# multicom-toolbox/Chromosome3D

Hardware: AMD Instinct MI355X
Metric: SA-steps/sec (replica-steps/s, 20 replicas of chr1_500kb in all: 20 per GPU, weak scaling; regions of 20 steps inside the first 2172 of the schedule's 5172: MD and FIRE steps in front of the final minimisation); wall-clock per chromosome (higher is better)
Workload: dtype f32

## Files before the change

chromosome3d_amd/csrc/c3d_api.cpp:

```cpp
#include <cstdlib>

#include "c3d_ctx.h"

using namespace c3d::host;

namespace {
inline void philox4x32(const uint32_t ctr_in[4], const uint32_t key_in[2], uint32_t out[4]) {
    uint32_t c[4] = {ctr_in[0], ctr_in[1], ctr_in[2], ctr_in[3]};
    uint32_t k[2] = {key_in[0], key_in[1]};
    for (int r = 0; r < 10; ++r) {
        const uint64_t p0 = (uint64_t)0xD2511F53u * c[0];
        const uint64_t p1 = (uint64_t)0xCD9E8D57u * c[2];
        const uint32_t n0 = (uint32_t)(p1 >> 32) ^ c[1] ^ k[0];
        const uint32_t n1 = (uint32_t)p1;
        const uint32_t n2 = (uint32_t)(p0 >> 32) ^ c[3] ^ k[1];
        const uint32_t n3 = (uint32_t)p0;
        c[0] = n0; c[1] = n1; c[2] = n2; c[3] = n3;
        k[0] += 0x9E3779B9u;
        k[1] += 0xBB67AE85u;
    }
    memcpy(out, c, sizeof(c));
}
inline double u01(uint32_t u) { return ((double)u + 0.5) * (1.0 / 4294967296.0); }
void philox_draw(uint64_t seed, uint32_t replica, uint32_t bead, uint32_t purpose, uint32_t out[4]) {
    const uint32_t ctr[4] = {bead, purpose, 0u, 0u};
    const uint32_t key[2] = {(uint32_t)(seed & 0xFFFFFFFFu) ^ (replica * 0x9E3779B9u), (uint32_t)(seed >> 32) + replica};
    philox4x32(ctr, key, out);
}
void normals4(uint64_t seed, uint32_t replica, uint32_t bead, uint32_t purpose, double g[4]) {
    uint32_t r[4];
    philox_draw(seed, replica, bead, purpose, r);
    const double two_pi = 6.283185307179586476925286766559;
    double a = sqrt(-2.0 * log(u01(r[0]))), b = two_pi * u01(r[1]);
    g[0] = a * cos(b); g[1] = a * sin(b);
    a = sqrt(-2.0 * log(u01(r[2]))); b = two_pi * u01(r[3]);
    g[2] = a * cos(b); g[3] = a * sin(b);
}

void release_context(c3d_ctx* c) {
    for (hipStream_t s : c->gstream) if (s) (void)hipStreamSynchronize(s);
    drop_graphs(c);
    free_replica_buffers(c);
    dev_free(c->buf.tgt); dev_free(c->buf.tgs2);
    dev_free(c->d_prog); dev_free(c->d_claim); dev_free(c->d_score);
    if (c->h_tmo) (void)hipHostFree(c->h_tmo);
    if (c->h_stage) (void)hipHostFree(c->h_stage);
    for (hipEvent_t e : {c->ev0, c->ev1, c->kev0, c->kev1, c->fork_ev}) if (e) (void)hipEventDestroy(e);
    for (hipEvent_t e : c->gev) if (e) (void)hipEventDestroy(e);
    for (hipStream_t s : c->gstream) if (s && s != c->stream) (void)hipStreamDestroy(s);
    if (c->stream) (void)hipStreamDestroy(c->stream);
}

void set_dims(c3d_ctx* c, int n) {
    c->n = n;
    c->npad = (n + 255) / 256 * 256;
    c->ntiles = (n + c3d::kTileRows - 1) / c3d::kTileRows;
    c->rep_floats = (size_t)3 * c->npad;
}

float pad_coord(int comp, int k) { return c3d::kPadCoord * (float)(comp + 1) + 16.0f * (float)k; }

void pack(const c3d_ctx* c, const float* aos, std::vector<float>& soa, bool pad_far) {
    soa.assign(c->rep_floats * c->nrep, 0.0f);
    for (int r = 0; r < c->nrep; ++r) {
        float* base = soa.data() + c->rep_floats * r;
        for (int comp = 0; comp < 3; ++comp) {
            for (int i = 0; i < c->n; ++i) base[(size_t)comp * c->npad + i] = aos[((size_t)r * c->n + i) * 3 + comp];
            if (pad_far)
                for (int i = c->n; i < c->npad; ++i) base[(size_t)comp * c->npad + i] = pad_coord(comp, i - c->n);
        }
    }
}
void unpack(const c3d_ctx* c, const float* soa, float* aos) {
    for (int r = 0; r < c->nrep; ++r) {
        const float* base = soa + c->rep_floats * r;
        for (int comp = 0; comp < 3; ++comp)
            for (int i = 0; i < c->n; ++i) aos[((size_t)r * c->n + i) * 3 + comp] = base[(size_t)comp * c->npad + i];
    }
}

void copy_energies(const c3d_ctx* c, double* e) {
    const double* h = static_cast<const double*>(c->h_stage);
    for (int r = 0; r < c->nrep; ++r) for (int k = 0; k < 3; ++k) e[3 * r + k] = h[4 * r + k];
}
float final_repel_s(const c3d_ctx* c) { return c->stages.empty() ? 0.85f : c->stages.back().repel_s; }

int import64(c3d_ctx* c) {
    LAUNCH_TRY("fp64 import", c3d::launch_import64(dev_model(c), c->buf.X[c->parity], c->b64, c->stream));
    HIP_TRY(hipStreamSynchronize(c->stream));
    return C3D_OK;
}
}

namespace c3d::host {
void free_replica_buffers(c3d_ctx* c) {
    for (int k = 0; k < 2; ++k) {
        dev_free(c->buf.X[k]); dev_free(c->buf.V[k]); dev_free(c->buf.P[k]); dev_free(c->buf.S[k]);
    }
    dev_free(c->d_crec);
    c->crec_bytes = 0; c->cl_ok = false;
    dev_free(c->buf.Vinit); dev_free(c->buf.E); dev_free(c->d_feval);
    dev_free(c->d_sym_scratch); dev_free(c->d_sym_tiles);
    dev_free(c->lb.hist); dev_free(c->lb.part); dev_free(c->lb.S[0]); dev_free(c->lb.S[1]);
    dev_free(c->lb64.hist); dev_free(c->lb64.part); dev_free(c->lb64.S[0]); dev_free(c->lb64.S[1]);
    c->lbfgs_parity = -1;
    dev_free(c->b64.T); dev_free(c->b64.t10); dev_free(c->b64.Vinit); dev_free(c->b64.F);
    for (int k = 0; k < 2; ++k) { dev_free(c->b64.X[k]); dev_free(c->b64.V[k]); dev_free(c->b64.P[k]); dev_free(c->b64.S[k]); }
    c->have_replicas = false;
}
int build_targets64(c3d_ctx* c) {
    const c3d::Model64 m = c3d::model64(dev_model(c), c->model);
    LAUNCH_TRY("fp64 targets", c3d::launch_targets64(m, c3d::form64(m, 0.0, 0), c->b64.t10, c->b64.T, c->stream));
    HIP_TRY(hipStreamSynchronize(c->stream));
    return C3D_OK;
}

int ensure_stage(c3d_ctx* c, size_t bytes) {
    if (bytes <= c->h_stage_bytes) return C3D_OK;
    if (c->h_stage) { HIP_TRY(hipStreamSynchronize(c->stream)); (void)hipHostFree(c->h_stage); c->h_stage = nullptr; c->h_stage_bytes = 0; }
    const size_t cap = std::max<size_t>(bytes, (size_t)64 << 10);
    HIP_TRY(hipHostMalloc(&c->h_stage, cap, hipHostMallocDefault));
    c->h_stage_bytes = cap;
    return C3D_OK;
}
int read_back(c3d_ctx* c, const void* dev, size_t bytes) {
    if (int rc = ensure_stage(c, bytes)) return rc;
    HIP_TRY(hipMemcpyAsync(c->h_stage, dev, bytes, hipMemcpyDeviceToHost, c->stream));
    HIP_TRY(hipStreamSynchronize(c->stream));
    return C3D_OK;
}
}

extern "C" int c3d_device_count(void) {
    int n = 0;
    if (hipGetDeviceCount(&n) != hipSuccess) return 0;
    return n;
}

extern "C" int c3d_create(int device, c3d_ctx** out) {
    if (!out) return fail(C3D_ERR_INVALID, "c3d_create: null out");
    int ndev = 0;
    if (hipGetDeviceCount(&ndev) != hipSuccess || ndev < 1)
        return fail(C3D_ERR_NO_DEVICE, "no HIP device visible: libc3d has no CPU fallback");
    if (device < 0 || device >= ndev) return fail(C3D_ERR_INVALID, "c3d_create: device index out of range");
    HIP_TRY(hipSetDevice(device));
    hipDeviceProp_t prop;
    HIP_TRY(hipGetDeviceProperties(&prop, device));
    if (strncmp(prop.gcnArchName, "gfx950", 6) != 0)
        return fail(C3D_ERR_NO_DEVICE, std::string("device is ") + prop.gcnArchName + ", libc3d is built for gfx950 only");
    int num_xcc = 0;
    if (hipDeviceGetAttribute(&num_xcc, hipDeviceAttributeNumberOfXccs, device) != hipSuccess) num_xcc = 0;
    if (const int rc = preload_units(device)) return rc;
    c3d_ctx* c = new c3d_ctx();
    c->device = device;
    c->num_cus = prop.multiProcessorCount;
    c->num_xcc = num_xcc;
    c3d_default_model(&c->model);
    c3d_default_fire(&c->fire);
    c->stages.resize(c3d_default_schedule(nullptr, 0, 3000));
    c3d_default_schedule(c->stages.data(), (int)c->stages.size(), 3000);
    Entry gate(c, 0u, false);
    if (gate.rc != C3D_OK) { delete c; return gate.rc; }
    bool ok = hipStreamCreateWithFlags(&c->stream, hipStreamNonBlocking) == hipSuccess &&
              hipEventCreate(&c->ev0) == hipSuccess && hipEventCreate(&c->ev1) == hipSuccess &&
              hipEventCreate(&c->kev0) == hipSuccess && hipEventCreate(&c->kev1) == hipSuccess &&
              hipEventCreateWithFlags(&c->fork_ev, hipEventDisableTiming) == hipSuccess;
    c->gstream[0] = c->stream;
    ok = ok && hipHostMalloc(reinterpret_cast<void**>(&c->h_tmo), 64, hipHostMallocMapped) == hipSuccess;
    if (ok) {
        *c->h_tmo = 0;
        ok = hipHostGetDevicePointer(reinterpret_cast<void**>(&c->h_tmo_dev), c->h_tmo, 0) == hipSuccess &&
             hipMalloc(&c->d_claim, sizeof(unsigned) * c3d_ctx::kClaimWords * c3d_ctx::kClaimSets) == hipSuccess;
        c->h_tmo[1] = 0;
    }
    if (!ok) {
        c3d_destroy(c);
        return fail(C3D_ERR_HIP, "cannot create HIP stream/events");
    }
    *out = c;
    return C3D_OK;
}

extern "C" void c3d_destroy(c3d_ctx* c) {
    if (!c) return;
    c->ifr.release();
    {
        Entry gate(c, 0u, false);
        release_context(c);
    }
    delete c;
}

static constexpr int kDefaultMaxBeads = C3D_MAX_BEADS_DEFAULT;
static constexpr int kMaxBeadsLimit = C3D_MAX_BEADS_LIMIT;
static_assert(kDefaultMaxBeads == c3d::kMaxStagedCols, "the default limit is the staged form's");
static int too_many_beads(const c3d_ctx* c, const char* fn, int n) {
    char b[192];
    if (c->max_beads == kDefaultMaxBeads)
        snprintf(b, sizeof b, "%s: %d beads: more than %d are accepted only after c3d_set_option(\"max_beads\", n) (up to %d)", fn, n,
                 kDefaultMaxBeads, kMaxBeadsLimit);
    else
        snprintf(b, sizeof b, "%s: %d beads: more than max_beads = %d (the option goes up to %d)", fn, n, c->max_beads, kMaxBeadsLimit);
    return fail(C3D_ERR_INVALID, b);
}
static constexpr int kRankPrefetchBeads = 2048;

extern "C" int c3d_set_if_matrix(c3d_ctx* c, const double* IF, int n, double alpha, double K) {
    if (!c || !IF || n < 2) return fail(C3D_ERR_INVALID, "c3d_set_if_matrix: bad arguments");
    if (n > c->max_beads) return too_many_beads(c, "c3d_set_if_matrix", n);
    C3D_ENTRY(c, 0u);
    free_replica_buffers(c);
    set_dims(c, n);
    const size_t nn = (size_t)n * n;
    c->ifr.join();
    c->ifr.valid = false;
    if (c->prefetch_ranks && n <= kRankPrefetchBeads) {
        try {
            c->ifr.matrix.assign(IF, IF + nn);
            c->ifr.n = n; c->ifr.range = 3;
            c3d_ctx::IfRanks* const w = &c->ifr;
            c->ifr.worker = std::thread([w] {
                try { c3d::if_pair_ranks(w->matrix.data(), w->n, w->range, w->rank, w->m, w->mean, w->saa); w->valid = true; }
                catch (...) { w->valid = false; }
            });
        } catch (...) { c->ifr.release(); }
    } else {
        c->ifr.release();
    }
    DevTmp<double> dIF, dP, dpart;
    DevTmp<int32_t> ddist;
    DevTmp<unsigned char> dflags;
    DevTmp<unsigned> dnflag;
    const int npartial = 64;
    dev_free(c->buf.tgt); dev_free(c->buf.tgs2);
    c->have_targets = false;
    HIP_TRY(hipMalloc(&dIF.p, sizeof(double) * nn));
    HIP_TRY(hipMalloc(&dP.p, sizeof(double) * nn));
    HIP_TRY(hipMalloc(&dpart.p, sizeof(double) * npartial));
    HIP_TRY(hipMalloc(&ddist.p, sizeof(int32_t) * nn));
    HIP_TRY(hipMalloc(&dflags.p, nn));
    HIP_TRY(hipMalloc(&dnflag.p, sizeof(unsigned)));
    HIP_TRY(hipMalloc(&c->buf.tgt, sizeof(float) * (size_t)n * c->npad));
    HIP_TRY(hipMemcpyAsync(dIF.p, IF, sizeof(double) * nn, hipMemcpyHostToDevice, c->stream));
    HIP_TRY(hipMemsetAsync(dnflag.p, 0, sizeof(unsigned), c->stream));
    HIP_TRY(hipMemsetAsync(dflags.p, 0, nn, c->stream));
    LAUNCH_TRY("K1 launch", c3d::launch_if_to_target(dIF.p, n, c->npad, alpha, K, c->model.min_sep, c->model.rep_sep, dP.p, dpart.p, npartial, ddist.p,
                                                     c->buf.tgt, dflags.p, dnflag.p, c->stream));
    c->h_dist10.resize(nn);
    c->r_i.clear(); c->r_j.clear(); c->r_t10.clear();
    unsigned nflag = 0;
    HIP_TRY(hipMemcpyAsync(c->h_dist10.data(), ddist.p, sizeof(int32_t) * nn, hipMemcpyDeviceToHost, c->stream));
    HIP_TRY(hipMemcpyAsync(&nflag, dnflag.p, sizeof(unsigned), hipMemcpyDeviceToHost, c->stream));
    HIP_TRY(hipStreamSynchronize(c->stream));
    c->k1_recomputed = 0;
    if (nflag) {
        std::vector<unsigned char> flags(nn);
        HIP_TRY(hipMemcpyAsync(flags.data(), dflags.p, nn, hipMemcpyDeviceToHost, c->stream));
        HIP_TRY(hipStreamSynchronize(c->stream));
        double sum = 0.0;
        for (size_t k = 0; k < nn; ++k) sum += pow(IF[k], alpha);
        const double mean = sum / ((double)n * (double)n);
        for (size_t k = 0; k < nn; ++k) {
            if (!flags[k]) continue;
            double v = pow(IF[k], alpha) / mean;
            if (v == 0) continue;
            v = K / v;
            char b[64];
            snprintf(b, sizeof b, "%.1f", v);
            char* dot = strchr(b, '.');
            long long t = atoll(b) * 10 + (dot ? dot[1] - '0' : 0);
            if (t > 2000000000LL) t = 2000000000LL;
            ++c->k1_recomputed;
            if ((int32_t)t == c->h_dist10[k]) continue;
            c->h_dist10[k] = (int32_t)t;
            const int i = (int)(k / n), j = (int)(k % n);
            const int sep = i > j ? i - j : j - i;
            const float enc = (sep >= c->model.min_sep && t > 0) ? (float)((double)t / 10.0) : 0.0f;
            HIP_TRY(hipMemcpyAsync(c->buf.tgt + (size_t)i * c->npad + j, &enc, sizeof(float), hipMemcpyHostToDevice, c->stream));
            HIP_TRY(hipStreamSynchronize(c->stream));
            dev_free(c->buf.tgs2);
            ++c->k1_patched;
        }
    }
    int R = 0;
    for (int i = 0; i < n; ++i)
        for (int j = i + 1; j < n; ++j)
            if (j - i >= c->model.min_sep && c->h_dist10[(size_t)i * n + j] > 0) ++R;
    c->R = R;
    c->have_targets = true;
    build_program(c);
    return C3D_OK;
}

extern "C" int c3d_set_restraints(c3d_ctx* c, int n, int R, const int32_t* ri, const int32_t* rj, const int32_t* rt10) {
    if (!c || n < 2 || R < 0 || (R > 0 && (!ri || !rj || !rt10))) return fail(C3D_ERR_INVALID, "c3d_set_restraints: bad arguments");
    if (n > c->max_beads) return too_many_beads(c, "c3d_set_restraints", n);
    C3D_ENTRY(c, 0u);
    free_replica_buffers(c);
    c->ifr.release();
    set_dims(c, n);
    std::vector<float> enc((size_t)n * c->npad);
    std::fill(enc.begin(), enc.end(), 0.0f);
    for (int k = 0; k < R; ++k) {
        const int i = ri[k] - 1, j = rj[k] - 1;
        if (i < 0 || j < 0 || i >= n || j >= n || i == j) return fail(C3D_ERR_INVALID, "c3d_set_restraints: index out of range");
        if (rt10[k] <= 0) continue;
        const float t = (float)((double)rt10[k] / 10.0);
        enc[(size_t)i * c->npad + j] = c3d::encode_target_host(t);
        enc[(size_t)j * c->npad + i] = c3d::encode_target_host(t);
    }
    dev_free(c->buf.tgt); dev_free(c->buf.tgs2);
    HIP_TRY(hipMalloc(&c->buf.tgt, sizeof(float) * enc.size()));
    HIP_TRY(hipMemcpyAsync(c->buf.tgt, enc.data(), sizeof(float) * enc.size(), hipMemcpyHostToDevice, c->stream));
    HIP_TRY(hipStreamSynchronize(c->stream));
    c->h_dist10.clear();
    {
        std::vector<std::pair<uint64_t, int>> key;
        key.reserve(R);
        for (int k = 0; k < R; ++k) {
            const int i = std::min(ri[k], rj[k]) - 1, j = std::max(ri[k], rj[k]) - 1;
            key.emplace_back((uint64_t)i * n + j, k);
        }
        std::sort(key.begin(), key.end());
        c->r_i.clear(); c->r_j.clear(); c->r_t10.clear();
        int32_t last = 0;
        for (size_t q = 0; q < key.size(); ++q) {
            if (rt10[key[q].second] > 0) last = rt10[key[q].second];
            if (q + 1 < key.size() && key[q + 1].first == key[q].first) continue;
            if (last > 0) { c->r_i.push_back((int32_t)(key[q].first / n)); c->r_j.push_back((int32_t)(key[q].first % n)); c->r_t10.push_back(last); }
            last = 0;
        }
    }
    c->R = R;
    c->have_targets = true;
    build_program(c);
    return C3D_OK;
}

extern "C" int c3d_get_dist10(c3d_ctx* c, int32_t* out) {
    if (!c || !out) return fail(C3D_ERR_INVALID, "c3d_get_dist10: null argument");
    if (c->h_dist10.empty()) return fail(C3D_ERR_INVALID, "c3d_get_dist10: targets were not built from an IF matrix");
    memcpy(out, c->h_dist10.data(), sizeof(int32_t) * c->h_dist10.size());
    return C3D_OK;
}
extern "C" int c3d_num_beads(const c3d_ctx* c) { return c ? c->n : 0; }
extern "C" int c3d_num_restraints(const c3d_ctx* c) { return c ? c->R : 0; }

// ... 390 lines not shown
```

chromosome3d_amd/csrc/c3d_cluster.hip:

```cpp
#include <hip/hip_ext.h>
#include <atomic>
#include <type_traits>
#include <cstdio>
#include <cstdlib>

#include "c3d_step_core.h"

namespace c3d {

typedef unsigned u32x4 __attribute__((ext_vector_type(4)));
constexpr int kClMaxThreads = 1024;

#ifdef C3D_STAMPS
__device__ unsigned long long g_cstamps[64][8];
__device__ unsigned long long g_pstamps[8];
#define CSTAMP(k) do { if (stamper) g_cstamps[s & 63][k] = __builtin_amdgcn_s_memrealtime(); } while (0)
#define CSTAMP_C(k) do { if (cstamper) g_cstamps[s & 63][k] = __builtin_amdgcn_s_memrealtime(); } while (0)
#else
#define CSTAMP(k) do { } while (0)
#define CSTAMP_C(k) do { } while (0)
#endif

template <int POT, int RPW, int NB, int WL, bool LATE, bool TWO>
__device__ __forceinline__ void cluster_body(
    const float* __restrict__ tgt, unsigned* __restrict__ claim, const StepRun* __restrict__ runs, const int P, const int CW, const int NH,
    const int static_place, const int nbeads, const int run0, const int skip0, const int nsteps,
    const unsigned tag_base, u32x4* __restrict__ rec, volatile unsigned* __restrict__ timeout, const unsigned expected,
    const AnnealIO& io, const DevModel& m, const DevFire& fp) {
    constexpr int NPAD = 256 * NB;
    constexpr int MAXT = NPAD / 8;
    constexpr int KUMAX = NB > 2 ? 3 : 2;
    extern __shared__ __attribute__((aligned(16))) float smem[];
    float* xs = smem;
    float* ys = smem + NPAD;
    float* zs = smem + 2 * NPAD;
    float* ps = smem + 3 * NPAD;
    float* fbuf = ps + 4 * MAXT;
    float* cbuf = fbuf + 3 * 64;
    float* lbuf = cbuf + 3 * 64;
    float* lcon = lbuf + 3 * 64;
    float* dump = lcon + 3 * 4 * 2 * 64;
    int* s_slot = reinterpret_cast<int*>(dump + 4);
#ifdef C3D_STAMPS
    const unsigned long long t_entry = __builtin_amdgcn_s_memrealtime();
#endif
    const int tid = threadIdx.x, lane = tid & 63, wave = tid >> 6;
    const int nthreads = (CW + NH) * 64;
    const int RW = CW * RPW;

    const int xcc = (int)(__builtin_amdgcn_s_getreg((3 << 11) | 20) & 0x7);
    const int sp_mode = static_place & 0xff, xcd0 = (static_place >> 8) & 0xff, nxcd = (static_place >> 16) & 0xff;
    int slot;
    if (sp_mode) {
        const unsigned off = ((unsigned)xcc - blockIdx.x + (sp_mode == 2 && blockIdx.x == 0 ? 1u : 0u)) & 7u;
        if (tid == 0) atomicOr(&claim[9], 1u << off);
        slot = (int)(blockIdx.x >> 3);
    } else {
        if (tid == 0) *s_slot = (int)atomicAdd(&claim[xcc], 1u);
        __syncthreads();
        slot = *s_slot;
    }
    const int lxcd = xcc - xcd0;
    const int lrep = lxcd + nxcd * (slot / P), part = slot % P;
#ifdef C3D_STAMPS
    const unsigned long long t_placed = __builtin_amdgcn_s_memrealtime();
#endif
    const bool is_compute = wave >= NH, is_h0 = wave == 0;
    const int cwave = wave - NH;
    const int wg_row0 = part * RW;
    const int row0 = wg_row0 + cwave * RPW;
    const StepRun first_run = runs[run0];
    float4 traw[RPW][NB];
#pragma unroll
    for (int r = 0; r < RPW; ++r)
#pragma unroll
        for (int jb = 0; jb < NB; ++jb) {
            float4 t = make_float4(0, 0, 0, 0);
            if (is_compute) {
                const float* trow = tgt + (size_t)min(row0 + r, nbeads - 1) * NPAD + 256 * jb;
                if (jb < NB - 1 || WL == 4) t = *reinterpret_cast<const float4*>(trow + 4 * lane);
                else if constexpr (WL == 3) {
                    struct F3 { float a, b, c; };
                    const F3 q = *reinterpret_cast<const F3*>(trow + 3 * lane);
                    t = make_float4(q.a, q.b, q.c, 0.0f);
                } else if constexpr (WL == 2) {
                    const float2 q = *reinterpret_cast<const float2*>(trow + 2 * lane);
                    t = make_float4(q.x, q.y, 0.0f, 0.0f);
                } else t = make_float4(trow[lane], 0.0f, 0.0f, 0.0f);
            }
            traw[r][jb] = t;
        }
    if (lxcd < 0 || lxcd >= nxcd || lrep >= m.nrep_g) return;
    const int rep = m.rep_base + lrep;
    const bool solo = P == 1;
    if (!is_compute) __builtin_amdgcn_s_setprio(3);

    const size_t roff = (size_t)rep * 3 * NPAD;
    const int hrow = wg_row0 + lane;
    const bool hfin = is_h0 && lane < RW && hrow < m.n;
#define C3D_HROW_INDEX const size_t ix = roff + hrow, iy = ix + NPAD, iz = iy + NPAD
    constexpr int rec_stride = NPAD + NPAD / 4;
    constexpr int KT = (MAXT + 63) / 64;
    constexpr bool late = LATE;
    const int gthreads = late ? nthreads - 64 : nthreads;
    const int gtid = late ? tid - 64 : tid;
    const int units = late ? m.n : m.n + 2 * m.ntiles;
    const int ku = (units + gthreads - 1) / gthreads;
    const auto rsrc = __builtin_amdgcn_make_buffer_rsrc(rec, 0, (int)(sizeof(u32x4) * 2 * m.nrep_g * rec_stride), 0x00020000);

    float vcx = 0.0f, vcy = 0.0f, vcz = 0.0f;
    FireState st;
    float4 cin[2], pin4 = make_float4(0, 0, 0, 0);
    {
        const float* xin = io.xin;
        const float* pin = io.pin;
        const float* vin = io.vin;
#pragma unroll
        for (int k = 0; k < 2; ++k) {
            const int b = 4 * (tid + k * nthreads);
            cin[k] = b < 3 * NPAD ? *reinterpret_cast<const float4*>(xin + roff + b) : make_float4(0, 0, 0, 0);
        }
        if (tid < m.ntiles) pin4 = reinterpret_cast<const float4*>(pin)[(size_t)rep * m.ntiles + tid];
        if (hfin) { C3D_HROW_INDEX; vcx = vin[ix]; vcy = vin[iy]; vcz = vin[iz]; }
        st = io.sin[rep];
    }
    float* const lc = lcon + (size_t)((wave >= 1 && wave <= 3) ? wave - 1 : 0) * (4 * 2 * 64);
    if (!is_compute && !is_h0 && wave <= 3 && m.nleft > 0) {
        for (int q = 0; q < 4; ++q) {
            const int k = 8 * (wave - 1) + 8 * (NH - 1) * q + (lane >> 3), c = lane & 7;
            float b = 0.0f, a = 0.0f;
            if (k < RW && c < m.nleft && wg_row0 + k < m.n) {
                const float t = tgt[(size_t)(wg_row0 + k) * NPAD + m.jl0 + c];
                b = t * m.inv_rs;
                a = t > 0.0f ? m.inv_rs : 0.0f;
            }
            lc[(2 * q) * 64 + lane] = b; lc[(2 * q + 1) * 64 + lane] = a;
        }
    }
#pragma unroll
    for (int k = 0; k < 2; ++k) {
        const int b = 4 * (tid + k * nthreads);
        if (b < 3 * NPAD) *reinterpret_cast<float4*>(smem + b) = cin[k];
    }
    if (tid < m.ntiles) reinterpret_cast<float4*>(ps)[tid] = pin4;
    if (tid < 3 * 64) lbuf[tid] = 0.0f;
#ifdef C3D_STAMPS
    asm volatile("s_waitcnt lgkmcnt(0)" ::: "memory");
    const unsigned long long t_coords = __builtin_amdgcn_s_memrealtime();
#endif
    constexpr bool PK = POT == 4;
    float4 tv[PK ? 1 : RPW][NB];
    PairConsts2<PK ? RPW : 1, NB> pc;
    float4* const mw = reinterpret_cast<float4*>(dump + 8) + (size_t)(is_compute ? cwave : 0) * (RPW * NB * 64);
    if constexpr (PK) {
        pair_consts2_build<RPW, NB>(m, traw, is_compute, lane, pc, mw);
    } else {
        DevStep p0{};
#pragma unroll
        for (int r = 0; r < RPW; ++r)
#pragma unroll
            for (int jb = 0; jb < NB; ++jb) {
                tv[r][jb] = pair_b<false>(m, traw[r][jb]);
                if (is_compute) mw[(r * NB + jb) * 64 + lane] = pair_a<false>(m, p0, traw[r][jb]);
            }
    }
#ifdef C3D_STAMPS
    asm volatile("s_waitcnt vmcnt(0) lgkmcnt(0)" ::: "memory");
    const unsigned long long t_targets = __builtin_amdgcn_s_memrealtime();
#endif
    int gsrc[KUMAX], gda[KUMAX], gdb[KUMAX], gdc[KUMAX];
    const int dump_off = (int)(dump - smem);
#pragma unroll
    for (int k = 0; k < KUMAX; ++k) {
        const int u = min(max(gtid + gthreads * k, 0), units - 1);
        int src, da, db = dump_off, dc = dump_off;
        if (u < m.n) { src = u; da = u; db = NPAD + u; dc = 2 * NPAD + u; }
        else {
            const int j = u - m.n, t = j >> 1;
            src = NPAD + j;
            if ((j & 1) == 0) { da = 3 * NPAD + 4 * t; db = da + 1; dc = da + 2; }
            else da = 3 * NPAD + 4 * t + 3;
        }
        if (gtid < 0 || gtid + gthreads * k >= units) da = db = dc = dump_off;
        gsrc[k] = src; gda[k] = da; gdb[k] = db; gdc[k] = dc;
    }

#ifdef C3D_STAMPS
    const bool stamper = lrep == 0 && part == 0 && is_h0 && lane == 0;
    const bool cstamper = lrep == 0 && part == 0 && cwave == 0 && lane == 0;
    if (stamper) { g_pstamps[0] = t_entry; g_pstamps[1] = __builtin_amdgcn_s_memrealtime(); g_pstamps[6] = t_placed; }
    if (cstamper) { g_pstamps[4] = t_targets; g_pstamps[5] = t_coords; }
#endif
    auto role_loop = [&](auto role) {
    constexpr int ROLE = decltype(role)::value;
    int s = 0;
    StepRun cur = first_run;
    for (int run = run0;; ++run) {
      if (run != run0) cur = runs[run];
      const DevStep p = cur.p;
      const int count = cur.count;
      const bool needs_partials = p.kind == 0 || p.kind == 1 || p.kind == 2 || (TWO && p.kind == 5);
      for (int it = run == run0 ? skip0 : 0; it < count; ++it, ++s) {
#ifdef C3D_STAMPS
        if (cstamper && s == 0) g_pstamps[7] = __builtin_amdgcn_s_memrealtime();
#endif
        __syncthreads();
        CSTAMP(0);
#ifdef C3D_STAMPS
        if (stamper && s == 0) g_pstamps[2] = __builtin_amdgcn_s_memrealtime();
#endif
        CSTAMP_C(6);

        float hx0 = 0.0f, hy0 = 0.0f, hz0 = 0.0f;
        StepScalars sc;
        sc.lam = 1.0f; sc.cmx = sc.cmy = sc.cmz = 0.0f; sc.keep = 0.0f; sc.mix = 0.0f;
        if constexpr (ROLE == 0) {
            if (p.kind != 4) {
                float Fx, Fy, Fz;
                if constexpr (PK) tile_pair_sums_pk<RPW, NB, WL>(m, p, pc, mw, xs, ys, zs, row0, lane, Fx, Fy, Fz);
                else tile_pair_sums_reg<POT, RPW, NB, WL, 1>(m, p, tv, mw, xs, ys, zs, row0, lane, Fx, Fy, Fz);
                if (lane < RPW) {
                    const int k = cwave * RPW + lane;
                    fbuf[k] = Fx; fbuf[64 + k] = Fy; fbuf[128 + k] = Fz;
                }
                CSTAMP_C(7);
            }
        } else if constexpr (ROLE == 1) {
            if (p.kind != 2 && !(TWO && p.kind == 5)) { st.dt = fp.dt_start; st.alpha = fp.alpha_start; st.npos = 0; st.pad = 0; }
            float4 psum = make_float4(0, 0, 0, 0);
            if (needs_partials) {
                if (late && !solo && s > 0) {
                    const unsigned tagp = tag_base + (unsigned)s;
                    const int basep = ((s & 1) * m.nrep_g + lrep) * rec_stride + NPAD;
                    u32x4 a[KT], b[KT];
                    unsigned spins = 0;
                    for (;;) {
                        bool ok = true;
                        asm volatile("" ::: "memory");
#pragma unroll
                        for (int k = 0; k < KT; ++k) {
                            const int t = min(lane + 64 * k, m.ntiles - 1);
                            a[k] = __builtin_amdgcn_raw_buffer_load_b128(rsrc, (basep + 2 * t) * 16, 0, 16);
                            b[k] = __builtin_amdgcn_raw_buffer_load_b128(rsrc, (basep + 2 * t + 1) * 16, 0, 16);
                        }
#pragma unroll
                        for (int k = 0; k < KT; ++k) ok &= a[k].x == tagp && b[k].x == tagp;
                        if (__all(ok)) break;
                        __builtin_amdgcn_s_sleep(1);
                        ++spins;
                        if (spins > (1u << 18) || ((spins & 1023u) == 0 && *timeout != 0u)) {
                            if (lane == 0) *timeout = 1u;
                            return;
                        }
                    }
#pragma unroll
                    for (int k = 0; k < KT; ++k)
                        if (lane + 64 * k < m.ntiles)
                            reinterpret_cast<float4*>(ps)[lane + 64 * k] = make_float4(__uint_as_float(a[k].y), __uint_as_float(a[k].z), __uint_as_float(a[k].w), __uint_as_float(b[k].y));
                }
                for (int t = lane; t < m.ntiles; t += 64) {
                    const float4 q = reinterpret_cast<const float4*>(ps)[t];
                    psum.x += q.x; psum.y += q.y; psum.z += q.z; psum.w += q.w;
                }
                psum = wave_sum4(psum);
                psum.x = __uint_as_float(__builtin_amdgcn_readfirstlane(__float_as_uint(psum.x)));
                psum.y = __uint_as_float(__builtin_amdgcn_readfirstlane(__float_as_uint(psum.y)));
                psum.z = __uint_as_float(__builtin_amdgcn_readfirstlane(__float_as_uint(psum.z)));
                psum.w = __uint_as_float(__builtin_amdgcn_readfirstlane(__float_as_uint(psum.w)));
            }
            sc = step_scalars<TWO>(m, p, fp, psum, st);
            if (lane < RW && hrow < NPAD) { hx0 = xs[hrow]; hy0 = ys[hrow]; hz0 = zs[hrow]; }
            CSTAMP(1);
        } else if (p.kind != 4) {
            for (int cb = 16 * (wave - 1); cb < RW; cb += 16 * (NH - 1)) {
                const int k = cb + (lane >> 2);
                float cx, cy, cz;
                chain_term(m, p, xs, ys, zs, wg_row0 + k, lane & 3, k < RW, cx, cy, cz);
                cx = quad_chain_sum(cx); cy = quad_chain_sum(cy); cz = quad_chain_sum(cz);
                if ((lane & 3) == 0 && k < RW) { cbuf[k] = cx; cbuf[64 + k] = cy; cbuf[128 + k] = cz; }
            }
            if (m.nleft > 0) {
                const PairK kk = pair_k(m, p);
                for (int q = 0; q < 4; ++q) {
                    const int k = 8 * (wave - 1) + 8 * (NH - 1) * q + (lane >> 3), c = lane & 7;
                    if (8 * (wave - 1) + 8 * (NH - 1) * q < RW) {
                        const bool active = k < RW && c < m.nleft && wg_row0 + k < m.n;
                        float lx, ly, lz;
                        leftover_terms<POT, false>(m, p, kk, xs, ys, zs, min(wg_row0 + k, m.n - 1), c, active, lc[(2 * q) * 64 + lane], lc[(2 * q + 1) * 64 + lane], lx, ly, lz);
                        if (c == 0 && k < RW) { lbuf[k] = lx; lbuf[64 + k] = ly; lbuf[128 + k] = lz; }
                    }
                }
            }
        }
        __syncthreads();
        CSTAMP(2);
        const bool last = s + 1 == nsteps;
        const unsigned tag = tag_base + (unsigned)s + 1u;
        const int base = (((s + 1) & 1) * m.nrep_g + lrep) * rec_stride;

        if constexpr (ROLE == 1) {
            float4 q = make_float4(0, 0, 0, 0);
            float xn = 0.0f, yn = 0.0f, zn = 0.0f;
            auto row_update = [&](auto kc) {
                constexpr int K = decltype(kc)::value;
                DevStep pk = p;
                pk.kind = K;
                if (hfin) {
                    float Fx = 0.0f, Fy = 0.0f, Fz = 0.0f;
                    if constexpr (K != 4) {
                        const float sx0 = fbuf[lane], sy0 = fbuf[64 + lane], sz0 = fbuf[128 + lane];
                        const float lx = lbuf[lane], ly = lbuf[64 + lane], lz = lbuf[128 + lane];
                        const float cx = cbuf[lane], cy = cbuf[64 + lane], cz = cbuf[128 + lane];
                        const bool lo = m.nleft > 0;
                        const float sx = lo ? sx0 + lx : sx0, sy = lo ? sy0 + ly : sy0, sz = lo ? sz0 + lz : sz0;
                        Fx = row_total<false>(pk, sx, cx);
                        Fy = row_total<false>(pk, sy, cy);
                        Fz = row_total<false>(pk, sz, cz);
                    }
                    float vx0 = vcx, vy0 = vcy, vz0 = vcz;
                    if constexpr (K == 3 || K == 6) { vx0 = vy0 = vz0 = 0.0f; }
                    else if constexpr (K == 4) { C3D_HROW_INDEX; const float* vinit = io.vinit; vx0 = vinit[ix]; vy0 = vinit[iy]; vz0 = vinit[iz]; }
                    finish_row(m, pk, fp, sc, st, Fx, Fy, Fz, hx0, hy0, hz0, vx0, vy0, vz0, xn, yn, zn, vcx, vcy, vcz, q);
                    if (!last && !solo) {
                        u32x4 o;
                        o.x = tag; o.y = __float_as_uint(xn); o.z = __float_as_uint(yn); o.w = __float_as_uint(zn);
                        __builtin_amdgcn_raw_buffer_store_b128(o, rsrc, (base + hrow) * 16, 0, 0);
                    }
                } else {
                    xn = hx0; yn = hy0; zn = hz0;
                }
            };
            bool two_point_step = false;
            if constexpr (TWO) {
                two_point_step = p.kind >= 5;
                if (p.kind == 5) row_update(std::integral_constant<int, 5>{});
                else if (p.kind == 6) row_update(std::integral_constant<int, 6>{});
            }
            if (!two_point_step) switch (p.kind) {
                case 0: row_update(std::integral_constant<int, 0>{}); break;
                case 1: row_update(std::integral_constant<int, 1>{}); break;
                case 2: row_update(std::integral_constant<int, 2>{}); break;
                case 3: row_update(std::integral_constant<int, 3>{}); break;
                default: row_update(std::integral_constant<int, 4>{}); break;
            }
            if (late && !last && !solo) { CSTAMP(4); __builtin_amdgcn_s_barrier(); }
            float4 t = q;
            t.x += dpp_mov<0xB1>(t.x); t.y += dpp_mov<0xB1>(t.y); t.z += dpp_mov<0xB1>(t.z); t.w += dpp_mov<0xB1>(t.w);
            t.x += dpp_mov<0x4E>(t.x); t.y += dpp_mov<0x4E>(t.y); t.z += dpp_mov<0x4E>(t.z); t.w += dpp_mov<0x4E>(t.w);
            t.x += dpp_mov<0x12C>(t.x); t.y += dpp_mov<0x12C>(t.y); t.z += dpp_mov<0x12C>(t.z); t.w += dpp_mov<0x12C>(t.w);
            CSTAMP(3);
            if (last) {
                if (hfin) {
                    C3D_HROW_INDEX;
                    float* xout = io.xout;
                    float* vout = io.vout;
                    xout[ix] = xn; xout[iy] = yn; xout[iz] = zn;
                    vout[ix] = vcx; vout[iy] = vcy; vout[iz] = vcz;
                }
                const int tl = (wg_row0 + lane) >> 3;
                if ((lane & 7) == 0 && lane < RW && tl < m.ntiles) reinterpret_cast<float4*>(io.pout)[(size_t)rep * m.ntiles + tl] = t;
                if (lane == 0 && part == 0) io.sout[rep] = st;
                if (lane == 0 && atomicAdd(&claim[8], 1u) + 1u == expected) {
                    const unsigned seen = sp_mode ? atomicOr(&claim[9], 0u) : 1u;
                    if ((seen & (seen - 1u)) == 0u) timeout[1] = tag_base | 1u;
                    else timeout[2] = 1u;
                }
#ifdef C3D_STAMPS
                if (stamper) g_pstamps[3] = __builtin_amdgcn_s_memrealtime();
#endif
                return;
            }
            if (solo) {
                if (lane < RW && hrow < NPAD) { xs[hrow] = xn; ys[hrow] = yn; zs[hrow] = zn; }
                if ((lane & 7) == 0 && lane < RW) reinterpret_cast<float4*>(ps)[lane >> 3] = t;
            } else if ((lane & 7) == 0 && lane < RW && ((wg_row0 + lane) >> 3) < m.ntiles) {
                u32x4 o0, o1;
                o0.x = tag; o0.y = __float_as_uint(t.x); o0.z = __float_as_uint(t.y); o0.w = __float_as_uint(t.z);
                o1.x = tag; o1.y = __float_as_uint(t.w); o1.z = 0u; o1.w = 0u;
                const int u0 = base + NPAD + 2 * ((wg_row0 + lane) >> 3);
                __builtin_amdgcn_raw_buffer_store_b128(o0, rsrc, u0 * 16, 0, 0);
                __builtin_amdgcn_raw_buffer_store_b128(o1, rsrc, (u0 + 1) * 16, 0, 0);
            }
            CSTAMP(5);
            if (solo || late) continue;
        }
        {
            if (last) return;
            if (solo) continue;
            __builtin_amdgcn_s_barrier();
            u32x4 v[KUMAX];
            unsigned spins = 0;
            for (;;) {
                bool ok = true;
                asm volatile("" ::: "memory");
#pragma unroll
                for (int k = 0; k < KUMAX; ++k)
                    if (k < ku) v[k] = __builtin_amdgcn_raw_buffer_load_b128(rsrc, (base + gsrc[k]) * 16, 0, 16);
#pragma unroll
                for (int k = 0; k < KUMAX; ++k)
                    if (k < ku) ok &= v[k].x == tag;
                if (__all(ok)) break;
                __builtin_amdgcn_s_sleep(1);
                ++spins;
                if (spins > (1u << 18) || ((spins & 1023u) == 0 && *timeout != 0u)) {
                    if (lane == 0) *timeout = 1u;
                    return;
                }
            }
#pragma unroll
            for (int k = 0; k < KUMAX; ++k)
                if (k < ku) { smem[gda[k]] = __uint_as_float(v[k].y); smem[gdb[k]] = __uint_as_float(v[k].z); smem[gdc[k]] = __uint_as_float(v[k].w); }
        }
      }
    }
    };
    if (is_compute) role_loop(std::integral_constant<int, 0>{});
    else if (is_h0) role_loop(std::integral_constant<int, 1>{});
    else role_loop(std::integral_constant<int, 2>{});
}

#define C3D_CLUSTER_ARGS                                                                                                                  \
    const float* __restrict__ tgt, unsigned* __restrict__ claim, const StepRun* __restrict__ runs, const int P, const int CW, const int NH, \
    const int static_place, const int nbeads, const int run0, const int skip0, const int nsteps, const unsigned tag_base,                 \
    u32x4* __restrict__ rec, volatile unsigned* __restrict__ timeout, const unsigned expected, const AnnealIO io, const DevModel m, const DevFire fp
#define C3D_CLUSTER_PASS tgt, claim, runs, P, CW, NH, static_place, nbeads, run0, skip0, nsteps, tag_base, rec, timeout, expected, io, m, fp
template <int POT, int RPW, int NB, int WL, bool LATE>
__global__ __launch_bounds__(kClMaxThreads) void k_cluster(C3D_CLUSTER_ARGS) { cluster_body<POT, RPW, NB, WL, LATE, false>(C3D_CLUSTER_PASS); }
template <int POT, int RPW, int NB, int WL, bool LATE>
__global__ __launch_bounds__(kClMaxThreads) void k_cluster_tp(C3D_CLUSTER_ARGS) { cluster_body<POT, RPW, NB, WL, LATE, true>(C3D_CLUSTER_PASS); }
#undef C3D_CLUSTER_ARGS
#undef C3D_CLUSTER_PASS

constexpr bool cluster_late_ok(int pot, int rpw, int nb, int wl) { return pot >= 3 && rpw * (4 * (nb - 1) + wl) >= 6; }
#ifndef C3D_CLUSTER_POT
#ifdef C3D_STAMPS
hipError_t read_cluster_stamps(unsigned long long* out) { return hipMemcpyFromSymbol(out, HIP_SYMBOL(g_cstamps), sizeof(unsigned long long) * 64 * 8); }
hipError_t read_cluster_pstamps(unsigned long long* out) { return hipMemcpyFromSymbol(out, HIP_SYMBOL(g_pstamps), sizeof(unsigned long long) * 8); }
#endif

__global__ __launch_bounds__(kClMaxThreads) void k_tear16(u32x4* buf, unsigned* stop, unsigned long long* stats, int iters) {
    const auto rsrc = __builtin_amdgcn_make_buffer_rsrc(buf, 0, kClMaxThreads * 16, 0x00020000);
    const int tid = threadIdx.x;
    if (blockIdx.x == 0) {
        for (int i = 1; i <= iters; ++i) {
            u32x4 v; v.x = v.y = v.z = v.w = (unsigned)i;
            __builtin_amdgcn_raw_buffer_store_b128(v, rsrc, tid * 16, 0, 0);
        }
        __threadfence();
        if (tid == 0) atomicExch(stop, 1u);
        return;
    }
    const auto ssrc = __builtin_amdgcn_make_buffer_rsrc(stop, 0, 4, 0x00020000);
    unsigned long long reads = 0, torn = 0, fresh = 0;
    unsigned lastv = 0;
    for (unsigned guard = 0; guard < (1u << 26); ++guard) {
        asm volatile("" ::: "memory");
        const u32x4 v = __builtin_amdgcn_raw_buffer_load_b128(rsrc, tid * 16, 0, 16);
        ++reads;
        if (!(v.x == v.y && v.y == v.z && v.z == v.w)) ++torn;
        if (v.x != lastv) { ++fresh; lastv = v.x; }
        if ((reads & 255) == 0 && __builtin_amdgcn_raw_buffer_load_b32(ssrc, 0, 0, 16) != 0u) break;
    }
    atomicAdd(&stats[0], reads); atomicAdd(&stats[1], torn); atomicAdd(&stats[2], fresh);
}
hipError_t launch_tear16(int num_cus, void* buf, unsigned* stop, unsigned long long* stats, int iters, hipStream_t s) {
    hipLaunchKernelGGL(k_tear16, dim3(num_cus), dim3(kClMaxThreads), 0, s, reinterpret_cast<u32x4*>(buf), stop, stats, iters);
    return hipGetLastError();
}


bool cluster_plan(const DevModel& m, int num_cus, int num_xcc, int forced_geom, int forced_late, int xcd_count, ClusterPlan* plan) {
    if (m.npad > 1024 || num_xcc != 8 || num_cus < 8 || num_cus % 8) return false;
    const int cus_per_xcd = num_cus / 8;
    if (xcd_count < 1 || xcd_count > 8) return false;
    const int per_xcd = (m.nrep_g + xcd_count - 1) / xcd_count;
    const int nb = m.npad / 256;
    static const int geoms[][4] = {{8, 1, 4, 1}, {8, 2, 4, 1}, {12, 2, 4, 1}, {8, 4, 4, 1}, {10, 4, 4, 1}, {12, 4, 4, 1}, {8, 3, 4, 1},
                                   {4, 2, 4, 1}, {4, 4, 4, 1}, {6, 4, 4, 1}};
    double best = 1e30;
    bool found = false;
    const int fcw = forced_geom / 100, frpw = forced_geom / 10 % 10, fnh = forced_geom % 10;
    for (const auto& g : geoms) {
        const int cw = g[0], rpw = g[1], nh = g[2], wpc = g[3], rw = cw * rpw;
        if (fcw && (cw != fcw || rpw != frpw || nh != fnh)) continue;
        if (rw % 8 || rw > 64) continue;
        if (rpw * nb > 8) continue;
        if (m.noe_pot < 3 && (m.wl != 4 || m.nleft != 0)) continue;
        if (m.nleft > 0 && (nh != 4 || (rw + 8 * (nh - 1) - 1) / (8 * (nh - 1)) > 4)) continue;
        const int P = (m.n + rw - 1) / rw;
        if (per_xcd * P > cus_per_xcd * wpc) continue;
        const int threads = (cw + nh) * 64;
        const int kumax = nb > 2 ? 3 : 2;
        const int late = P > 1 && forced_late != 0 && cluster_late_ok(m.noe_pot, rpw, nb, m.wl) &&
                         (m.noe_pot != 4 || ((cw + 3) / 4) * rpw * (4 * (nb - 1) + m.wl) >= 12);
        if ((late ? m.n : m.n + 2 * ((m.n + 7) / 8)) > (late ? threads - 64 : threads) * kumax) continue;
        size_t lds = sizeof(float) * (3 * m.npad + 4 * (m.npad / 8) + 9 * 64 + 24 * 64 + 16) + (size_t)cw * rpw * nb * 64 * 16;
        if (wpc == 1) { if (lds < 84 * 1024) lds = 84 * 1024; }
        else if (lds > 78 * 1024 || threads > 512) continue;
        const int wps = (cw * wpc + 3) / 4;
        const double per_slot = m.noe_pot == 4 ? (rpw / 2) * 22.0 + (rpw & 1) * 19.0 : rpw * 15.0;
        const double valu = (wps == 1 ? 1.6 : (wps == 2 ? 1.15 : 1.0)) * wps * ((4 * (nb - 1) + m.wl) * per_slot + 60.0);
        const double serial = 200.0 + (P > 1 ? 140.0 + 0.92 * m.n : 0.0);
        const double cost = wpc == 1 ? valu + serial : (valu > serial ? valu + 0.35 * serial : 0.5 * valu + serial);
        if (cost < best) {
            best = cost; found = true;
            plan->rpw = rpw; plan->cw = cw; plan->helpers = nh; plan->wgs_per_cu = wpc; plan->parts = P; plan->per_xcd = per_xcd;
            plan->grid = num_cus * wpc; plan->threads = threads; plan->units = 2 * rw; plan->device = 0; plan->lds = lds;
            plan->expected = (unsigned)(m.nrep_g * P);
            plan->late_tiles = late;
            plan->xcd_count = xcd_count;
        }
    }
    return found;
}

size_t cluster_record_bytes(const DevModel& m, const ClusterPlan& pl) { (void)pl; return (size_t)2 * m.nrep_g * (m.npad + m.npad / 4) * 16; }

#endif

template <int POT, int RPW, int NB, int WL, bool LATE>
static hipError_t cluster_go(const DevModel& m, const DevFire& fp, const ClusterPlan& pl, const AnnealIO& io, const float* tgt, void* rec,
                             const StepRun* runs, int run0, int skip0, int nsteps, unsigned tag_base, unsigned* timeout, unsigned* claim,
                             hipStream_t s) {
#if defined(C3D_CLUSTER_TP)
    constexpr bool kHasLean = false, kHasTp = true;
#elif defined(C3D_CLUSTER_POT)
    constexpr bool kHasLean = true, kHasTp = false;
#else
    constexpr bool kHasLean = true, kHasTp = true;
#endif
    const int tp = pl.two_point ? 1 : 0;
    if ((tp && !kHasTp) || (!tp && !kHasLean)) return hipErrorInvalidValue;
    const int sp = (pl.static_place & 0xff) | ((pl.xcd_base & 0xff) << 8) | ((pl.xcd_count & 0xff) << 16);
#define C3D_CL_LAUNCH(K)                                                                                                                              \
    do {                                                                                                                                              \
        if (pl.t0 && pl.t1)                                                                                                                           \
            hipExtLaunchKernelGGL((K<POT, RPW, NB, WL, LATE>), dim3(pl.grid), dim3(pl.threads), pl.lds, s, pl.t0, pl.t1, 0, tgt, claim, runs,          \
                                  pl.parts, pl.cw, pl.helpers, sp, m.n, run0, skip0, nsteps, tag_base, reinterpret_cast<u32x4*>(rec), timeout, pl.expected, io, m, fp); \
        else                                                                                                                                          \
            hipLaunchKernelGGL((K<POT, RPW, NB, WL, LATE>), dim3(pl.grid), dim3(pl.threads), pl.lds, s, tgt, claim, runs, pl.parts, pl.cw, pl.helpers, \
                               sp, m.n, run0, skip0, nsteps, tag_base, reinterpret_cast<u32x4*>(rec), timeout, pl.expected, io, m, fp);                \
    } while (0)
    if constexpr (kHasTp) { if (tp) C3D_CL_LAUNCH(k_cluster_tp); }
    if constexpr (kHasLean) { if (!tp) C3D_CL_LAUNCH(k_cluster); }
#undef C3D_CL_LAUNCH
    return hipGetLastError();
}
template <int POT, class F>
static void for_each_cluster_form(F&& f) {
    auto widths = [&](auto R, auto B) {
        auto w = [&](auto W) {
            f(R, B, W, bool_c<false>{});
            if constexpr (cluster_late_ok(POT, R, B, W)) f(R, B, W, bool_c<true>{});
        };
        w(int_c<4>{});
        if constexpr (POT >= 3) { w(int_c<3>{}); w(int_c<2>{}); w(int_c<1>{}); }
    };
    widths(int_c<1>{}, int_c<1>{}); widths(int_c<1>{}, int_c<2>{}); widths(int_c<1>{}, int_c<3>{}); widths(int_c<1>{}, int_c<4>{});
    widths(int_c<2>{}, int_c<1>{}); widths(int_c<2>{}, int_c<2>{}); widths(int_c<2>{}, int_c<3>{}); widths(int_c<2>{}, int_c<4>{});
    widths(int_c<3>{}, int_c<1>{}); widths(int_c<3>{}, int_c<2>{});
    widths(int_c<4>{}, int_c<1>{}); widths(int_c<4>{}, int_c<2>{});
}
template <int POT>
static hipError_t cluster_geom(const DevModel& m, const DevFire& fp, const ClusterPlan& pl, const AnnealIO& io, const float* tgt, void* rec,
                               const StepRun* runs, int run0, int skip0, int nsteps, unsigned tag_base, unsigned* timeout, unsigned* claim,
                               hipStream_t s) {
    hipError_t e = hipErrorInvalidValue;
    for_each_cluster_form<POT>([&](auto R, auto B, auto W, auto L) {
        if (pl.rpw == R && m.npad == 256 * B && m.wl == W && (pl.late_tiles != 0) == L)
            e = cluster_go<POT, R, B, W, L>(m, fp, pl, io, tgt, rec, runs, run0, skip0, nsteps, tag_base, timeout, claim, s);
    });
    return e;
}

template <int POT, bool TP>
static hipError_t cluster_prepare_unit() {
    hipError_t e = hipSuccess;
    for_each_cluster_form<POT>([&](auto R, auto B, auto W, auto L) {
        const void* k;
        if constexpr (TP) k = reinterpret_cast<const void*>(&k_cluster_tp<POT, R, B, W, L>);
        else k = reinterpret_cast<const void*>(&k_cluster<POT, R, B, W, L>);
        if (e == hipSuccess) e = hipFuncSetAttribute(k, hipFuncAttributeMaxDynamicSharedMemorySize, 160 * 1024);
    });
    return e;
}

#define C3D_CL_CAT2(a, b) a##b
#define C3D_CL_CAT(a, b) C3D_CL_CAT2(a, b)
#if defined(C3D_CLUSTER_POT) && defined(C3D_CLUSTER_TP)
hipError_t C3D_CL_CAT(launch_cluster_tp_pot, C3D_CLUSTER_POT)(const DevModel& m, const DevFire& fp, const ClusterPlan& pl, const AnnealIO& io, const float* tgt, void* rec,
                          const StepRun* runs, int run0, int skip0, int nsteps, unsigned tag_base, unsigned* timeout, unsigned* claim,
                          hipStream_t s) {
    return cluster_geom<C3D_CLUSTER_POT>(m, fp, pl, io, tgt, rec, runs, run0, skip0, nsteps, tag_base, timeout, claim, s);
}
hipError_t C3D_CL_CAT(preload_cluster_tp_pot, C3D_CLUSTER_POT)() { return cluster_prepare_unit<C3D_CLUSTER_POT, true>(); }
#elif defined(C3D_CLUSTER_POT)
hipError_t C3D_CL_CAT(launch_cluster_pot, C3D_CLUSTER_POT)(const DevModel& m, const DevFire& fp, const ClusterPlan& pl, const AnnealIO& io, const float* tgt, void* rec,
                          const StepRun* runs, int run0, int skip0, int nsteps, unsigned tag_base, unsigned* timeout, unsigned* claim,
                          hipStream_t s) {
    return cluster_geom<C3D_CLUSTER_POT>(m, fp, pl, io, tgt, rec, runs, run0, skip0, nsteps, tag_base, timeout, claim, s);
}
hipError_t C3D_CL_CAT(preload_cluster_pot, C3D_CLUSTER_POT)() { return cluster_prepare_unit<C3D_CLUSTER_POT, false>(); }
#else
using ClusterLaunch = hipError_t(const DevModel& m, const DevFire& fp, const ClusterPlan& pl, const AnnealIO& io, const float* tgt, void* rec,
                                 const StepRun* runs, int run0, int skip0, int nsteps, unsigned tag_base, unsigned* timeout, unsigned* claim,
                                 hipStream_t s);
#if defined(C3D_CLUSTER_SPLIT)
ClusterLaunch launch_cluster_pot0, launch_cluster_pot1, launch_cluster_pot2, launch_cluster_pot3, launch_cluster_pot4;
ClusterLaunch launch_cluster_tp_pot0, launch_cluster_tp_pot1, launch_cluster_tp_pot2, launch_cluster_tp_pot3, launch_cluster_tp_pot4;
hipError_t preload_cluster_pot0(), preload_cluster_pot1(), preload_cluster_pot2(), preload_cluster_pot3(), preload_cluster_pot4();
hipError_t preload_cluster_tp_pot0(), preload_cluster_tp_pot1(), preload_cluster_tp_pot2(), preload_cluster_tp_pot3(), preload_cluster_tp_pot4();
static ClusterLaunch* const kClusterLaunch[2][5] = {{launch_cluster_pot0, launch_cluster_pot1, launch_cluster_pot2, launch_cluster_pot3, launch_cluster_pot4},
                                                    {launch_cluster_tp_pot0, launch_cluster_tp_pot1, launch_cluster_tp_pot2, launch_cluster_tp_pot3, launch_cluster_tp_pot4}};
static hipError_t (*const kClusterPreload[2][5])() = {{preload_cluster_pot0, preload_cluster_pot1, preload_cluster_pot2, preload_cluster_pot3, preload_cluster_pot4},
                                                      {preload_cluster_tp_pot0, preload_cluster_tp_pot1, preload_cluster_tp_pot2, preload_cluster_tp_pot3, preload_cluster_tp_pot4}};
#endif
hipError_t launch_cluster(const DevModel& m, const DevFire& fp, const ClusterPlan& pl, const AnnealIO& io, const float* tgt, void* rec,
                          const StepRun* runs, int run0, int skip0, int nsteps, unsigned tag_base, unsigned* timeout, unsigned* claim,
                          hipStream_t s) {
#if defined(C3D_CLUSTER_SPLIT)
    return kClusterLaunch[pl.two_point][device_pot(m.noe_pot)](m, fp, pl, io, tgt, rec, runs, run0, skip0, nsteps, tag_base, timeout, claim, s);
#else
    return with_pot(m.noe_pot, [&](auto POT) { return cluster_geom<POT>(m, fp, pl, io, tgt, rec, runs, run0, skip0, nsteps, tag_base, timeout, claim, s); });
#endif
}

AnnealIO anneal_io(const DevBuffers& b, int parity) {
    const int q = parity ^ 1;
    AnnealIO io;
    io.pin = b.P[parity]; io.xin = b.X[parity]; io.vin = b.V[parity]; io.vinit = b.Vinit; io.sin = b.S[parity];
    io.xout = b.X[q]; io.vout = b.V[q]; io.pout = b.P[q]; io.sout = b.S[q];
    return io;
}

hipError_t preload_cluster_unit(int pot, bool two_point) {
    if (pot < 0 || pot > 4) return hipErrorInvalidValue;
#if defined(C3D_CLUSTER_SPLIT)
    return kClusterPreload[two_point][pot]();
#else
    return with_pot(pot, [&](auto POT) { return with_bool(two_point, [&](auto TP) { return cluster_prepare_unit<POT, TP>(); }); });
#endif
}
hipError_t preload_cluster_base_unit() {
    hipFuncAttributes a;
    return hipFuncGetAttributes(&a, reinterpret_cast<const void*>(&k_tear16));
}
#endif

}
```

chromosome3d_amd/csrc/c3d_config.cpp:

```cpp
#include <climits>

#include "c3d_ctx.h"

using namespace c3d::host;

namespace {
float clamp_scale(const c3d_ctx* c) { return dev_model(c).noe_pot == 4 ? c->model.mrswitch : c->model.rswitch; }

enum Stale : unsigned { STALE_REPLICAS = 1, STALE_GRAPHS = 2, STALE_PAIR_TARGETS = 4, STALE_PROGRAM = 8 };
void drop_stale(c3d_ctx* c, unsigned stale) {
    if (stale & STALE_REPLICAS) free_replica_buffers(c);
    if (stale & STALE_PAIR_TARGETS) dev_free(c->buf.tgs2);
    if (stale & STALE_PROGRAM) build_program(c);
    else if (stale & STALE_GRAPHS) drop_graphs(c);
}
int drop_stale_gated(c3d_ctx* c, unsigned stale) {
    const bool device_side = ((stale & STALE_REPLICAS) && (c->buf.X[0] || c->b64.t10)) || ((stale & STALE_PAIR_TARGETS) && c->buf.tgs2) ||
                             ((stale & (STALE_GRAPHS | STALE_PROGRAM)) && !c->graphs.empty());
    if (!device_side) { drop_stale(c, stale); return C3D_OK; }
    C3D_GATE(c);
    drop_stale(c, stale);
    return C3D_OK;
}
bool holds_lbfgs_stage(const c3d_ctx* c) { return std::any_of(c->stages.begin(), c->stages.end(), [](const c3d_stage& s) { return s.kind == 8; }); }

using Admit = const char* (*)(c3d_ctx* c, double value, const char* refusal);
template <class Member, class V> const char* store(Member& m, V v) { m = v; return nullptr; }
template <auto M> const char* flag(c3d_ctx* c, double v, const char*) { return store(c->*M, v != 0); }
template <auto M> const char* tristate(c3d_ctx* c, double v, const char*) { return store(c->*M, v < 0 ? -1 : (v != 0)); }
template <auto M, int... Set> const char* one_of(c3d_ctx* c, double v, const char* refusal) { return ((v != Set) && ...) ? refusal : store(c->*M, (int)v); }
template <auto M, int Lo, int Hi> const char* whole_in(c3d_ctx* c, double v, const char* refusal) { return v != (int)v || v < Lo || v > Hi ? refusal : store(c->*M, (int)v); }
template <auto M, int Lo, int Hi> const char* truncated_in(c3d_ctx* c, double v, const char* refusal) { return v < Lo || v > Hi ? refusal : store(c->*M, (int)v); }
template <auto M, bool (*Valid)(int)> const char* chunk(c3d_ctx* c, double v, const char* refusal) { return v != (int)v || (v != 0 && !Valid((int)v)) ? refusal : store(c->*M, (int)v); }
const char* set_resident(c3d_ctx* c, double v, const char*) { c->resident_skip = 0; return store(c->resident, v < 0 ? -1 : (v != 0)); }
const char* set_precision(c3d_ctx* c, double v, const char* refusal) {
    if (v != 32 && v != 64) return refusal;
    if (v == 64 && !c->f64_lbfgs && holds_lbfgs_stage(c)) return "precision 64: the schedule holds a stage of kind 8 (L-BFGS), which has no fp64 form";
    return store(c->precision, (int)v);
}
const char* set_f64_lbfgs(c3d_ctx* c, double v, const char* refusal) {
    if (v != 0 && v != 1) return refusal;
    if (v == 0 && c->precision == 64 && holds_lbfgs_stage(c)) return "f64_lbfgs: precision is 64 and the schedule holds a stage of kind 8 (L-BFGS); change one of them first";
    return store(c->f64_lbfgs, v != 0);
}
const char* set_symmetric(c3d_ctx* c, double v, const char*) { return store(c->sym, v > 0); }
const char* set_static_placement(c3d_ctx* c, double v, const char*) { c->inject_misplaced = v == 2; return store(c->static_place, v != 0); }
const char* set_num_xcc(c3d_ctx* c, double v, const char*) { return store(c->num_xcc, (int)v); }
const char* set_xcd_count(c3d_ctx* c, double v, const char* refusal) { return (int)v < 1 || (int)v > 8 || c->xcd_base + (int)v > 8 ? refusal : store(c->xcd_count, (int)v); }
const char* set_xcd_base(c3d_ctx* c, double v, const char* refusal) { return (int)v < 0 || (int)v + c->xcd_count > 8 ? refusal : store(c->xcd_base, (int)v); }
const char* set_late_tiles(c3d_ctx* c, double v, const char*) { return store(c->cluster_late, v != 0 ? -1 : 0); }
const char* set_spin_wait(c3d_ctx* c, double v, const char*) { return store(c->spin_wait_us, v < 0 ? 0 : v); }
const char* set_resident_min_ops(c3d_ctx* c, double v, const char*) { return store(c->resident_min_ops, v < 1 ? 1 : (int)v); }
const char* set_graph_chunk(c3d_ctx* c, double v, const char* refusal) { return v < 8 ? refusal : store(c->graph_chunk, (int)v & ~1); }

constexpr unsigned R = STALE_REPLICAS, G = STALE_GRAPHS, T = STALE_PAIR_TARGETS, P = STALE_PROGRAM;
using X = c3d_ctx;
const struct Option { const char* key; unsigned stale; Admit admit; const char* refusal; } kOptions[] = {
    {"use_graph",                 0,     flag<&X::use_graph>},
    {"rows_per_wave",             G,     one_of<&X::rpw, 1, 2, 4>, "rows_per_wave must be 1, 2 or 4"},
    {"replica_groups",            G,     truncated_in<&X::ngroups, 1, X::kMaxGroups>, "replica_groups must be 1..4"},
    {"event_timing",              0,     flag<&X::event_timing>},
    {"kernel_timing",             0,     flag<&X::kernel_timing>},
    {"resident",                  0,     set_resident},
    {"precision",                 R | G, set_precision, "precision must be 32 or 64"},
    {"eval_rows_per_wave",        0,     one_of<&X::eval_rpw, 2, 4, -2>, "eval_rows_per_wave must be 4, 2 (packed pair term) or -2 (two rows per wave, scalar pair term)"},
    {"pair_targets",              T | G, flag<&X::pair_targets>},
    {"wide_tiles",                G,     flag<&X::wide_tiles>},
    {"symmetric",                 R | G, set_symmetric},
    {"start",                     0,     one_of<&X::start_mode, 0, 1>, "start must be 0 (random coil) or 1 (extended strand)"},
    {"cluster",                   0,     tristate<&X::cluster>},
    {"resident_inject_timeout",   0,     flag<&X::inject_timeout>},
    {"narrow_columns",            R | G, flag<&X::narrow_columns>},
    {"cluster_static_placement",  0,     set_static_placement},
    {"cluster_inject_incomplete", 0,     flag<&X::inject_incomplete>},
    {"cluster_num_xcc",           R,     set_num_xcc},
    {"prefetch_ranks",            0,     flag<&X::prefetch_ranks>},
    {"device_ranks",              0,     one_of<&X::device_ranks, -1, 0, 1>, "device_ranks is 0 (the device beyond 5120 beads), 1 (the device for every symmetric matrix) or -1 (the host)"},
    {"final_minimiser_steps",     P,     truncated_in<&X::bb_steps, 2, INT_MAX>, "c3d_set_option: final_minimiser_steps >= 2"},
    {"final_minimiser",           P,     one_of<&X::final_bb, 0, 1>, "c3d_set_option: final_minimiser is 0 (FIRE) or 1 (two-point step size)"},
    {"lbfgs_memory",              G,     whole_in<&X::lbfgs_mem, 1, c3d::kLbfgsMaxPairs>, "c3d_set_option: lbfgs_memory is 1..8"},
    {"cluster_xcd_count",         R,     set_xcd_count, "cluster_xcd_count: 1..8, and cluster_xcd_base + cluster_xcd_count <= 8"},
    {"cluster_xcd_base",          0,     set_xcd_base, "cluster_xcd_base: 0 .. 8 - cluster_xcd_count"},
    {"cluster_late_tiles",        R,     set_late_tiles},
    {"cluster_geometry",          R,     truncated_in<&X::cluster_geom, 0, 1699>, "cluster_geometry = 100 compute waves + 10 rows per wave + helper waves"},
    {"spin_wait_us",              0,     set_spin_wait},
    {"resident_min_ops",          0,     set_resident_min_ops},
    {"stage_dma",                 G,     flag<&X::stage_dma>},
    {"max_beads",                 0,     whole_in<&X::max_beads, C3D_MAX_BEADS_DEFAULT, C3D_MAX_BEADS_LIMIT>, "max_beads must be an integer from 5120 to 16384"},
    {"embed_max_beads",           0,     whole_in<&X::embed_max_beads, C3D_EMBED_MAX_BEADS_DEFAULT, C3D_EMBED_MAX_BEADS_LIMIT>, "embed_max_beads must be an integer from 4549 to 16384"},
    {"f64_max_beads",             0,     whole_in<&X::f64_max_beads, C3D_F64_MAX_BEADS_DEFAULT, C3D_F64_MAX_BEADS_LIMIT>, "f64_max_beads must be an integer from 2560 to 16384"},
    {"f64_lbfgs",                 0,     set_f64_lbfgs, "f64_lbfgs must be 0 or 1"},
    {"f64_column_chunk",          G,     chunk<&X::f64_column_chunk, c3d::column_chunk64_valid>, "f64_column_chunk must be 0 (by size), 256, 512 or 1024"},
    {"embed_form",                0,     one_of<&X::embed_form, 0, 1>, "embed_form is 0 (k_dg_eig while it fits, tiled beyond) or 1 (tiled)"},
    {"embed_batch",               0,     whole_in<&X::embed_batch, 0, INT_MAX>, "embed_batch is 0 (by the scratch budget) or a number of replicas"},
    {"column_chunk",              G,     chunk<&X::column_chunk, c3d::column_chunk_valid>, "column_chunk must be 0 (the library's choice), 256, 1024 or 2048"},
    {"graph_chunk",               G,     set_graph_chunk, "graph_chunk must be >= 8"},
};

template <auto M> double value(const c3d_ctx* c) { return (double)(c->*M); }
template <auto M> double planned(const c3d_ctx* c) { return c->cl_ok ? (double)(c->cl_plan.*M) : 0.0; }
int rms_force(const c3d_ctx* c, double* out) {
    if (!c->have_replicas) return fail(C3D_ERR_INVALID, "c3d_get_stat: rms_force needs replicas");
    C3D_ENTRY(c, 0u);
    return max_rms_force(const_cast<c3d_ctx*>(c), out);
}
int lbfgs_resets(const c3d_ctx* c, double* out) {
    *out = 0;
    const c3d::LbfgsState* dev = c->lbfgs_parity < 0 ? nullptr : c->precision == 64 ? c->lb64.S[c->lbfgs_parity] : c->lb.S[c->lbfgs_parity];
    if (!dev) return C3D_OK;
    C3D_ENTRY(c, 0u);
    if (int rc = read_back(const_cast<c3d_ctx*>(c), dev, sizeof(c3d::LbfgsState) * c->nrep)) return rc;
    const c3d::LbfgsState* h = static_cast<const c3d::LbfgsState*>(c->h_stage);
    long r = 0;
    for (int k = 0; k < c->nrep; ++k) r += h[k].resets;
    *out = (double)r;
    return C3D_OK;
}
const struct Stat { const char* key; double (*get)(const c3d_ctx*); int (*enter)(const c3d_ctx*, double*); } kStats[] = {
    {"graph_captures", value<&X::graph_captures>},
    {"last_kernel_us", [](const c3d_ctx* c) { return 1e3 * c->last_kernel_ms; }},
    {"last_host_launch_us", value<&X::last_host_launch_us>},
    {"last_host_sync_us", value<&X::last_host_sync_us>},
    {"graph_launches", value<&X::graph_launches>},
    {"graphs_cached", [](const c3d_ctx* c) { return (double)c->graphs.size(); }},
    {"step_launches", value<&X::step_launches>},
    {"resident_launches", value<&X::resident_launches>},
    {"cluster_launches", value<&X::cluster_launches>},
    {"resident_fallbacks", value<&X::resident_fallbacks>},
    {"cluster_incomplete", value<&X::cluster_incomplete>},
    {"spin_completions", value<&X::spin_completions>},
    {"cluster_static_placement", value<&X::static_place>},
    {"cluster_placement_mismatches", value<&X::placement_mismatches>},
    {"num_xcc", value<&X::num_xcc>},
    {"rms_force", nullptr, rms_force},
    {"lbfgs_steps", value<&X::lbfgs_steps>},
    {"lbfgs_resets", nullptr, lbfgs_resets},
    {"k1_recomputed", value<&X::k1_recomputed>},
    {"k1_patched", value<&X::k1_patched>},
    {"last_path", value<&X::last_path>},
    {"rank_prefetch_hits", value<&X::rank_prefetch_hits>},
    {"device_rank_runs", value<&X::device_rank_runs>},
    {"score_wide_runs", value<&X::score_wide_runs>},
    {"compare_runs", value<&X::compare_runs>},
    {"f64_evals", value<&X::f64_evals>},
    {"superpose_runs", value<&X::superpose_runs>},
    {"rmsd_table_runs", value<&X::rmsd_table_runs>},
    {"ensemble_map_runs", value<&X::ensemble_map_runs>},
    {"ensemble_score_runs", value<&X::ensemble_score_runs>},
    {"geometry_runs", value<&X::geometry_runs>},
    {"separation_runs", value<&X::separation_runs>},
    {"stratified_runs", value<&X::stratified_runs>},
    {"stratified_if_ms", value<&X::stratified_if_ms>},
    {"stratified_models_ms", value<&X::stratified_models_ms>},
    {"bead_runs", value<&X::bead_runs>},
    {"bead_if_ms", value<&X::bead_if_ms>},
    {"bead_models_ms", value<&X::bead_models_ms>},
    {"cluster_xcd_count", value<&X::xcd_count>},
    {"cluster_xcd_base", value<&X::xcd_base>},
    {"cluster_ok", value<&X::cl_ok>},
    {"cluster_parts", planned<&c3d::ClusterPlan::parts>},
    {"cluster_rows_per_wave", planned<&c3d::ClusterPlan::rpw>},
    {"cluster_late_tiles", planned<&c3d::ClusterPlan::late_tiles>},
    {"cluster_compute_waves", planned<&c3d::ClusterPlan::cw>},
    {"cluster_helper_waves", planned<&c3d::ClusterPlan::helpers>},
    {"cluster_wgs_per_cu", planned<&c3d::ClusterPlan::wgs_per_cu>},
    {"replica_groups", [](const c3d_ctx* c) { return (double)active_groups(c); }},
    {"embed_form", value<&X::last_embed_form>},
    {"embed_batches", value<&X::last_embed_batches>},
    {"units_loaded", [](const c3d_ctx*) { return (double)units_loaded(); }},
    {"units_loaded_mask", [](const c3d_ctx* c) { return (double)units_loaded_mask(c->device); }},
};

template <class Row, size_t N> const Row* find_row(const Row (&rows)[N], const char* key) {
    for (const Row& r : rows) if (!strcmp(key, r.key)) return &r;
    return nullptr;
}
}

namespace c3d::host {
const char* option_key(int k) { return k >= 0 && k < (int)std::size(kOptions) ? kOptions[k].key : nullptr; }
const char* stat_key(int k) { return k >= 0 && k < (int)std::size(kStats) ? kStats[k].key : nullptr; }

c3d::DevModel dev_model(const c3d_ctx* c) {
    c3d::DevModel m{};
    const c3d_model& h = c->model;
    m.n = c->n; m.npad = c->npad; m.ntiles = c->ntiles; m.nrep = c->nrep;
    m.rep_base = 0; m.nrep_g = c->nrep;
    m.rpw = c->rpw;
    m.stage_dma = c->stage_dma;
    m.noe_pot = h.noe_pot; m.ang_mode = h.ang_mode; m.rep_sep = h.rep_sep;
    m.mexp = h.msoexp == 2 ? 2 : 1;
    m.rs = h.rswitch;
    m.tail_c = h.asym * h.rswitch;
    m.tail_b = (m.tail_c - 2.0f * h.rswitch) * h.rswitch * h.rswitch;
    m.mrs = h.mrswitch; m.nmrs = -h.mrswitch;
    m.inv_rs = 1.0f / h.rswitch; m.nm_rs = -h.mrswitch / h.rswitch;
    if (h.noe_pot == 3 && h.msoexp == 2 && h.masym == 0.0f && m.tail_b == 0.0f && m.tail_c == 2.0f * m.rs) {
        m.noe_pot = 4;
        m.inv_rs = 1.0f / h.mrswitch; m.nm_rs = h.rswitch / h.mrswitch;
    }
    {
        const int cols_last = c->n - (c->npad - 256);
        int wl = cols_last / 64, nleft = cols_last - 64 * wl;
        if (wl == 0 || nleft > 8) { wl = std::min(4, wl + 1); nleft = 0; }
        if (!c->narrow_columns || c->npad > 1024) { wl = 4; nleft = 0; }
        m.wl = wl; m.nleft = nleft; m.jl0 = c->npad - 256 + 64 * wl;
    }
    m.mtail_c = h.masym;
    m.mtail_b = (m.mtail_c - 2.0f * h.mrswitch) * h.mrswitch * h.mrswitch * (m.mexp == 2 ? h.mrswitch : 1.0f);
    m.k_bond2 = 2.0f * h.k_bond; m.b0 = h.b0;
    m.k_ang2 = 2.0f * h.k_ang; m.a0 = h.a0;
    m.acc = c3d::kAccel / h.mass;
    const int ndf = std::max(3 * c->n - 3, 1);
    m.t_fac = h.mass / c3d::kAccel / ((float)ndf * c3d::kBoltz);
    m.fbeta = h.fbeta;
    m.inv_n = 1.0f / (float)c->n;
    return m;
}
c3d::DevStep dev_step(const c3d_ctx* c, int kind, float dt, float w_all, float w_vdw, float repel_s, float t_bath) {
    c3d::DevStep p;
    p.kind = kind; p.dt = dt; p.w_all = w_all;
    p.w_noe2n = -2.0f * w_all * c->model.s_noe;
    p.w_rep4 = 4.0f * w_vdw * c->model.k_rep;
    const float rr = repel_s * c->model.r0_rep;
    p.rep_r2 = rr * rr;
    p.inv_rep_r2 = rr > 0.0f ? 1.0f / p.rep_r2 : 0.0f;
    p.w_rep4r2 = p.w_rep4 * p.rep_r2;
    p.w_rs = p.w_noe2n * clamp_scale(c);
    p.kq = p.w_rs != 0.0f ? p.w_rep4r2 / p.w_rs : 0.0f;
    p.t_bath = t_bath;
    return p;
}
}

extern "C" void c3d_default_model(c3d_model* m) {
    if (!m) return;
    m->min_sep = 5; m->noe_pot = 3; m->rep_sep = 2; m->ang_mode = 1;
    m->s_noe = 10.0f; m->rswitch = 0.5f; m->asym = 2.0f;
    m->k_bond = 500.0f; m->b0 = 3.93f;
    m->k_ang = 15.0f; m->a0 = 5.55f;
    m->r0_rep = 5.25f; m->k_rep = 4.0f;
    m->mass = 100.0f; m->fbeta = 10.0f;
    m->mrswitch = 10.0f; m->masym = 0.0f; m->msoexp = 2;
}
extern "C" void c3d_default_fire(c3d_fire_params* f) {
    if (!f) return;
    f->dt_start = 0.002f; f->dt_max = 0.02f; f->f_inc = 1.1f; f->f_dec = 0.5f;
    f->alpha_start = 0.1f; f->f_alpha = 0.99f; f->max_step = 0.5f; f->n_min = 5;
}
extern "C" int c3d_default_schedule(c3d_stage* st, int cap, int min_steps) {
    std::vector<c3d_stage> v;
    v.push_back({2, 200, 0.0f, 1.0f, 20.0f, 0.5f, 0.0f});
    const float hot_t = 2000.0f, hot_dt = 0.003f;
    const int hot_n[5] = {125, 125, 125, 500, 125};
    const float hot_w[5] = {0.1f, 0.2f, 0.2f, 0.4f, 1.0f};
    const float hot_v[5] = {20.0f, 20.0f, 0.01f, 0.003f, 0.003f};
    const float hot_r[5] = {0.5f, 0.5f, 0.9f, 0.9f, 0.9f};
    for (int k = 0; k < 5; ++k) v.push_back({0, hot_n[k], hot_dt, hot_w[k], hot_v[k], hot_r[k], hot_t});
    const int ncycle = (int)(hot_t / 25.0f);
    const int nstep = 1000 / ncycle;
    const double vdw_step = pow(4.0 / 0.003, 1.0 / ncycle);
    const double rad_step = (1.0 - 0.85) / ncycle;
    double radius = 1.0, kv = 0.003, bath = hot_t;
    for (int i = 0; i <= ncycle; ++i) {
        v.push_back({1, nstep, 0.005f, 1.0f, (float)kv, (float)radius, (float)bath});
        radius = std::max(0.85, radius - rad_step);
        kv = std::min(4.0, kv * vdw_step);
        bath -= 25.0;
    }
    v.push_back({5, min_steps, 0.0f, 1.0f, 1.0f, 0.85f, 0.0f});
    if (st) for (int k = 0; k < (int)v.size() && k < cap; ++k) st[k] = v[k];
    return (int)v.size();
}

extern "C" int c3d_set_model(c3d_ctx* c, const c3d_model* m) {
    if (!c || !m) return fail(C3D_ERR_INVALID, "c3d_set_model: null argument");
    const int msoexp = m->msoexp == 0 ? 2 : m->msoexp;
    if (m->mass <= 0 || m->rswitch <= 0 || m->min_sep < 1 || m->rep_sep < 1 || m->rep_sep > 3 || m->noe_pot < 0 || m->noe_pot > 3 || m->mrswitch <= 0 || (msoexp != 1 && msoexp != 2))
        return fail(C3D_ERR_INVALID, "c3d_set_model: parameter out of range");
    if (c->have_targets && m->min_sep != c->model.min_sep)
        return fail(C3D_ERR_INVALID, "c3d_set_model: min_sep must be set before the targets are built");
    const bool targets64 = c->precision == 64 && c->b64.T;
    Entry entry(c, 0u, targets64);
    if (entry.rc != C3D_OK) return entry.rc;
    c->model = *m;
    c->model.msoexp = msoexp;
    drop_stale(c, STALE_PAIR_TARGETS | STALE_PROGRAM);
    if (c->have_replicas)
        if (int rc = plan_cluster(c)) return rc;
    return targets64 ? build_targets64(c) : C3D_OK;
}

extern "C" int c3d_set_schedule(c3d_ctx* c, const c3d_stage* st, int n_stages, const c3d_fire_params* fire, float gtol,
                                int check_every) {
    if (!c || !st || n_stages < 1) return fail(C3D_ERR_INVALID, "c3d_set_schedule: bad arguments");
    for (int k = 0; k < n_stages; ++k) {
        if (st[k].kind < 0 || (st[k].kind > 2 && st[k].kind != 5 && st[k].kind != 8) || st[k].nsteps < 0) return fail(C3D_ERR_INVALID, "c3d_set_schedule: bad stage");
        if (st[k].kind == 8 && c->precision == 64 && !c->f64_lbfgs)
            return fail(C3D_ERR_INVALID, "c3d_set_schedule: a stage of kind 8 (L-BFGS) has no fp64 form; set precision 32 first");
    }
    c->stages.assign(st, st + n_stages);
    if (fire) c->fire = *fire;
    c->gtol = gtol;
    if (check_every > 0) c->check_every = check_every;
    return drop_stale_gated(c, STALE_PROGRAM);
}

extern "C" int c3d_set_option(c3d_ctx* c, const char* key, double value) {
    if (!c || !key) return fail(C3D_ERR_INVALID, "c3d_set_option: null argument");
    const Option* row = find_row(kOptions, key);
    if (!row) return fail(C3D_ERR_INVALID, std::string("unknown option ") + key);
    if (const char* refusal = row->admit(c, value, row->refusal)) return fail(C3D_ERR_INVALID, refusal);
    return drop_stale_gated(c, row->stale);
}

extern "C" int c3d_get_stat(const c3d_ctx* c, const char* key, double* value) {
    if (!c || !key || !value) return fail(C3D_ERR_INVALID, "c3d_get_stat: null argument");
    const Stat* row = find_row(kStats, key);
    if (!row) return fail(C3D_ERR_INVALID, std::string("c3d_get_stat: unknown key ") + key);
    if (row->enter) return row->enter(c, value);
    *value = row->get(c);
    return C3D_OK;
}
```

chromosome3d_amd/csrc/c3d_ctx.h:

```cpp
#pragma once
#include <hip/hip_runtime.h>

#include <algorithm>
#include <cmath>
#include <cstdio>
#include <cstring>
#include <map>
#include <string>
#include <thread>
#include <tuple>
#include <vector>

#include "../../include/c3d.h"
#include "c3d_host.h"
#include "c3d_internal.h"

#define LAUNCH_TRY(what, expr)                                                                 \
    do {                                                                                       \
        if (const hipError_t e__ = (expr); e__ != hipSuccess)                                  \
            return c3d::fail(C3D_ERR_HIP, std::string(what ": ") + hipGetErrorString(e__));    \
    } while (0)
#define HIP_TRY(expr) LAUNCH_TRY(#expr, expr)

namespace c3d::host {
using c3d::fail;
template <class T>
struct DevTmp {
    T* p = nullptr;
    ~DevTmp() { if (p) (void)hipFree(p); }
};

struct Op {
    c3d::DevStep p;
    int stage;
    bool counted;
};

struct KernelRecord {
    enum Family { NONE, STEP, LBFGS_EVAL, PAIRS_SYM, STEP64, LBFGS_EVAL64, CLUSTER } family = NONE;
    c3d::StepForm step{};
    c3d::Form64 f64{};
    int pot = 0, rpw = 0, nb = 0, wl = 0;
    bool rs1 = false, late = false, tp = false;
};

template <class T>
void dev_free(T*& p) {
    if (!p) return;
    const hipError_t e = hipFree(p);
    if (e != hipSuccess) (void)fail(C3D_ERR_HIP, std::string("hipFree: ") + hipGetErrorString(e));
    p = nullptr;
}

c3d::DevModel dev_model(const c3d_ctx* c);
c3d::DevStep dev_step(const c3d_ctx* c, int kind, float dt, float w_all, float w_vdw, float repel_s, float t_bath);
const char* option_key(int k);
const char* stat_key(int k);

void free_replica_buffers(c3d_ctx* c);
int build_targets64(c3d_ctx* c);
int ensure_stage(c3d_ctx* c, size_t bytes);
int read_back(c3d_ctx* c, const void* dev, size_t bytes);

enum Unit : unsigned {
    UNIT_DEVICE = 0, UNIT_SCORE, UNIT_CLUSTER_BASE, UNIT_EMBED, UNIT_F64, UNIT_SYM,
    UNIT_CLUSTER_P0, UNIT_CLUSTER_TP0 = UNIT_CLUSTER_P0 + 5, UNIT_COUNT = UNIT_CLUSTER_TP0 + 5
};
constexpr unsigned unit_bit(unsigned u) { return 1u << u; }
struct Entry {
    int rc = C3D_OK;
    bool locked = false;
    Entry(const c3d_ctx* c, unsigned extra, bool launches);
    ~Entry();
    Entry(const Entry&) = delete;
    Entry& operator=(const Entry&) = delete;
};
int preload_units(int device);
long units_loaded();
unsigned units_loaded_mask(int device);

void build_program(c3d_ctx* c);
void drop_graphs(c3d_ctx* c);
int plan_cluster(c3d_ctx* c);
int active_groups(const c3d_ctx* c);
int max_rms_force(c3d_ctx* c, double* out);
}

struct c3d_ctx {
    c3d_model model;
    std::vector<c3d_stage> stages;
    c3d_fire_params fire;
    float gtol = 0.0f;
    int check_every = 250;
    bool use_graph = true;
    int rpw = 2, stage_dma = 1, graph_chunk = 256;
    static constexpr int kMaxGroups = 4;
    int ngroups = 2;
    int event_timing = 1;
    int kernel_timing = 0;
    int precision = 32;
    int f64_max_beads = C3D_F64_MAX_BEADS_DEFAULT;
    bool f64_lbfgs = false;
    int f64_column_chunk = 0;
    int sym = 0;
    int start_mode = 0;
    bool narrow_columns = true;
    int resident = -1;
    int resident_min_ops = 4;
    double spin_wait_us = 400.0;
    int cluster = -1;
    int cluster_late = -1;
    int cluster_geom = 0;
    int xcd_base = 0, xcd_count = 8;
    bool static_place = true;
    int eval_rpw = 4;
    bool pair_targets = true;
    bool wide_tiles = true;
    int column_chunk = 0;
    int max_beads = C3D_MAX_BEADS_DEFAULT;
    int embed_max_beads = C3D_EMBED_MAX_BEADS_DEFAULT;
    int embed_form = 0;
    int embed_batch = 0;
    int bb_steps = 1000;
    bool final_bb = true;
    int lbfgs_mem = 5;
    int prefetch_ranks = 1;
    int device_ranks = 0;
    bool inject_timeout = false;
    bool inject_misplaced = false;
    bool inject_incomplete = false;
    int device = 0, num_cus = 0, num_xcc = 0;
    int n = 0, npad = 0, ntiles = 0, nrep = 0, R = 0;
    size_t rep_floats = 0;
    bool have_targets = false, have_replicas = false;
    uint64_t seed = 82364;
    uint32_t first_rep = 0;
    std::vector<int32_t> h_dist10;
    std::vector<int32_t> r_i, r_j, r_t10;
    c3d::DevBuffers buf{};
    c3d::Buffers64 b64;
    float *d_feval = nullptr, *d_sym_scratch = nullptr;
    int2* d_sym_tiles = nullptr;
    c3d::LbfgsBuffers lb{};
    c3d::LbfgsBuffers64 lb64{};
    int lbfgs_parity = -1;
    int parity = 0;
    struct IfRanks {
        std::thread worker;
        std::vector<double> matrix, rank;
        size_t m = 0;
        double mean = 0, saa = 0;
        int n = 0, range = 0;
        bool valid = false;
        void join() { if (worker.joinable()) worker.join(); }
        void release() {
            join();
            valid = false;
            std::vector<double>().swap(matrix);
            std::vector<double>().swap(rank);
        }
    } ifr;
    std::vector<c3d::host::Op> program;
    size_t pc = 0;
    long steps_done = 0;
    bool zero_weight = false;
    bool has_two_point = false;
    bool has_lbfgs = false;
    std::map<std::tuple<long, int, int, int>, hipGraphExec_t> graphs;
    hipStream_t stream = nullptr;
    hipStream_t gstream[kMaxGroups] = {nullptr, nullptr, nullptr, nullptr};
    hipEvent_t gev[kMaxGroups] = {nullptr, nullptr, nullptr, nullptr};
    hipEvent_t fork_ev = nullptr, ev0 = nullptr, ev1 = nullptr;
    hipEvent_t kev0 = nullptr, kev1 = nullptr;
    bool ev1_recorded = false;
    c3d::host::KernelRecord ran;
    bool cl_ok = false;
    c3d::ClusterPlan cl_plan{};
    void* d_crec = nullptr;
    size_t crec_bytes = 0;
    static constexpr unsigned kClaimSets = 4096;
    static constexpr unsigned kClaimWords = 16;
    unsigned* d_claim = nullptr;
    unsigned cl_seq = 0;
    c3d::StepRun* d_prog = nullptr;
    size_t prog_cap = 0;
    bool prog_dirty = true;
    std::vector<int> op_run, op_skip;
    std::vector<c3d::StepRun> prog_runs;
    unsigned *h_tmo = nullptr, *h_tmo_dev = nullptr;
    int resident_skip = 0;
    int resident_backoff = 0;
    void* h_stage = nullptr;
    size_t h_stage_bytes = 0;
    void* d_score = nullptr;
    size_t d_score_bytes = 0;
    double last_ms = 0, last_kernel_ms = 0;
    long last_steps = 0, last_launches = 0;
    double last_host_launch_us = 0, last_host_sync_us = 0;
    int last_path = 0;
    long graph_captures = 0, graph_launches = 0, step_launches = 0, resident_launches = 0, cluster_launches = 0;
    long spin_completions = 0, lbfgs_steps = 0;
    int resident_fallbacks = 0;
    int cluster_incomplete = 0, placement_mismatches = 0;
    long k1_recomputed = 0, k1_patched = 0;
    int last_embed_form = 0, last_embed_batches = 0;
    long rank_prefetch_hits = 0, device_rank_runs = 0, score_wide_runs = 0;
    long compare_runs = 0, f64_evals = 0;
    long superpose_runs = 0, rmsd_table_runs = 0;
    long ensemble_map_runs = 0, ensemble_score_runs = 0;
    long geometry_runs = 0, separation_runs = 0;
    long stratified_runs = 0, bead_runs = 0;
    double stratified_if_ms = 0, stratified_models_ms = 0;
    double bead_if_ms = 0, bead_models_ms = 0;
};

#define C3D_ENTRY(c, extra)                       \
    c3d::host::Entry entry__((c), (extra), true); \
    if (entry__.rc != C3D_OK) return entry__.rc
#define C3D_GATE(c)                           \
    c3d::host::Entry entry__((c), 0u, false); \
    if (entry__.rc != C3D_OK) return entry__.rc
```

chromosome3d_amd/csrc/c3d_internal.h:

```cpp
#pragma once
#include <hip/hip_runtime.h>
#include <stdint.h>
#include <type_traits>

#include "../../include/c3d.h"
#include "c3d_superpose.h"

namespace c3d {

constexpr float kBoltz = 0.0019872f;
constexpr float kAccel = 418.4f;

constexpr int kTileRows = 8;
constexpr int kEvalRowsPerWave = 4;
constexpr int kEvalBlock = 64 * kTileRows / kEvalRowsPerWave;

constexpr float kPadCoord = 1.0e4f;

struct DevModel {
    int n, npad, ntiles, nrep;
    int rep_base, nrep_g;
    int stage_dma;
    int rpw;
    int noe_pot, ang_mode, rep_sep;
    int mexp;
    float rs, tail_c, tail_b;
    float mrs, mtail_c, mtail_b;
    float nmrs;
    float inv_rs, nm_rs;
    int wl, nleft, jl0;
    float k_bond2, b0;
    float k_ang2, a0;
    float acc;
    float t_fac;
    float fbeta;
    float inv_n;
    const float* tgs2;
};

struct DevStep {
    int kind;
    float dt;
    float w_all;
    float w_noe2n;
    float w_rep4;
    float rep_r2;
    float inv_rep_r2;
    float w_rep4r2;
    float w_rs;
    float kq;
    float t_bath;
};

struct DevFire {
    float dt_start, dt_max, f_inc, f_dec, alpha_start, f_alpha, max_step;
    int n_min;
};

struct FireState {
    float dt, alpha;
    int npos, pad;
};

struct DevBuffers {
    float* tgt;
    float* tgs2;
    float* X[2];
    float* V[2];
    float* Vinit;
    float* P[2];
    FireState* S[2];
    double* E;
};

template <int V> using int_c = std::integral_constant<int, V>;
template <bool V> using bool_c = std::integral_constant<bool, V>;
inline int device_pot(int noe_pot) { return noe_pot == 0 || noe_pot == 1 || noe_pot == 3 || noe_pot == 4 ? noe_pot : 2; }
template <class F> hipError_t with_pot(int pot, F&& f) {
    switch (device_pot(pot)) {
        case 0: return f(int_c<0>{});
        case 1: return f(int_c<1>{});
        case 3: return f(int_c<3>{});
        case 4: return f(int_c<4>{});
        default: return f(int_c<2>{});
    }
}
template <class F> hipError_t with_rpw(int rpw, F&& f) { return rpw == 1 ? f(int_c<1>{}) : rpw == 2 ? f(int_c<2>{}) : f(int_c<4>{}); }
template <class F> hipError_t with_bool(bool b, F&& f) { return b ? f(bool_c<true>{}) : f(bool_c<false>{}); }

inline bool general_tail(const DevModel& m) {
    if (!(m.tail_b == 0.0f && m.tail_c == 2.0f * m.rs)) return true;
    return m.noe_pot == 3 && !(m.mtail_b == 0.0f && m.mtail_c == 2.0f * m.mrs);
}
inline bool general_step(const DevModel& m, const DevStep& p) { return general_tail(m) || p.w_rs == 0.0f; }
inline bool pair_targets_fit(const DevModel& m) { return device_pot(m.noe_pot) == 4 && m.rpw == 2 && m.wl == 4 && m.nleft == 0; }

struct StepForm {
    int pot;
    bool gen;
    int rpw;
    bool nc, pairs, wide;
    int chunk;
};
constexpr int kMaxStagedCols = 5120;
constexpr int kDefaultColumnChunk = 1024;
inline bool column_chunk_valid(int chunk) { return chunk == 256 || chunk == 1024 || chunk == 2048; }
inline int column_chunk_for(const DevModel& m, int option) {
    if (!(m.wl == 4 && m.nleft == 0)) return 0;
    if (option > 0) return option;
    return m.npad <= kMaxStagedCols ? 0 : kDefaultColumnChunk;
}
inline StepForm step_form(const DevModel& m, const DevStep& p, bool wide_tiles, bool pair_targets, bool tgs2_built, int column_chunk) {
    StepForm f;
    f.pot = device_pot(m.noe_pot);
    f.rpw = m.rpw == 1 || m.rpw == 2 ? m.rpw : 4;
    f.gen = general_step(m, p);
    f.nc = !(m.wl == 4 && m.nleft == 0);
    f.pairs = !f.gen && pair_targets_fit(m) && tgs2_built;
    f.wide = wide_tiles && pair_targets && f.pairs && m.npad > 1024;
    f.chunk = column_chunk_for(m, column_chunk);
    return f;
}
inline bool sym_rs1(const DevModel& m) { return m.rs == 1.0f; }

hipError_t launch_step(const DevModel& m, const DevStep& p, const DevFire& fp, const DevBuffers& b, int parity, const StepForm& f, hipStream_t s);
hipError_t launch_eval_forces(const DevModel& m, const DevStep& p, const DevBuffers& b, int parity, float* Fout,
                              bool general_tail, int rows_per_wave, int chunk, hipStream_t s);
hipError_t launch_energy(const DevModel& m, const DevStep& p, const DevBuffers& b, int parity, float s_noe,
                         float k_rep, double rep_r2, hipStream_t s);
hipError_t launch_centre(const DevModel& m, const DevBuffers& b, int parity, hipStream_t s);
constexpr int kLbfgsMaxPairs = 8;
constexpr int kLbfgsQ = 4 * kLbfgsMaxPairs + 4;
struct LbfgsState {
    int cnt, head, mem, resets;
    double gamma;
    double SY[kLbfgsMaxPairs][kLbfgsMaxPairs];
    double YY[kLbfgsMaxPairs][kLbfgsMaxPairs];
};
struct LbfgsBuffers {
    float* hist;
    float* part;
    LbfgsState* S[2];
};
__host__ __device__ inline size_t lbfgs_hist_floats(int npad) { return (size_t)2 * kLbfgsMaxPairs * 3 * npad; }
hipError_t launch_lbfgs_eval(const DevModel& m, const DevStep& p, const DevBuffers& b, const LbfgsBuffers& lb, int parity, int mem,
                             const StepForm& f, hipStream_t s);
hipError_t launch_lbfgs_move(const DevModel& m, const DevStep& p, const DevFire& fp, const DevBuffers& b, const LbfgsBuffers& lb, int parity,
                             int mem, hipStream_t s);
hipError_t launch_lbfgs_direction(const DevModel& m, const DevFire& fp, int rows, const double* sums, const LbfgsState* in, const int* flags,
                                  LbfgsState* out, double* coef, int* shi, hipStream_t s);
size_t pair_targets_floats(int n, int npad);
hipError_t launch_pair_targets(const DevModel& m, const float* tgt, float* tgs2, hipStream_t s);
struct StepRun {
    DevStep p;
    int count;
};
struct AnnealIO {
    const float *pin, *xin, *vin, *vinit;
    const FireState* sin;
    float *xout, *vout, *pout;
    FireState* sout;
};
AnnealIO anneal_io(const DevBuffers& b, int parity);
struct ClusterPlan {
    int rpw, cw, helpers, wgs_per_cu, parts, per_xcd, grid, threads, units, device;
    int static_place = 1;
    int xcd_base = 0, xcd_count = 8;
    bool two_point = false;
    int late_tiles = 0;
    unsigned expected = 0;
    size_t lds;
    hipEvent_t t0 = nullptr, t1 = nullptr;
};
bool cluster_plan(const DevModel& m, int num_cus, int num_xcc, int forced_geom, int forced_late, int xcd_count, ClusterPlan* plan);
size_t cluster_record_bytes(const DevModel& m, const ClusterPlan& pl);
hipError_t launch_cluster(const DevModel& m, const DevFire& fp, const ClusterPlan& pl, const AnnealIO& io, const float* tgt, void* rec,
                          const StepRun* runs, int run0, int skip0, int nsteps, unsigned tag_base, unsigned* timeout,
                          unsigned* claim, hipStream_t s);
hipError_t preload_device_unit();
hipError_t preload_cluster_base_unit();
hipError_t preload_cluster_unit(int pot, bool two_point);
hipError_t preload_score_unit();
hipError_t preload_embed_unit();
hipError_t preload_f64_unit();
hipError_t preload_sym_unit();
hipError_t launch_tear16(int num_cus, void* buf, unsigned* stop, unsigned long long* stats, int iters, hipStream_t s);
void sym_geometry(const DevModel& m, int* Q, int* G, int* ntiles_offdiag, int* ntiles_diag);
size_t sym_scratch_floats(const DevModel& m);
void sym_tile_list(const DevModel& m, int2* out);
hipError_t launch_step_sym(const DevModel& m, const DevStep& p, const DevFire& fp, const DevBuffers& b, int parity, const void* tiles,
                           float* scratch, hipStream_t s);
hipError_t launch_step_scalars(const DevModel& m, const DevStep& p, const DevFire& fp, int rows, const float* psum, const FireState* in,
                               float* scalars, FireState* out, hipStream_t s);
struct Buffers64 {
    int32_t* t10 = nullptr;
    double* T = nullptr;
    double* X[2] = {nullptr, nullptr};
    double* V[2] = {nullptr, nullptr};
    double* Vinit = nullptr;
    double* P[2] = {nullptr, nullptr};
    void* S[2] = {nullptr, nullptr};
    double* F = nullptr;
};
int cols64(int n);
constexpr int kMaxStagedBeads64 = 2560;
constexpr int kDefaultColumnChunk64 = 512;
inline bool column_chunk64_valid(int chunk) { return chunk == 256 || chunk == 512 || chunk == 1024; }
inline int column_chunk64_for(int n, int option) {
    if (option > 0) return n > option ? option : 0;
    return n <= kMaxStagedBeads64 ? 0 : kDefaultColumnChunk64;
}
struct Model64 {
    int n, np, ntiles, min_sep, noe_pot, rep_sep, ang_mode, mexp;
    double s_noe, rs, tail_c, tail_b, mrs, mtail_c, mtail_b;
    double k_bond, b0, k_ang, a0, r0_rep, k_rep, mass, fbeta;
    double nmrs4;
    double t_fac, inv_n;
};
struct Step64 {
    int kind;
    double dt, w_all, w_vdw, repel_s, t_bath;
    double R2, wr4, nws4, wq;
    double acc;
    double kb4, ka4;
    double kacc;
    double a0sq;
};
struct Fire64 {
    double dt_start, dt_max, f_inc, f_dec, alpha_start, f_alpha, max_step;
    int n_min;
};
Model64 model64(const DevModel& d, const c3d_model& h);
Step64 step64(const Model64& m, int kind, double dt, double w_all, double w_vdw, double repel_s, double t_bath);
Fire64 fire64(const c3d_fire_params& f);
struct Form64 {
    int pot;
    bool gen, fold;
    int chunk;
};
inline Form64 form64(const Model64& m, double w_all, int column_chunk) {
    Form64 f;
    f.pot = m.noe_pot;
    f.gen = !(m.tail_b == 0.0 && m.tail_c == 2.0 * m.rs) || (f.pot == 3 && !(m.mtail_b == 0.0 && m.mtail_c == 2.0 * m.mrs));
    f.fold = f.pot == 4 && !f.gen && w_all != 0.0;
    f.chunk = column_chunk64_for(m.n, column_chunk);
    return f;
}
hipError_t launch_step64(const DevModel& d, const Model64& m, const Step64& p, const Fire64& fp, const Form64& f, const Buffers64& b, int parity,
                         hipStream_t s);
struct LbfgsBuffers64 {
    double* hist = nullptr;
    double* part = nullptr;
    LbfgsState* S[2] = {nullptr, nullptr};
};
hipError_t launch_lbfgs_eval64(const DevModel& d, const Model64& m, const Step64& p, const Form64& f, const Buffers64& b, const LbfgsBuffers64& lb,
                               int parity, int mem, hipStream_t s);
hipError_t launch_lbfgs_move64(const DevModel& d, const Model64& m, const Step64& p, const Fire64& fp, const Buffers64& b, const LbfgsBuffers64& lb,
                               int parity, int mem, hipStream_t s);
hipError_t launch_lbfgs_direction64(const Step64& p, const Fire64& fp, int rows, const double* sums, const LbfgsState* in, const int* flags,
                                    LbfgsState* out, double* coef, int* shi, hipStream_t s);
hipError_t launch_targets64(const Model64& m, const Form64& f, const int32_t* t10, double* T, hipStream_t s);
hipError_t launch_tenths64(int n, int R, const int32_t* ri, const int32_t* rj, const int32_t* rt10, int32_t* t10, hipStream_t s);
hipError_t launch_import64(const DevModel& d, const float* Xf, const Buffers64& b, hipStream_t s);
hipError_t launch_export64(const DevModel& d, const Buffers64& b, int parity, float* Xf, float* Vf, float* Pf, hipStream_t s);
hipError_t launch_eval_forces64(const DevModel& d, const Model64& m, const Step64& p, const Form64& f, const Buffers64& b, int parity, double* Fout,
                                hipStream_t s);
hipError_t launch_energy64(const DevModel& d, const Model64& m, double rep_r2, const Buffers64& b, int parity, double* Eout, hipStream_t s);
size_t fire_state64_bytes();
hipError_t launch_if_to_target(const double* IF, int n, int npad, double alpha, double K, int min_sep, int rep_sep,
                               double* scratchP, double* partial, int npartial, int32_t* dist10, float* tgt,
                               unsigned char* flags, unsigned* nflag, hipStream_t s);

constexpr int kDgEigMaxBeads = (int)((160 * 1024 / sizeof(float) - 16) / 9);
hipError_t launch_dg_smooth(const float* tgt, int n, int npad, float b0, float lower, float* U, float* L, hipStream_t s);
hipError_t launch_dg_embed(const float* U, const float* L, int n, int npad, int nrep, uint64_t seed, uint32_t first_replica, int iters,
                           float* v, float* D2, float* wt, float* x0, float* x1, bool tiled, int batch, hipStream_t s);

hipError_t launch_score(const float* xin, const float* tgt, const double* rankA, int n, int npad, int nrep, int range, int min_sep,
                        unsigned nbins, double ma, double mb, double relax, double* xr, unsigned* hist, unsigned* below,
                        double* partial, int* overflow, hipStream_t s);
hipError_t launch_score_bbox(const double* xr, int n, int nrep, double* box, hipStream_t s);
hipError_t launch_score_wide(const double* xr, const float* tgt, const double* rankA, int n, int npad, int nrep, int range, int min_sep,
                             unsigned nbins, double ma, double mb, double relax, unsigned* hist, unsigned* below, double* partial,
                             int* overflow, hipStream_t s);
constexpr int kRankTile = 4096;
inline size_t if_rank_key_slots(size_t mh) {
    size_t slots = kRankTile;
    while (slots < mh) slots <<= 1;
    return slots;
}
hipError_t launch_if_rank_keys(const double* M, int n, int range, unsigned long long* keys, size_t mh, size_t slots, int* asym, hipStream_t s);
hipError_t launch_if_rank_sort(double* M, int n, int range, unsigned long long* keys, size_t mh, size_t slots, double ma, double* saa_rows,
                               hipStream_t s);
constexpr int kCmpModels = 16;
constexpr int model_blocks(int K) { return (K + kCmpModels - 1) / kCmpModels; }
static_assert(kCmpModels == 16, "pair_row shifts by log2(kCmpModels), and a block of pairs is one 256-thread workgroup");
constexpr int pair_row(int tid) { return tid >> 4; }
constexpr int pair_col(int tid) { return tid & (kCmpModels - 1); }
inline size_t compare_chunk_pairs(size_t m, int K) {
    const size_t nb = (size_t)model_blocks(K), want = 2048 / (nb * nb) > 64 ? 2048 / (nb * nb) : 64;
    return ((m + want - 1) / want + 63) / 64 * 64;
}
inline int compare_table_chunks(size_t m, int K) {
    const size_t per = compare_chunk_pairs(m, K);
    return (int)((m + per - 1) / per);
}
hipError_t launch_compare_coords(const float* xin, int n, int npad, int nrep, double* xyz, hipStream_t s);
hipError_t launch_compare_ranks(const double* x, int n, unsigned long long* keys, size_t m, size_t slots, unsigned* ke, double* rowsum,
                                hipStream_t s);
hipError_t launch_compare_table(const double* xyz, const unsigned* ke, const double* rowsum, int n, int K, size_t m, double* sums,
                                double* partial, double* table, hipStream_t s);
constexpr int kSupNoIdent = -(1 << 30);
inline int superpose_chunks(int n) { return (n + 63) / 64; }
inline size_t superpose_partial_doubles(int n, int KB) {
    return (size_t)superpose_chunks(n) * (size_t)model_blocks(KB) * 256 * kSupCov;
}
hipError_t launch_superpose_gather64(const double* X, int n, int np, int nrep, double* xyz, hipStream_t s);
hipError_t launch_superpose_centre(double* xyz, int n, int K, double* cent, hipStream_t s);
hipError_t launch_superpose_fit(const double* A, int KA, const double* B, int KB, int n, int ident, bool mirror, const int* fixed, double* partial,
                                double* cov, double* fit, int* mirrored, double* res, hipStream_t s);
hipError_t launch_superpose_apply(const double* A, int K, int n, const double* fit, const double* shift, double* fitted, hipStream_t s);
hipError_t launch_superpose_mean(const double* fitted, int K, int n, double* mean, double* rmsf, double* dev, hipStream_t s);
hipError_t launch_superpose_store32(const double* fitted, int n, int npad, int nrep, float* X, hipStream_t s);
hipError_t launch_superpose_store64(const double* fitted, int n, int np, int nrep, double* X0, double* X1, hipStream_t s);
constexpr int kEnsModels = 16;
constexpr int kEnsMaxPicks = 4096;
inline int ensemble_tiles(int n) { return (n + 63) / 64; }
hipError_t launch_ensemble_map(const double* xyz, int n, const int* pick, int Kp, double cutoff, double* mean, double* sd, double* contact,
                               hipStream_t s);
hipError_t launch_ensemble_corr(const double* A, const double* B, int n, int range, double ma, double* rows, hipStream_t s);
hipError_t launch_geometry(const double* xyz, int n, int K, double cutoff, int sep, int* bead_clashes, double* nearest, double* furthest,
                           long long* clashes, double* chain, hipStream_t s);
hipError_t launch_separation_profile(const double* xyz, int n, const int* pick, int Kp, double cutoff, double* mean, double* sd, double* contact,
                                     hipStream_t s);
constexpr int kStrFlags = 4;
inline size_t stratified_pairs(int n, int lo, int hi) { return (size_t)(hi - lo + 1) * (size_t)n - ((size_t)hi * (hi + 1) / 2 - (size_t)lo * (lo - 1) / 2); }
hipError_t launch_stratified_if(const double* IF, int n, int lo, int hi, unsigned* a, long long* saa, int* flags, hipStream_t s);
hipError_t launch_stratified_models(const double* xyz, int n, int K, int lo, int hi, const unsigned* a, const long long* saa, long long* sums, int* flags,
                                    hipStream_t s);
hipError_t launch_bead_if(const double* IF, int n, int range, const int* beads, int nb, unsigned* a, long long* saa, int* flags, hipStream_t s);
hipError_t launch_bead_models(const double* xyz, int n, int K, int range, const int* beads, int nb, const unsigned* a, const long long* saa, const float* tgt,
                              int npad, const int* t10, int min_sep, long long* sums, int* restrained, int* satisfied, long long* dev_milli, int* flags,
                              hipStream_t s);
hipError_t launch_accessibility(const double* xyz, int n, int K, const double* points, int P, double R, double R2, double keep2, int* exposed, int* flags,
                                hipStream_t s);

inline float encode_target_host(float t) { return t > 0 ? t : 0.0f; }

}
```

chromosome3d_amd/csrc/c3d_run.cpp:

```cpp
#include <chrono>

#include "c3d_ctx.h"

using namespace c3d::host;

static bool is_two_point(int kind) { return kind == 5 || kind == 6; }
static bool is_lbfgs(int kind) { return kind == 8 || kind == 9; }

namespace c3d::host {
void drop_graphs(c3d_ctx* c) {
    for (auto& kv : c->graphs) (void)hipGraphExecDestroy(kv.second);
    c->graphs.clear();
}

void build_program(c3d_ctx* c) {
    c->program.clear();
    int prev_kind = -1;
    for (size_t s = 0; s < c->stages.size(); ++s) {
        const c3d_stage& st = c->stages[s];
        if (st.kind == 2 || st.kind == 5 || st.kind == 8) {
            const bool lbfgs = st.kind == 8;
            const int nbb = (st.kind == 5 && c->final_bb) || lbfgs ? std::min(st.nsteps, c->bb_steps) : 0;
            for (int k = 0; k < st.nsteps; ++k) {
                const int kind = k < nbb ? (k == 0 ? (lbfgs ? 9 : 6) : (lbfgs ? 8 : 5)) : (k == nbb ? 3 : 2);
                c->program.push_back({dev_step(c, kind, 0.0f, st.w_all, st.w_vdw, st.repel_s, 0.0f), (int)s, true});
            }
        } else {
            if (prev_kind == 2 || prev_kind == 5 || prev_kind == 8 || prev_kind == -1)
                c->program.push_back({dev_step(c, 4, 0.0f, st.w_all, st.w_vdw, st.repel_s, st.t_bath), (int)s, false});
            for (int k = 0; k < st.nsteps; ++k)
                c->program.push_back({dev_step(c, st.kind, st.dt, st.w_all, st.w_vdw, st.repel_s, st.t_bath), (int)s, true});
        }
        prev_kind = st.kind;
    }
    c->pc = 0;
    c->zero_weight = false;
    for (const Op& op : c->program) c->zero_weight = c->zero_weight || op.p.w_rs == 0.0f;
    c->has_two_point = false;
    for (const Op& op : c->program) c->has_two_point = c->has_two_point || is_two_point(op.p.kind);
    c->has_lbfgs = false;
    for (const Op& op : c->program) c->has_lbfgs = c->has_lbfgs || is_lbfgs(op.p.kind);
    drop_graphs(c);
    c->prog_runs.clear();
    c->op_run.assign(c->program.size(), 0);
    c->op_skip.assign(c->program.size(), 0);
    for (size_t k = 0; k < c->program.size(); ++k) {
        const c3d::DevStep& p = c->program[k].p;
        if (!c->prog_runs.empty() && memcmp(&c->prog_runs.back().p, &p, sizeof(p)) == 0) ++c->prog_runs.back().count;
        else c->prog_runs.push_back({p, 1});
        c->op_run[k] = (int)c->prog_runs.size() - 1;
        c->op_skip[k] = c->prog_runs.back().count - 1;
    }
    c->prog_dirty = true;
}

int active_groups(const c3d_ctx* c) { return std::min(c->ngroups, std::max(c->nrep, 1)); }

int plan_cluster(c3d_ctx* c) {
    c3d::DevModel m = dev_model(c);
    m.nrep = c->nrep; m.nrep_g = c->nrep; m.rep_base = 0;
    c->cl_ok = false;
    if (!c3d::cluster_plan(m, c->num_cus, c->num_xcc, c->cluster_geom, c->cluster_late, c->xcd_count, &c->cl_plan)) return C3D_OK;
    c->cl_plan.device = c->device;
    const size_t bytes = c3d::cluster_record_bytes(m, c->cl_plan);
    if (!c->d_crec || bytes > c->crec_bytes) {
        if (c->d_crec) { HIP_TRY(hipStreamSynchronize(c->stream)); dev_free(c->d_crec); }
        c->crec_bytes = 0;
        HIP_TRY(hipMalloc(&c->d_crec, bytes));
        c->crec_bytes = bytes;
    }
    c->cl_seq = 0;
    c->cl_ok = true;
    return C3D_OK;
}

int max_rms_force(c3d_ctx* c, double* out) {
    const int nparts = c->ntiles;
    if (int rc = read_back(c, c->buf.P[c->parity], sizeof(float) * (size_t)c->nrep * nparts * 4)) return rc;
    const float* h = static_cast<const float*>(c->h_stage);
    double worst = 0;
    for (int r = 0; r < c->nrep; ++r) {
        double ff = 0;
        for (int t = 0; t < nparts; ++t) ff += h[((size_t)r * nparts + t) * 4 + 1];
        const double rms = sqrt(ff / (3.0 * c->n));
        if (!(rms <= worst)) worst = rms;
    }
    *out = worst;
    return C3D_OK;
}
}

namespace {
c3d::DevFire dev_fire(const c3d_ctx* c) {
    c3d::DevFire f;
    f.dt_start = c->fire.dt_start; f.dt_max = c->fire.dt_max; f.f_inc = c->fire.f_inc; f.f_dec = c->fire.f_dec;
    f.alpha_start = c->fire.alpha_start; f.f_alpha = c->fire.f_alpha; f.max_step = c->fire.max_step; f.n_min = c->fire.n_min;
    return f;
}

void group_range(const c3d_ctx* c, int g, int& base, int& count) {
    const int G = active_groups(c);
    const int q = c->nrep / G, r = c->nrep % G;
    base = g * q + std::min(g, r);
    count = q + (g < r ? 1 : 0);
}

bool use_sym(const c3d_ctx* c) {
    return c->sym > 0 && c->d_sym_scratch && !c3d::general_tail(dev_model(c));
}

template <class T, class Buffers>
int ensure_lbfgs(c3d_ctx* c, Buffers& lb, int cols) {
    if (lb.hist) return C3D_OK;
    const size_t hist = c3d::lbfgs_hist_floats(cols) * c->nrep, part = (size_t)c->nrep * c->ntiles * c3d::kLbfgsQ;
    HIP_TRY(hipMalloc(&lb.hist, sizeof(T) * hist));
    HIP_TRY(hipMalloc(&lb.part, sizeof(T) * part));
    for (int k = 0; k < 2; ++k) HIP_TRY(hipMalloc(&lb.S[k], sizeof(c3d::LbfgsState) * c->nrep));
    HIP_TRY(hipMemsetAsync(lb.hist, 0, sizeof(T) * hist, c->stream));
    HIP_TRY(hipMemsetAsync(lb.part, 0, sizeof(T) * part, c->stream));
    for (int k = 0; k < 2; ++k) HIP_TRY(hipMemsetAsync(lb.S[k], 0, sizeof(c3d::LbfgsState) * c->nrep, c->stream));
    HIP_TRY(hipStreamSynchronize(c->stream));
    return C3D_OK;
}

int ensure_pair_targets(c3d_ctx* c, const c3d::DevModel& m) {
    if (c->buf.tgs2 || !c->pair_targets || !c3d::pair_targets_fit(m) || c->npad <= 1024 || !c->buf.tgt) return C3D_OK;
    HIP_TRY(hipMalloc(&c->buf.tgs2, sizeof(float) * c3d::pair_targets_floats(c->n, c->npad)));
    LAUNCH_TRY("pair targets", c3d::launch_pair_targets(m, c->buf.tgt, c->buf.tgs2, c->stream));
    HIP_TRY(hipStreamSynchronize(c->stream));
    return C3D_OK;
}
KernelRecord op_kernel(const c3d_ctx* c, const c3d::DevModel& m, const Op& op, const c3d::Model64* m64 = nullptr) {
    KernelRecord k;
    if (c->precision == 64) {
        k.family = is_lbfgs(op.p.kind) ? KernelRecord::LBFGS_EVAL64 : KernelRecord::STEP64;
        k.f64 = c3d::form64(m64 ? *m64 : c3d::model64(m, c->model), c->stages[op.stage].w_all, c->f64_column_chunk);
    } else if (!is_lbfgs(op.p.kind) && use_sym(c)) {
        k.family = KernelRecord::PAIRS_SYM;
        k.pot = c3d::device_pot(m.noe_pot);
        k.rs1 = c3d::sym_rs1(m);
    } else {
        k.family = is_lbfgs(op.p.kind) ? KernelRecord::LBFGS_EVAL : KernelRecord::STEP;
        k.step = c3d::step_form(m, op.p, c->wide_tiles, c->pair_targets, c->buf.tgs2 != nullptr, c->column_chunk);
    }
    return k;
}
int launch_op(c3d_ctx* c, const Op& op, int g, int par) {
    c3d::DevModel m = dev_model(c);
    group_range(c, g, m.rep_base, m.nrep_g);
    if (c->precision == 64) {
        const c3d_stage& st = c->stages[op.stage];
        const c3d::Model64 m64 = c3d::model64(m, c->model);
        const c3d::Step64 p = c3d::step64(m64, op.p.kind, st.dt, st.w_all, st.w_vdw, st.repel_s, st.t_bath);
        const c3d::Fire64 fp = c3d::fire64(c->fire);
        const c3d::Form64 f = op_kernel(c, m, op, &m64).f64;
        if (is_lbfgs(op.p.kind)) {
            hipError_t e = c3d::launch_lbfgs_eval64(m, m64, p, f, c->b64, c->lb64, par, c->lbfgs_mem, c->gstream[g]);
            if (e == hipSuccess) e = c3d::launch_lbfgs_move64(m, m64, p, fp, c->b64, c->lb64, par, c->lbfgs_mem, c->gstream[g]);
            LAUNCH_TRY("fp64 L-BFGS step launch", e);
        } else LAUNCH_TRY("fp64 step launch", c3d::launch_step64(m, m64, p, fp, f, c->b64, par, c->gstream[g]));
        return C3D_OK;
    }
    const KernelRecord k = op_kernel(c, m, op);
    if (k.family == KernelRecord::LBFGS_EVAL) {
        hipError_t e = c3d::launch_lbfgs_eval(m, op.p, c->buf, c->lb, par, c->lbfgs_mem, k.step, c->gstream[g]);
        if (e == hipSuccess) e = c3d::launch_lbfgs_move(m, op.p, dev_fire(c), c->buf, c->lb, par, c->lbfgs_mem, c->gstream[g]);
        LAUNCH_TRY("L-BFGS step launch", e);
        return C3D_OK;
    }
    LAUNCH_TRY("step launch", k.family == KernelRecord::PAIRS_SYM
                                  ? c3d::launch_step_sym(m, op.p, dev_fire(c), c->buf, par, c->d_sym_tiles, c->d_sym_scratch, c->gstream[g])
                                  : c3d::launch_step(m, op.p, dev_fire(c), c->buf, par, k.step, c->gstream[g]));
    return C3D_OK;
}

bool cluster_ok(c3d_ctx* c) {
    if (!c->resident || !c->cluster || !c->cl_ok || !c->d_crec) return false;
    return !c3d::general_tail(dev_model(c));
}

bool launch_was_abandoned(c3d_ctx* c, unsigned done_mark) {
    if (c->h_tmo[2]) { c->h_tmo[2] = 0; c->static_place = false; ++c->placement_mismatches; }
    const bool complete = c->h_tmo[1] == done_mark;
    if (!*c->h_tmo && complete) { c->resident_backoff = 0; return false; }
    if (!*c->h_tmo) ++c->cluster_incomplete;
    *c->h_tmo = 0;
    c->resident_backoff = std::min(4096, std::max(4, 2 * c->resident_backoff));
    c->resident_skip = c->resident_backoff;
    ++c->resident_fallbacks;
    return true;
}

void account_ops(c3d_ctx* c, size_t nops, long launches) {
    for (size_t k = 0; k < nops; ++k)
        if (c->program[c->pc + k].counted) { ++c->steps_done; ++c->last_steps; }
    c->last_launches += launches;
    c->pc += nops;
}

int run_cluster(c3d_ctx* c, size_t nops, bool* ran) {
    if (c->prog_dirty) {
        if (c->prog_runs.size() > c->prog_cap) {
            if (c->d_prog) { HIP_TRY(hipStreamSynchronize(c->stream)); dev_free(c->d_prog); }
            c->prog_cap = std::max<size_t>(c->prog_runs.size(), 256);
            HIP_TRY(hipMalloc(&c->d_prog, sizeof(c3d::StepRun) * c->prog_cap));
        }
        HIP_TRY(hipMemcpyAsync(c->d_prog, c->prog_runs.data(), sizeof(c3d::StepRun) * c->prog_runs.size(), hipMemcpyHostToDevice, c->stream));
        HIP_TRY(hipStreamSynchronize(c->stream));
        c->prog_dirty = false;
    }
    const unsigned seq = c->cl_seq % c3d_ctx::kClaimSets;
    if (seq == 0) {
        HIP_TRY(hipMemsetAsync(c->d_crec, 0, c->crec_bytes, c->stream));
        HIP_TRY(hipMemsetAsync(c->d_claim, 0, sizeof(unsigned) * c3d_ctx::kClaimWords * c3d_ctx::kClaimSets, c->stream));
    }
    ++c->cl_seq;
    if (c->inject_timeout) { *c->h_tmo = 1; c->inject_timeout = false; }
    c->h_tmo[1] = 0;
    const c3d::DevModel m = dev_model(c);
    c3d::ClusterPlan pl = c->cl_plan;
    if (c->inject_incomplete) { ++pl.expected; c->inject_incomplete = false; }
    if (c->kernel_timing) { pl.t0 = c->kev0; pl.t1 = c->kev1; }
    pl.static_place = c->static_place ? (c->inject_misplaced ? 2 : 1) : 0;
    pl.xcd_base = c->xcd_base;
    pl.two_point = false;
    for (size_t k = 0; k < nops && !pl.two_point; ++k) pl.two_point = is_two_point(c->program[c->pc + k].p.kind);
    c->inject_misplaced = false;
    c->h_tmo[2] = 0;
    const auto h0 = std::chrono::steady_clock::now();
    LAUNCH_TRY("cluster launch", c3d::launch_cluster(m, dev_fire(c), pl, c3d::anneal_io(c->buf, c->parity), c->buf.tgt, c->d_crec, c->d_prog,
                                                     c->op_run[c->pc], c->op_skip[c->pc], (int)nops, seq << 20, c->h_tmo_dev,
                                                     c->d_claim + c3d_ctx::kClaimWords * seq, c->stream));
    if (c->event_timing) HIP_TRY(hipEventRecord(c->ev1, c->stream));
    const auto h1 = std::chrono::steady_clock::now();
    bool marked = false;
    if (c->spin_wait_us > 0 && !c->kernel_timing) {
        const unsigned mark = (seq << 20) | 1u;
        for (;;) {
            if (__atomic_load_n(&c->h_tmo[1], __ATOMIC_ACQUIRE) == mark) { marked = true; break; }
            if (__atomic_load_n(&c->h_tmo[0], __ATOMIC_RELAXED) || __atomic_load_n(&c->h_tmo[2], __ATOMIC_RELAXED)) break;
            if (std::chrono::duration<double, std::micro>(std::chrono::steady_clock::now() - h1).count() > c->spin_wait_us) break;
            __builtin_ia32_pause();
        }
    }
    if (!marked) HIP_TRY(hipStreamSynchronize(c->stream));
    else ++c->spin_completions;
    const auto h2 = std::chrono::steady_clock::now();
    c->last_host_launch_us += std::chrono::duration<double, std::micro>(h1 - h0).count();
    c->last_host_sync_us += std::chrono::duration<double, std::micro>(h2 - h1).count();
    c->ev1_recorded = true;
    ++c->cluster_launches;
    if (c->kernel_timing) {
        float kms = 0;
        HIP_TRY(hipEventElapsedTime(&kms, c->kev0, c->kev1));
        c->last_kernel_ms += kms;
    }
    if (launch_was_abandoned(c, (seq << 20) | 1u)) { *ran = false; c->ev1_recorded = false; return C3D_OK; }
    *ran = true;
    c->last_path = 2;
    KernelRecord& k = c->ran;
    k = KernelRecord();
    k.family = KernelRecord::CLUSTER;
    k.pot = c3d::device_pot(m.noe_pot); k.rpw = pl.rpw; k.nb = m.npad / 256; k.wl = m.wl; k.late = pl.late_tiles != 0; k.tp = pl.two_point;
    c->parity ^= 1;
    account_ops(c, nops, 1);
    return C3D_OK;
}

int ensure_group_streams(c3d_ctx* c, int G) {
    for (int g = 1; g < G && g < c3d_ctx::kMaxGroups; ++g) {
        if (c->gstream[g]) continue;
        HIP_TRY(hipStreamCreateWithFlags(&c->gstream[g], hipStreamNonBlocking));
        HIP_TRY(hipEventCreateWithFlags(&c->gev[g], hipEventDisableTiming));
    }
    return C3D_OK;
}

int run_ops_segment(c3d_ctx* c, size_t nops, bool zero_w, bool lbfgs = false) {
    if (nops == 0) return C3D_OK;
    if (c->precision == 64 || zero_w || lbfgs) { }
    else if (c->resident_skip > 0 && c->resident < 1) --c->resident_skip;
    else if (nops >= (size_t)c->resident_min_ops && nops < ((size_t)1 << 20)) {
        bool ran = false;
        int rc = C3D_OK;
        if (cluster_ok(c)) rc = run_cluster(c, nops, &ran);
        if (rc != C3D_OK || ran) return rc;
    }
    c->last_path = 0;
    c->ev1_recorded = false;
    if (c->precision != 64 && (!use_sym(c) || lbfgs)) {
        if (int rc = ensure_pair_targets(c, dev_model(c))) return rc;
    }
    if (lbfgs)
        if (int rc = c->precision == 64 ? ensure_lbfgs<double>(c, c->lb64, c3d::cols64(c->n)) : ensure_lbfgs<float>(c, c->lb, c->npad)) return rc;
    const int G = active_groups(c);
    if (int rc = ensure_group_streams(c, G)) return rc;
    if (G > 1) {
        HIP_TRY(hipEventRecord(c->fork_ev, c->stream));
        for (int g = 1; g < G; ++g) HIP_TRY(hipStreamWaitEvent(c->gstream[g], c->fork_ev, 0));
    }
    size_t done = 0;
    while (done < nops) {
        const size_t chunk = std::min<size_t>(nops - done, c->use_graph ? (size_t)c->graph_chunk : nops - done);
        if (!c->use_graph || chunk < 4) {
            for (int g = 0; g < G; ++g) {
                int par = c->parity;
                for (size_t k = 0; k < chunk; ++k) {
                    if (int rc = launch_op(c, c->program[c->pc + k], g, par)) return rc;
                    par ^= 1;
                }
            }
        } else {
            const Op& first = c->program[c->pc];
            const Op& last = c->program[c->pc + chunk - 1];
            long sig = (long)c->pc;
            if ((first.p.kind == 2 || first.p.kind == 5 || first.p.kind == 8) && last.p.kind == first.p.kind && first.stage == last.stage)
                sig = -(long)(first.stage + 1) - (first.p.kind == 5 ? 1000000L : first.p.kind == 8 ? 2000000L : 0L);
            if (c->graphs.size() >= 2048) {
                for (int g = 0; g < G; ++g) HIP_TRY(hipStreamSynchronize(c->gstream[g]));
                drop_graphs(c);
            }
            for (int g = 0; g < G; ++g) {
                const auto key = std::make_tuple(sig, (int)chunk, c->parity, g);
                auto it = c->graphs.find(key);
                if (it == c->graphs.end()) {
                    hipGraph_t gr = nullptr;
                    HIP_TRY(hipStreamBeginCapture(c->gstream[g], hipStreamCaptureModeThreadLocal));
                    int par = c->parity;
                    int rc = C3D_OK;
                    for (size_t k = 0; k < chunk && rc == C3D_OK; ++k) { rc = launch_op(c, c->program[c->pc + k], g, par); par ^= 1; }
                    hipError_t ce = hipStreamEndCapture(c->gstream[g], &gr);
                    if (rc) { if (gr) (void)hipGraphDestroy(gr); return rc; }
                    LAUNCH_TRY("hipStreamEndCapture", ce);
                    hipGraphExec_t ge = nullptr;
                    hipError_t ie = hipGraphInstantiate(&ge, gr, nullptr, nullptr, 0);
                    (void)hipGraphDestroy(gr);
                    LAUNCH_TRY("hipGraphInstantiate", ie);
                    it = c->graphs.emplace(key, ge).first;
                    ++c->graph_captures;
                }
                HIP_TRY(hipGraphLaunch(it->second, c->gstream[g]));
                ++c->graph_launches;
            }
        }
        c->step_launches += (long)chunk * G;
        if (lbfgs) { c->lbfgs_steps += (long)chunk; c->lbfgs_parity = c->parity ^ (int)(chunk & 1); }
        if (chunk & 1) c->parity ^= 1;
        account_ops(c, chunk, (long)chunk);
        done += chunk;
    }
    for (int g = 1; g < G; ++g) {
        HIP_TRY(hipEventRecord(c->gev[g], c->gstream[g]));
        HIP_TRY(hipStreamWaitEvent(c->stream, c->gev[g], 0));
    }
    if (c->precision == 64) {
        LAUNCH_TRY("fp64 export", c3d::launch_export64(dev_model(c), c->b64, c->parity, c->buf.X[c->parity], c->buf.V[c->parity], c->buf.P[c->parity], c->stream));
        c->last_path = 3;
    }
    c->ran = op_kernel(c, dev_model(c), c->program[c->pc - 1]);
    return C3D_OK;
}

int run_ops(c3d_ctx* c, size_t nops) {
    const bool p64 = c->precision == 64;
    if (p64 ? !c->has_lbfgs : (!c->zero_weight && !c->has_two_point && !c->has_lbfgs)) return run_ops_segment(c, nops, false);
    const size_t end = c->pc + nops;
    while (c->pc < end) {
        const c3d::DevStep& p0 = c->program[c->pc].p;
        const bool z = !p64 && p0.w_rs == 0.0f, tp = !p64 && is_two_point(p0.kind), lb = is_lbfgs(p0.kind);
        size_t k = 1;
        while (c->pc + k < end) {
            const c3d::DevStep& p = c->program[c->pc + k].p;
            if ((!p64 && p.w_rs == 0.0f) != z || (!p64 && is_two_point(p.kind)) != tp || is_lbfgs(p.kind) != lb) break;
            ++k;
        }
        if (int rc = run_ops_segment(c, k, z, lb)) return rc;
    }
    return C3D_OK;
}

int begin_timing(c3d_ctx* c) {
    c->last_ms = 0; c->last_kernel_ms = 0; c->last_steps = 0; c->last_launches = 0; c->last_host_launch_us = 0; c->last_host_sync_us = 0;
    c->ev1_recorded = false;
    if (c->event_timing) HIP_TRY(hipEventRecord(c->ev0, c->stream));
    return C3D_OK;
}
int end_timing(c3d_ctx* c) {
    if (!c->ev1_recorded) {
        if (c->event_timing) HIP_TRY(hipEventRecord(c->ev1, c->stream));
        HIP_TRY(hipStreamSynchronize(c->stream));
    }
    if (!c->event_timing) return C3D_OK;
    HIP_TRY(hipEventSynchronize(c->ev1));
    float ms = 0;
    HIP_TRY(hipEventElapsedTime(&ms, c->ev0, c->ev1));
    c->last_ms = ms;
    return C3D_OK;
}

int partials_finite(c3d_ctx* c, bool* ok) {
    const size_t cnt = (size_t)c->nrep * c->ntiles * 4;
    if (int rc = read_back(c, c->buf.P[c->parity], sizeof(float) * cnt)) return rc;
    const float* h = static_cast<const float*>(c->h_stage);
    *ok = true;
    for (size_t k = 0; k < cnt; ++k) if (!std::isfinite(h[k])) { *ok = false; break; }
    return C3D_OK;
}
}

extern "C" long c3d_schedule_length(const c3d_ctx* c) {
    if (!c) return 0;
    long n = 0;
    for (const Op& op : c->program) n += op.counted;
    return n;
}
extern "C" long c3d_steps_done(const c3d_ctx* c) { return c ? c->steps_done : 0; }

extern "C" int c3d_run_steps(c3d_ctx* c, long nsteps, long* done) {
    if (!c || nsteps < 0) return fail(C3D_ERR_INVALID, "c3d_run_steps: bad arguments");
    if (!c->have_replicas) return fail(C3D_ERR_INVALID, "c3d_run_steps: call c3d_init_replicas first");
    C3D_ENTRY(c, 0u);
    size_t nops = 0;
    long counted = 0;
    while (c->pc + nops < c->program.size() && counted < nsteps) {
        counted += c->program[c->pc + nops].counted;
        ++nops;
    }
    if (int rc = begin_timing(c)) return rc;
    if (int rc = run_ops(c, nops)) return rc;
    if (int rc = end_timing(c)) return rc;
    if (done) *done = counted;
    return C3D_OK;
}

extern "C" int c3d_centre(c3d_ctx* c) {
    if (!c || !c->have_replicas) return fail(C3D_ERR_INVALID, "c3d_centre: bad state");
    C3D_ENTRY(c, 0u);
    LAUNCH_TRY("centre launch", c3d::launch_centre(dev_model(c), c->buf, c->parity, c->stream));
    HIP_TRY(hipStreamSynchronize(c->stream));
    return C3D_OK;
}

extern "C" int c3d_run(c3d_ctx* c) {
    if (!c) return fail(C3D_ERR_INVALID, "c3d_run: null context");
    if (!c->have_replicas) return fail(C3D_ERR_INVALID, "c3d_run: call c3d_init_replicas first");
    C3D_ENTRY(c, 0u);
    if (int rc = begin_timing(c)) return rc;
    const int last_stage = (int)c->stages.size() - 1;
    const bool early = c->gtol > 0.0f && last_stage >= 0 && (c->stages[last_stage].kind == 2 || c->stages[last_stage].kind == 5 || c->stages[last_stage].kind == 8);
    size_t nfixed = c->program.size() - c->pc;
    if (early) {
        nfixed = 0;
        while (c->pc + nfixed < c->program.size() && c->program[c->pc + nfixed].stage != last_stage) ++nfixed;
    }
    if (int rc = run_ops(c, nfixed)) return rc;
    if (early) {
        while (c->pc < c->program.size()) {
            const size_t chunk = std::min<size_t>((size_t)c->check_every, c->program.size() - c->pc);
            if (int rc = run_ops(c, chunk)) return rc;
            double rms = 0;
            if (int rc = max_rms_force(c, &rms)) return rc;
            if (rms < c->gtol) break;
        }
        c->pc = c->program.size();
    }
    LAUNCH_TRY("centre launch", c3d::launch_centre(dev_model(c), c->buf, c->parity, c->stream));
    c->ev1_recorded = false;
    if (int rc = end_timing(c)) return rc;
    bool finite = true;
    if (int rc = partials_finite(c, &finite)) return rc;
    if (!finite) return fail(C3D_ERR_DIVERGED, "c3d_run: the trajectory diverged (non-finite forces); reduce the time step or stiffness");
    return C3D_OK;
}

extern "C" int c3d_last_timing(const c3d_ctx* c, double* ms_total, long* steps, long* launches) {
    if (!c) return fail(C3D_ERR_INVALID, "c3d_last_timing: null context");
    if (ms_total) *ms_total = c->last_ms;
    if (steps) *steps = c->last_steps;
    if (launches) *launches = c->last_launches;
    return C3D_OK;
}

extern "C" int c3d_debug_step_scalars(c3d_ctx* c, int kind, float dt, float t_bath, int rows, const float* psum, const float* state_in,
                                      const int32_t* npos_in, float* scalars, float* state_out, int32_t* npos_out) {
    if (!c || !psum || !state_in || !npos_in || !scalars || !state_out || !npos_out || rows < 1 || rows > (1 << 20))
        return fail(C3D_ERR_INVALID, "c3d_debug_step_scalars: bad arguments");
    if (!(kind == 0 || kind == 1 || kind == 2 || kind == 3 || kind == 5 || kind == 6))
        return fail(C3D_ERR_INVALID, "c3d_debug_step_scalars: kind is 0, 1, 2, 3, 5 or 6");
    if (c->n < 1) return fail(C3D_ERR_INVALID, "c3d_debug_step_scalars: set the targets first (the bead count enters the temperature)");
    C3D_ENTRY(c, unit_bit(UNIT_SYM));
    std::vector<c3d::FireState> st((size_t)rows);
    for (int r = 0; r < rows; ++r) st[r] = c3d::FireState{state_in[2 * r], state_in[2 * r + 1], npos_in[r], 0};
    DevTmp<float> d_psum, d_out;
    DevTmp<c3d::FireState> d_in, d_st;
    HIP_TRY(hipMalloc(&d_psum.p, sizeof(float) * 4 * (size_t)rows));
    HIP_TRY(hipMalloc(&d_out.p, sizeof(float) * 6 * (size_t)rows));
    HIP_TRY(hipMalloc(&d_in.p, sizeof(c3d::FireState) * (size_t)rows));
    HIP_TRY(hipMalloc(&d_st.p, sizeof(c3d::FireState) * (size_t)rows));
    HIP_TRY(hipMemcpyAsync(d_psum.p, psum, sizeof(float) * 4 * (size_t)rows, hipMemcpyHostToDevice, c->stream));
    HIP_TRY(hipMemcpyAsync(d_in.p, st.data(), sizeof(c3d::FireState) * (size_t)rows, hipMemcpyHostToDevice, c->stream));
    LAUNCH_TRY("step scalars launch", c3d::launch_step_scalars(dev_model(c), dev_step(c, kind, dt, 1.0f, 1.0f, 0.85f, t_bath), dev_fire(c), rows,
                                                               d_psum.p, d_in.p, d_out.p, d_st.p, c->stream));
    HIP_TRY(hipMemcpyAsync(scalars, d_out.p, sizeof(float) * 6 * (size_t)rows, hipMemcpyDeviceToHost, c->stream));
    HIP_TRY(hipMemcpyAsync(st.data(), d_st.p, sizeof(c3d::FireState) * (size_t)rows, hipMemcpyDeviceToHost, c->stream));
    HIP_TRY(hipStreamSynchronize(c->stream));
    for (int r = 0; r < rows; ++r) { state_out[2 * r] = st[r].dt; state_out[2 * r + 1] = st[r].alpha; npos_out[r] = st[r].npos; }
    return C3D_OK;
}

static_assert(C3D_LBFGS_MAX_PAIRS == c3d::kLbfgsMaxPairs && C3D_LBFGS_SUMS == c3d::kLbfgsQ, "c3d.h states the L-BFGS stage's sizes");
static_assert(sizeof(c3d::LbfgsState) == 4 * sizeof(int32_t) + C3D_LBFGS_STATE_DOUBLES * sizeof(double), "LbfgsState is 4 ints, then doubles");
extern "C" int c3d_debug_lbfgs_direction(c3d_ctx* c, int rows, const double* sums, const int32_t* state_int_in, const double* state_dbl_in,
                                         const int32_t* first, const int32_t* mem0, int32_t* state_int_out, double* state_dbl_out,
                                         double* coef, int32_t* mask_slot) {
    if (!c || !sums || !state_int_in || !state_dbl_in || !first || !mem0 || !state_int_out || !state_dbl_out || !coef || !mask_slot ||
        rows < 1 || rows > (1 << 16))
        return fail(C3D_ERR_INVALID, "c3d_debug_lbfgs_direction: bad arguments");
    for (int r = 0; r < rows; ++r)
        if (mem0[r] < 1 || mem0[r] > c3d::kLbfgsMaxPairs) return fail(C3D_ERR_INVALID, "c3d_debug_lbfgs_direction: mem0 is 1 .. 8 (lbfgs_memory)");
    if (c->n < 1) return fail(C3D_ERR_INVALID, "c3d_debug_lbfgs_direction: set the targets first (the model is built for a bead count)");
    const bool f64 = c->precision == 64;
    C3D_ENTRY(c, f64 ? unit_bit(UNIT_F64) : 0u);
    constexpr int ND = C3D_LBFGS_STATE_DOUBLES, NC = C3D_LBFGS_COEFS;
    std::vector<c3d::LbfgsState> st((size_t)rows);
    std::vector<int> flags(2 * (size_t)rows);
    for (int r = 0; r < rows; ++r) {
        c3d::LbfgsState& s = st[r];
        s.cnt = state_int_in[4 * r]; s.head = state_int_in[4 * r + 1]; s.mem = state_int_in[4 * r + 2]; s.resets = state_int_in[4 * r + 3];
        memcpy(reinterpret_cast<char*>(&s) + 4 * sizeof(int32_t), state_dbl_in + (size_t)ND * r, sizeof(double) * ND);
        flags[2 * r] = first[r] != 0; flags[2 * r + 1] = mem0[r];
    }
    DevTmp<double> d_sums, d_coef;
    DevTmp<c3d::LbfgsState> d_in, d_out;
    DevTmp<int> d_flags, d_shi;
    HIP_TRY(hipMalloc(&d_sums.p, sizeof(double) * C3D_LBFGS_SUMS * (size_t)rows));
    HIP_TRY(hipMalloc(&d_coef.p, sizeof(double) * NC * (size_t)rows));
    HIP_TRY(hipMalloc(&d_in.p, sizeof(c3d::LbfgsState) * (size_t)rows));
    HIP_TRY(hipMalloc(&d_out.p, sizeof(c3d::LbfgsState) * (size_t)rows));
    HIP_TRY(hipMalloc(&d_flags.p, sizeof(int) * 2 * (size_t)rows));
    HIP_TRY(hipMalloc(&d_shi.p, sizeof(int) * 2 * (size_t)rows));
    HIP_TRY(hipMemcpyAsync(d_sums.p, sums, sizeof(double) * C3D_LBFGS_SUMS * (size_t)rows, hipMemcpyHostToDevice, c->stream));
    HIP_TRY(hipMemcpyAsync(d_in.p, st.data(), sizeof(c3d::LbfgsState) * (size_t)rows, hipMemcpyHostToDevice, c->stream));
    HIP_TRY(hipMemcpyAsync(d_flags.p, flags.data(), sizeof(int) * 2 * (size_t)rows, hipMemcpyHostToDevice, c->stream));
    if (f64) {
        const c3d::Model64 m64 = c3d::model64(dev_model(c), c->model);
        LAUNCH_TRY("fp64 L-BFGS direction launch", c3d::launch_lbfgs_direction64(c3d::step64(m64, 9, 0.0, 1.0, 1.0, 0.85, 0.0), c3d::fire64(c->fire), rows,
                                                                                 d_sums.p, d_in.p, d_flags.p, d_out.p, d_coef.p, d_shi.p, c->stream));
    } else {
        LAUNCH_TRY("L-BFGS direction launch", c3d::launch_lbfgs_direction(dev_model(c), dev_fire(c), rows, d_sums.p, d_in.p, d_flags.p, d_out.p,
                                                                          d_coef.p, d_shi.p, c->stream));
    }
    HIP_TRY(hipMemcpyAsync(coef, d_coef.p, sizeof(double) * NC * (size_t)rows, hipMemcpyDeviceToHost, c->stream));
    HIP_TRY(hipMemcpyAsync(st.data(), d_out.p, sizeof(c3d::LbfgsState) * (size_t)rows, hipMemcpyDeviceToHost, c->stream));
    HIP_TRY(hipMemcpyAsync(flags.data(), d_shi.p, sizeof(int) * 2 * (size_t)rows, hipMemcpyDeviceToHost, c->stream));
    HIP_TRY(hipStreamSynchronize(c->stream));
    for (int r = 0; r < rows; ++r) {
        const c3d::LbfgsState& s = st[r];
        state_int_out[4 * r] = s.cnt; state_int_out[4 * r + 1] = s.head; state_int_out[4 * r + 2] = s.mem; state_int_out[4 * r + 3] = s.resets;
        memcpy(state_dbl_out + (size_t)ND * r, reinterpret_cast<const char*>(&s) + 4 * sizeof(int32_t), sizeof(double) * ND);
        mask_slot[2 * r] = flags[2 * r]; mask_slot[2 * r + 1] = flags[2 * r + 1];
    }
    return C3D_OK;
}

extern "C" const char* c3d_step_kernel_name(const c3d_ctx* c) {
    static thread_local char buf[96];
    if (!c) return "";
    const KernelRecord& k = c->ran;
    auto tf = [](bool b) { return b ? "true" : "false"; };
    switch (k.family) {
        case KernelRecord::CLUSTER:
            snprintf(buf, sizeof(buf), "c3d::k_cluster%s<%d, %d, %d, %d, %s>", k.tp ? "_tp" : "", k.pot, k.rpw, k.nb, k.wl, tf(k.late));
            break;
        case KernelRecord::STEP64:
        case KernelRecord::LBFGS_EVAL64: {
            const char* kernel = k.family == KernelRecord::STEP64 ? "k64_step" : "k64_lbfgs_eval";
            if (k.f64.chunk) snprintf(buf, sizeof(buf), "c3d::%s_chunked<%d, %s, %s, %d>", kernel, k.f64.pot, tf(k.f64.gen), tf(k.f64.fold), k.f64.chunk);
            else snprintf(buf, sizeof(buf), "c3d::%s<%d, %s, %s>", kernel, k.f64.pot, tf(k.f64.gen), tf(k.f64.fold));
            break;
        }
        case KernelRecord::PAIRS_SYM: snprintf(buf, sizeof(buf), "c3d::k_pairs_sym<%d, %s, false>", k.pot, tf(k.rs1)); break;
        case KernelRecord::STEP:
        case KernelRecord::LBFGS_EVAL: {
            const char* kernel = k.family == KernelRecord::STEP ? "k_step" : "k_lbfgs_eval";
            if (k.step.chunk) {
                if (k.step.wide) snprintf(buf, sizeof(buf), "c3d::%s_chunked<4, false, 4, 16, true, %d>", kernel, k.step.chunk);
                else snprintf(buf, sizeof(buf), "c3d::%s_chunked<%d, %s, %d, 8, false, %d>", kernel, k.step.pot, tf(k.step.gen), k.step.rpw, k.step.chunk);
            } else if (k.step.wide) snprintf(buf, sizeof(buf), "c3d::%s<4, false, 4, false, 16, true>", kernel);
            else snprintf(buf, sizeof(buf), "c3d::%s<%d, %s, %d, %s, 8, false>", kernel, k.step.pot, tf(k.step.gen), k.step.rpw, tf(k.step.nc));
            break;
        }
        default: return "";
    }
    return buf;
}
```

chromosome3d_amd/lib.py:

```python
import ctypes as C
import os

import numpy as np

_HERE = os.path.dirname(os.path.abspath(__file__))
LIB_PATH = os.path.join(_HERE, "_lib", "libc3d.so")


class C3DError(RuntimeError):
    pass


class Model(C.Structure):
    _fields_ = [("min_sep", C.c_int32), ("noe_pot", C.c_int32), ("rep_sep", C.c_int32), ("ang_mode", C.c_int32),
                ("s_noe", C.c_float), ("rswitch", C.c_float), ("asym", C.c_float),
                ("k_bond", C.c_float), ("b0", C.c_float), ("k_ang", C.c_float), ("a0", C.c_float),
                ("r0_rep", C.c_float), ("k_rep", C.c_float), ("mass", C.c_float), ("fbeta", C.c_float), ("masym", C.c_float), ("mrswitch", C.c_float),
                ("msoexp", C.c_int32)]


class Stage(C.Structure):
    _fields_ = [("kind", C.c_int32), ("nsteps", C.c_int32), ("dt", C.c_float), ("w_all", C.c_float),
                ("w_vdw", C.c_float), ("repel_s", C.c_float), ("t_bath", C.c_float)]


class FireParams(C.Structure):
    _fields_ = [("dt_start", C.c_float), ("dt_max", C.c_float), ("f_inc", C.c_float), ("f_dec", C.c_float),
                ("alpha_start", C.c_float), ("f_alpha", C.c_float), ("max_step", C.c_float), ("n_min", C.c_int32)]


_vp, _i, _l, _d, _f = C.c_void_p, C.c_int, C.c_long, C.c_double, C.c_float
_i32p, _fp, _dp = C.POINTER(C.c_int32), C.POINTER(C.c_float), C.POINTER(C.c_double)
SIGNATURES = {
    "c3d_last_error": (C.c_char_p, []),
    "c3d_version": (C.c_char_p, []),
    "c3d_device_count": (_i, []),
    "c3d_create": (_i, [_i, C.POINTER(_vp)]),
    "c3d_destroy": (None, [_vp]),
    "c3d_default_model": (None, [C.POINTER(Model)]),
    "c3d_default_fire": (None, [C.POINTER(FireParams)]),
    "c3d_default_schedule": (_i, [C.POINTER(Stage), _i, _i]),
    "c3d_set_if_matrix": (_i, [_vp, _dp, _i, _d, _d]),
    "c3d_set_restraints": (_i, [_vp, _i, _i, _i32p, _i32p, _i32p]),
    "c3d_get_dist10": (_i, [_vp, _i32p]),
    "c3d_num_beads": (_i, [_vp]),
    "c3d_num_restraints": (_i, [_vp]),
    "c3d_set_model": (_i, [_vp, C.POINTER(Model)]),
    "c3d_set_schedule": (_i, [_vp, C.POINTER(Stage), _i, C.POINTER(FireParams), _f, _i]),
    "c3d_set_option": (_i, [_vp, C.c_char_p, _d]),
    "c3d_set_process_option": (_i, [C.c_char_p, _d]),
    "c3d_init_replicas": (_i, [_vp, _i, C.c_uint64, C.c_uint32]),
    "c3d_embed_replicas": (_i, [_vp, _i]),
    "c3d_set_coords": (_i, [_vp, _fp]),
    "c3d_get_coords": (_i, [_vp, _fp]),
    "c3d_get_velocities": (_i, [_vp, _fp]),
    "c3d_get_coords_f64": (_i, [_vp, _dp]),
    "c3d_get_velocities_f64": (_i, [_vp, _dp]),
    "c3d_set_coords_f64": (_i, [_vp, _dp]),
    "c3d_run": (_i, [_vp]),
    "c3d_run_steps": (_i, [_vp, _l, C.POINTER(_l)]),
    "c3d_schedule_length": (_l, [_vp]),
    "c3d_steps_done": (_l, [_vp]),
    "c3d_centre": (_i, [_vp]),
    "c3d_last_timing": (_i, [_vp, _dp, C.POINTER(_l), C.POINTER(_l)]),
    "c3d_get_stat": (_i, [_vp, C.c_char_p, _dp]),
    "c3d_step_kernel_name": (C.c_char_p, [_vp]),
    "c3d_debug_tear16": (_i, [_vp, _i, C.POINTER(C.c_ulonglong), C.POINTER(C.c_ulonglong), C.POINTER(C.c_ulonglong)]),
    "c3d_debug_step_scalars": (_i, [_vp, _i, _f, _f, _i, _fp, _fp, _i32p, _fp, _fp, _i32p]),
    "c3d_debug_lbfgs_direction": (_i, [_vp, _i, _dp, _i32p, _dp, _i32p, _i32p, _i32p, _dp, _dp, _i32p]),
    "c3d_dg_smoothed_bounds": (_i, [_vp, _fp, _fp]),
    "c3d_debug_if_ranks": (_i, [_vp, _dp, _i, _dp, _dp, C.POINTER(C.c_size_t)]),
    "c3d_eval": (_i, [_vp, _f, _f, _f, _fp, _dp]),
    "c3d_eval_f64": (_i, [_vp, _d, _d, _d, _dp, _dp]),
    "c3d_get_energies": (_i, [_vp, _dp]),
    "c3d_score_replicas": (_i, [_vp, _dp, _i, _i32p, _dp, _dp]),
    "c3d_compare_replicas": (_i, [_vp, _dp, _i, _dp, _dp]),
    "c3d_debug_distance_ranks": (_i, [_vp, _i, _dp]),
    "c3d_superpose_replicas": (_i, [_vp, _i, _dp, _i, _i, _dp, _i32p, _dp, _dp]),
    "c3d_rmsd_table": (_i, [_vp, _dp, _i, _i, _dp, _i32p]),
    "c3d_ensemble_map": (_i, [_vp, _dp, _i, _i32p, _i, _d, _dp, _dp, _dp]),
    "c3d_ensemble_score": (_i, [_vp, _dp, _i, _dp, _i, _i32p, _i, _d, _dp, _dp]),
    "c3d_geometry_replicas": (_i, [_vp, _dp, _i, _d, _i, C.POINTER(C.c_int64), _i32p, _dp, _dp]),
    "c3d_separation_profile": (_i, [_vp, _dp, _i, _i32p, _i, _d, _dp, _dp, _dp]),
    "c3d_stratified_score": (_i, [_vp, _dp, _i, _i, _dp, _i, _dp, _dp, C.POINTER(C.c_int64)]),
    "c3d_bead_scores": (_i, [_vp, _dp, _i, _i32p, _i, _dp, _i, _dp, C.POINTER(C.c_int64), _i32p, _i32p, C.POINTER(C.c_int64)]),
    "c3d_sphere_points": (_i, [_i, _dp]),
    "c3d_accessibility": (_i, [_vp, _dp, _i, _d, _d, _dp, _i, _i32p, _dp]),
    "c3d_rank": (_i, [_vp, _i32p]),
    "c3d_reduce_model": (_i, [_dp, _i, _dp]),
    "c3d_model_similarity": (_i, [_dp, _dp, _i, _dp, _dp]),
    "c3d_parse_if_file": (_i, [C.c_char_p, C.POINTER(_dp), C.POINTER(_i)]),
    "c3d_free": (None, [_vp]),
    "c3d_write_front_half": (_i, [_i32p, _i, _i, C.c_char_p, C.c_char_p, C.c_char_p, C.POINTER(_i)]),
    "c3d_read_tbl": (_i, [C.c_char_p, C.POINTER(_i32p), C.POINTER(_i32p), C.POINTER(_i32p), C.POINTER(_i)]),
    "c3d_write_pdb": (_i, [C.c_char_p, _fp, _i, _d, _d, _d, C.c_char_p]),
    "c3d_set_residue_sequence": (_i, [C.c_char_p]),
    "c3d_shape_pdb": (_i, [C.c_char_p, C.c_char_p, C.c_char_p]),
    "c3d_read_pdb_ca": (_i, [C.c_char_p, C.POINTER(_fp), C.POINTER(_i)]),
    "c3d_assess": (_i, [_fp, _i, _i, _i32p, _i32p, _i32p, _d, C.POINTER(_i), _dp]),
    "c3d_write_violations": (_i, [_fp, _i, _i, _i32p, _i32p, _i32p, _d, C.c_char_p, C.c_char_p, C.c_char_p, C.POINTER(_i), _dp]),
    "c3d_spearman_if_dist": (_i, [_dp, _fp, _i, _i, _dp]),
    "c3d_spearman_if_dist_batch": (_i, [_dp, _fp, _i, _i, _i, _dp]),
}

SUPERPOSE_MIRROR, SUPERPOSE_APPLY = 1, 2
GEOMETRY_FIELDS = 6
STRATUM_FIELDS = 3
BEAD_FIELDS = 3
ACCESS_MAX_POINTS = 1024
LBFGS_MAX_PAIRS, LBFGS_SUMS, LBFGS_STATE_DOUBLES, LBFGS_COEFS = 8, 36, 129, 17

_lib = None


def load():
    global _lib
    if _lib is None:
        if not os.path.exists(LIB_PATH):
            raise C3DError(f"{LIB_PATH} not found: build it with `python -c 'import __graft_entry__ as g; g.build()'` "
                           "(make -C chromosome3d_amd/csrc). There is no CPU fallback.")
        os.environ.setdefault("HSA_DISABLE_COREDUMP_ON_EXCEPTION", "1")
        L = C.CDLL(LIB_PATH)
        for name, (res, args) in SIGNATURES.items():
            fn = getattr(L, name)
            fn.restype = res
            fn.argtypes = args
        _lib = L
    return _lib


def check(rc):
    if rc != 0:
        raise C3DError(f"libc3d error {rc}: {load().c3d_last_error().decode(errors='replace')}")


def fptr(a):
    return a.ctypes.data_as(_fp)


def dptr(a):
    return a.ctypes.data_as(_dp)


def i32ptr(a):
    return a.ctypes.data_as(_i32p)


def as_f32(a):
    return np.ascontiguousarray(a, dtype=np.float32)
```

include/c3d.h:

```cpp
#ifndef C3D_H_
#define C3D_H_

#include <stddef.h>
#include <stdint.h>

#ifdef __cplusplus
extern "C" {
#endif

typedef enum {
    C3D_OK = 0,
    C3D_ERR_INVALID = -1,
    C3D_ERR_NO_DEVICE = -2,
    C3D_ERR_HIP = -3,
    C3D_ERR_IO = -4,
    C3D_ERR_NOMEM = -5,
    C3D_ERR_DIVERGED = -6
} c3d_status;

typedef struct c3d_ctx c3d_ctx;

typedef struct {
    int32_t min_sep;
    int32_t noe_pot;
    int32_t rep_sep;
    int32_t ang_mode;
    float s_noe;
    float rswitch;
    float asym;
    float k_bond, b0;
    float k_ang, a0;
    float r0_rep;
    float k_rep;
    float mass;
    float fbeta;
    float masym;
    float mrswitch;
    int32_t msoexp;
} c3d_model;

typedef struct {
    int32_t kind;
    int32_t nsteps;
    float dt;
    float w_all;
    float w_vdw;
    float repel_s;
    float t_bath;
} c3d_stage;

typedef struct {
    float dt_start, dt_max, f_inc, f_dec, alpha_start, f_alpha, max_step;
    int32_t n_min;
} c3d_fire_params;

const char* c3d_last_error(void);
const char* c3d_version(void);
int c3d_device_count(void);
int c3d_create(int device, c3d_ctx** out);
void c3d_destroy(c3d_ctx* ctx);

void c3d_default_model(c3d_model* m);
void c3d_default_fire(c3d_fire_params* f);
int c3d_default_schedule(c3d_stage* stages, int cap, int min_steps);

int c3d_set_if_matrix(c3d_ctx* ctx, const double* IF, int n, double alpha, double K);
int c3d_set_restraints(c3d_ctx* ctx, int n, int R, const int32_t* ri, const int32_t* rj, const int32_t* rt10);
int c3d_get_dist10(c3d_ctx* ctx, int32_t* dist10);
int c3d_num_beads(const c3d_ctx* ctx);
int c3d_num_restraints(const c3d_ctx* ctx);

int c3d_set_model(c3d_ctx* ctx, const c3d_model* m);
int c3d_set_schedule(c3d_ctx* ctx, const c3d_stage* stages, int n_stages, const c3d_fire_params* fire,
                     float gtol, int check_every);
int c3d_set_option(c3d_ctx* ctx, const char* key, double value);
#define C3D_MAX_BEADS_DEFAULT 5120
#define C3D_MAX_BEADS_LIMIT 16384
#define C3D_F64_MAX_BEADS_DEFAULT 2560
#define C3D_F64_MAX_BEADS_LIMIT 16384
#define C3D_EMBED_MAX_BEADS_DEFAULT 4549
#define C3D_EMBED_MAX_BEADS_LIMIT 16384
#define C3D_EMBED_SCRATCH_BYTES (4ull << 30)
#define C3D_SCORE_SCRATCH_BYTES (1ull << 30)

int c3d_set_process_option(const char* key, double value);

int c3d_init_replicas(c3d_ctx* ctx, int n_replicas, uint64_t seed, uint32_t first_replica);
int c3d_embed_replicas(c3d_ctx* ctx, int iters);
int c3d_set_coords(c3d_ctx* ctx, const float* xyz);
int c3d_get_coords(c3d_ctx* ctx, float* xyz);
int c3d_get_velocities(c3d_ctx* ctx, float* v);
int c3d_get_coords_f64(c3d_ctx* ctx, double* xyz);
int c3d_get_velocities_f64(c3d_ctx* ctx, double* v);
int c3d_set_coords_f64(c3d_ctx* ctx, const double* xyz);

int c3d_run(c3d_ctx* ctx);
int c3d_run_steps(c3d_ctx* ctx, long nsteps, long* done);
long c3d_schedule_length(const c3d_ctx* ctx);
long c3d_steps_done(const c3d_ctx* ctx);
int c3d_centre(c3d_ctx* ctx);
int c3d_last_timing(const c3d_ctx* ctx, double* ms_total, long* steps, long* launches);
int c3d_get_stat(const c3d_ctx* ctx, const char* key, double* value);
int c3d_debug_tear16(c3d_ctx* ctx, int iterations, unsigned long long* unit_reads, unsigned long long* torn, unsigned long long* fresh);
int c3d_debug_step_scalars(c3d_ctx* ctx, int kind, float dt, float t_bath, int rows, const float* psum, const float* state_in,
                           const int32_t* npos_in, float* scalars, float* state_out, int32_t* npos_out);
#define C3D_LBFGS_MAX_PAIRS 8
#define C3D_LBFGS_SUMS (4 * C3D_LBFGS_MAX_PAIRS + 4)
#define C3D_LBFGS_STATE_DOUBLES (1 + 2 * C3D_LBFGS_MAX_PAIRS * C3D_LBFGS_MAX_PAIRS)
#define C3D_LBFGS_COEFS (1 + 2 * C3D_LBFGS_MAX_PAIRS)
int c3d_debug_lbfgs_direction(c3d_ctx* ctx, int rows, const double* sums, const int32_t* state_int_in, const double* state_dbl_in,
                              const int32_t* first, const int32_t* mem0, int32_t* state_int_out, double* state_dbl_out, double* coef,
                              int32_t* mask_slot);
int c3d_dg_smoothed_bounds(c3d_ctx* ctx, float* U, float* L);
int c3d_debug_if_ranks(c3d_ctx* ctx, const double* IF, int range, double* rank, double* saa, size_t* m);
const char* c3d_step_kernel_name(const c3d_ctx* ctx);

int c3d_eval(c3d_ctx* ctx, float w_all, float w_vdw, float repel_s, float* F, double* e);
int c3d_eval_f64(c3d_ctx* ctx, double w_all, double w_vdw, double repel_s, double* F, double* e);
int c3d_get_energies(c3d_ctx* ctx, double* e);
int c3d_score_replicas(c3d_ctx* ctx, const double* IF, int range, int32_t* satisfied, double* sum_dev, double* rho);
#define C3D_COMPARE_MAX_MODELS 256
int c3d_compare_replicas(c3d_ctx* ctx, const double* extra_xyz, int n_extra, double* spearman, double* rmsd);
int c3d_debug_distance_ranks(c3d_ctx* ctx, int replica, double* rank);
#define C3D_SUPERPOSE_MIRROR 1
#define C3D_SUPERPOSE_APPLY  2
#define C3D_SUPERPOSE_MAX_ITERS 50
int c3d_superpose_replicas(c3d_ctx* ctx, int reference, const double* ref_xyz, int flags, int iters, double* rmsd, int32_t* mirrored,
                           double* mean_xyz, double* rmsf);
int c3d_rmsd_table(c3d_ctx* ctx, const double* extra_xyz, int n_extra, int flags, double* rmsd, int32_t* mirrored);
int c3d_ensemble_map(c3d_ctx* ctx, const double* extra_xyz, int n_extra, const int32_t* pick, int n_pick, double cutoff,
                     double* mean, double* sd, double* contact);
int c3d_ensemble_score(c3d_ctx* ctx, const double* IF, int range, const double* extra_xyz, int n_extra,
                       const int32_t* pick, int n_pick, double cutoff, double* rho_mean, double* rho_contact);
#define C3D_GEOMETRY_FIELDS 6
int c3d_geometry_replicas(c3d_ctx* ctx, const double* extra_xyz, int n_extra, double cutoff, int sep,
                          int64_t* clashes, int32_t* bead_clashes, double* nearest, double* chain);
int c3d_separation_profile(c3d_ctx* ctx, const double* extra_xyz, int n_extra, const int32_t* pick, int n_pick,
                           double cutoff, double* mean, double* sd, double* contact);
#define C3D_STRATUM_FIELDS 3
int c3d_stratified_score(c3d_ctx* ctx, const double* IF, int range, int max_sep, const double* extra_xyz, int n_extra,
                         double* rho, double* scc, int64_t* sums);
#define C3D_BEAD_FIELDS 3
int c3d_bead_scores(c3d_ctx* ctx, const double* IF, int range, const int32_t* beads, int n_beads,
                    const double* extra_xyz, int n_extra,
                    double* rho, int64_t* sums, int32_t* restrained, int32_t* satisfied, int64_t* dev_milli);
#define C3D_ACCESS_MAX_POINTS 1024
int c3d_sphere_points(int n_points, double* u);
int c3d_accessibility(c3d_ctx* ctx, const double* extra_xyz, int n_extra, double radius, double probe,
                      const double* points, int n_points, int32_t* exposed, double* device_ms);
int c3d_rank(c3d_ctx* ctx, int32_t* rank);

int c3d_parse_if_file(const char* path, double** IF, int* n);
void c3d_free(void* p);
int c3d_write_front_half(const int32_t* dist10, int n, int min_sep, const char* dist_path,
                         const char* rr_path, const char* tbl_path, int* n_restraints);
int c3d_read_tbl(const char* path, int32_t** ri, int32_t** rj, int32_t** rt10, int* R);
int c3d_write_pdb(const char* path, const float* xyz, int n, double e_noe, double e_bond, double e_rep,
                  const char* title);
int c3d_set_residue_sequence(const char* seq1);
int c3d_read_pdb_ca(const char* path, float** xyz, int* n);
int c3d_shape_pdb(const char* in_path, const char* out_path, const char* log_path);
int c3d_assess(const float* xyz, int n, int R, const int32_t* ri, const int32_t* rj, const int32_t* rt10,
               double relax, int* satisfied, double* sum_dev);
int c3d_write_violations(const float* xyz, int n, int R, const int32_t* ri, const int32_t* rj, const int32_t* rt10, double relax,
                         const char* pdb_label, const char* tbl_label, const char* path, int* satisfied, double* sum_dev);
int c3d_spearman_if_dist(const double* IF, const float* xyz, int n, int range, double* rho);
int c3d_spearman_if_dist_batch(const double* IF, const float* xyz, int n, int n_models, int range, double* rho);

int c3d_reduce_model(const double* xyz, int n, double* out);
int c3d_model_similarity(const double* a, const double* b, int n, double* spearman, double* rmsd);

#ifdef __cplusplus
}
#endif
#endif
```

Baseline: 4.705 million.

## Add step-budget load balancing for uneven replica-per-XCD cluster placement

When the replica count leaves some XCDs with fewer replicas (nrep mod 8 == 4), the resident cluster kernel now runs in segments. Replicas rotate between heavy and light XCDs, and light XCDs use a different partition and wave count and take more steps per segment, so all XCDs finish together. A per-replica budget table sets the run, skip and step count for each replica in each segment. The heavy/light speed ratio is measured from device timestamps and fed back, and state is checkpointed so a failed segment can be restored. This adds several launches, checkpoint copies and host bookkeeping per range.

```diff
diff --git a/chromosome3d_amd/csrc/c3d_api.cpp b/chromosome3d_amd/csrc/c3d_api.cpp
--- a/chromosome3d_amd/csrc/c3d_api.cpp
+++ b/chromosome3d_amd/csrc/c3d_api.cpp
@@ -43,6 +43,7 @@
     free_replica_buffers(c);
     dev_free(c->buf.tgt); dev_free(c->buf.tgs2);
     dev_free(c->d_prog); dev_free(c->d_claim); dev_free(c->d_score);
+    dev_free(c->d_budget); dev_free(c->d_budget_ckpt);
     if (c->h_tmo) (void)hipHostFree(c->h_tmo);
     if (c->h_stage) (void)hipHostFree(c->h_stage);
     for (hipEvent_t e : {c->ev0, c->ev1, c->kev0, c->kev1, c->fork_ev}) if (e) (void)hipEventDestroy(e);
diff --git a/chromosome3d_amd/csrc/c3d_cluster.hip b/chromosome3d_amd/csrc/c3d_cluster.hip
--- a/chromosome3d_amd/csrc/c3d_cluster.hip
+++ b/chromosome3d_amd/csrc/c3d_cluster.hip
@@ -21,12 +21,12 @@
 #define CSTAMP_C(k) do { } while (0)
 #endif
 
-template <int POT, int RPW, int NB, int WL, bool LATE, bool TWO>
+template <int POT, int RPW, int NB, int WL, bool LATE, bool TWO, bool BUD = false>
 __device__ __forceinline__ void cluster_body(
-    const float* __restrict__ tgt, unsigned* __restrict__ claim, const StepRun* __restrict__ runs, const int P, const int CW, const int NH,
-    const int static_place, const int nbeads, const int run0, const int skip0, const int nsteps,
+    const float* __restrict__ tgt, unsigned* __restrict__ claim, const StepRun* __restrict__ runs, const int P_launch, const int CW_launch, const int NH,
+    const int static_place, const int nbeads, const int run0_launch, const int skip0_launch, const int nsteps_launch,
     const unsigned tag_base, u32x4* __restrict__ rec, volatile unsigned* __restrict__ timeout, const unsigned expected,
-    const AnnealIO& io, const DevModel& m, const DevFire& fp) {
+    const AnnealIO& io, const DevModel& m, const DevFire& fp, const int* __restrict__ bud = nullptr) {
     constexpr int NPAD = 256 * NB;
     constexpr int MAXT = NPAD / 8;
     constexpr int KUMAX = NB > 2 ? 3 : 2;
@@ -45,6 +45,14 @@
     const unsigned long long t_entry = __builtin_amdgcn_s_memrealtime();
 #endif
     const int tid = threadIdx.x, lane = tid & 63, wave = tid >> 6;
+    int P = P_launch, CW = CW_launch;
+    bool light_xcd = false;
+    if constexpr (BUD) {
+        const int lx = (int)(__builtin_amdgcn_s_getreg((3 << 11) | 20) & 0x7) - ((static_place >> 8) & 0xff);
+        light_xcd = lx >= bud[0] && lx < bud[0] + bud[1];
+        if (light_xcd) { P = bud[2]; CW = bud[3]; }
+        if (wave >= CW + NH) return;
+    }
     const int nthreads = (CW + NH) * 64;
     const int RW = CW * RPW;
 
@@ -69,6 +77,11 @@
     const int cwave = wave - NH;
     const int wg_row0 = part * RW;
     const int row0 = wg_row0 + cwave * RPW;
+    int run0 = run0_launch, skip0 = skip0_launch, nsteps = nsteps_launch, rep_bud = 0;
+    if constexpr (BUD) {
+        const int* e = bud + 4 + 4 * min(max(lrep, 0), m.nrep_g - 1);
+        rep_bud = e[0]; run0 = e[1]; skip0 = e[2]; nsteps = e[3];
+    }
     const StepRun first_run = runs[run0];
     float4 traw[RPW][NB];
 #pragma unroll
@@ -91,7 +104,7 @@
             traw[r][jb] = t;
         }
     if (lxcd < 0 || lxcd >= nxcd || lrep >= m.nrep_g) return;
-    const int rep = m.rep_base + lrep;
+    const int rep = BUD ? rep_bud : m.rep_base + lrep;
     const bool solo = P == 1;
     if (!is_compute) __builtin_amdgcn_s_setprio(3);
 
@@ -360,7 +373,11 @@
                 const int tl = (wg_row0 + lane) >> 3;
                 if ((lane & 7) == 0 && lane < RW && tl < m.ntiles) reinterpret_cast<float4*>(io.pout)[(size_t)rep * m.ntiles + tl] = t;
                 if (lane == 0 && part == 0) io.sout[rep] = st;
+                if constexpr (BUD) {
+                    if (lane == 0) { atomicMax(&claim[light_xcd ? 11 : 10], (unsigned)__builtin_amdgcn_s_memrealtime()); __threadfence(); }
+                }
                 if (lane == 0 && atomicAdd(&claim[8], 1u) + 1u == expected) {
+                    if constexpr (BUD) { timeout[5] = atomicOr(&claim[10], 0u); timeout[6] = atomicOr(&claim[11], 0u); __threadfence_system(); }
                     const unsigned seen = sp_mode ? atomicOr(&claim[9], 0u) : 1u;
                     if ((seen & (seen - 1u)) == 0u) timeout[1] = tag_base | 1u;
                     else timeout[2] = 1u;
@@ -428,6 +445,10 @@
 __global__ __launch_bounds__(kClMaxThreads) void k_cluster(C3D_CLUSTER_ARGS) { cluster_body<POT, RPW, NB, WL, LATE, false>(C3D_CLUSTER_PASS); }
 template <int POT, int RPW, int NB, int WL, bool LATE>
 __global__ __launch_bounds__(kClMaxThreads) void k_cluster_tp(C3D_CLUSTER_ARGS) { cluster_body<POT, RPW, NB, WL, LATE, true>(C3D_CLUSTER_PASS); }
+template <int POT, int RPW, int NB, int WL, bool LATE>
+__global__ __launch_bounds__(kClMaxThreads) void k_cluster_bud(C3D_CLUSTER_ARGS, const int* __restrict__ bud) { cluster_body<POT, RPW, NB, WL, LATE, false, true>(C3D_CLUSTER_PASS, bud); }
+template <int POT, int RPW, int NB, int WL, bool LATE>
+__global__ __launch_bounds__(kClMaxThreads) void k_cluster_tp_bud(C3D_CLUSTER_ARGS, const int* __restrict__ bud) { cluster_body<POT, RPW, NB, WL, LATE, true, true>(C3D_CLUSTER_PASS, bud); }
 #undef C3D_CLUSTER_ARGS
 #undef C3D_CLUSTER_PASS
 
@@ -469,11 +490,11 @@
 }
 
 
-bool cluster_plan(const DevModel& m, int num_cus, int num_xcc, int forced_geom, int forced_late, int xcd_count, ClusterPlan* plan) {
+static bool cluster_plan_search(const DevModel& m, int num_cus, int num_xcc, int forced_geom, int forced_late, int xcd_count, int per_xcd,
+                                int need_rpw, int need_late, ClusterPlan* plan) {
     if (m.npad > 1024 || num_xcc != 8 || num_cus < 8 || num_cus % 8) return false;
     const int cus_per_xcd = num_cus / 8;
     if (xcd_count < 1 || xcd_count > 8) return false;
-    const int per_xcd = (m.nrep_g + xcd_count - 1) / xcd_count;
     const int nb = m.npad / 256;
     static const int geoms[][4] = {{8, 1, 4, 1}, {8, 2, 4, 1}, {12, 2, 4, 1}, {8, 4, 4, 1}, {10, 4, 4, 1}, {12, 4, 4, 1}, {8, 3, 4, 1},
                                    {4, 2, 4, 1}, {4, 4, 4, 1}, {6, 4, 4, 1}};
@@ -484,6 +505,7 @@
         const int cw = g[0], rpw = g[1], nh = g[2], wpc = g[3], rw = cw * rpw;
         if (fcw && (cw != fcw || rpw != frpw || nh != fnh)) continue;
         if (rw % 8 || rw > 64) continue;
+        if (need_rpw && (rpw != need_rpw || nh != plan->helpers)) continue;
         if (rpw * nb > 8) continue;
         if (m.noe_pot < 3 && (m.wl != 4 || m.nleft != 0)) continue;
         if (m.nleft > 0 && (nh != 4 || (rw + 8 * (nh - 1) - 1) / (8 * (nh - 1)) > 4)) continue;
@@ -493,6 +515,7 @@
         const int kumax = nb > 2 ? 3 : 2;
         const int late = P > 1 && forced_late != 0 && cluster_late_ok(m.noe_pot, rpw, nb, m.wl) &&
                          (m.noe_pot != 4 || ((cw + 3) / 4) * rpw * (4 * (nb - 1) + m.wl) >= 12);
+        if (need_rpw && late != need_late) continue;
         if ((late ? m.n : m.n + 2 * ((m.n + 7) / 8)) > (late ? threads - 64 : threads) * kumax) continue;
         size_t lds = sizeof(float) * (3 * m.npad + 4 * (m.npad / 8) + 9 * 64 + 24 * 64 + 16) + (size_t)cw * rpw * nb * 64 * 16;
         if (wpc == 1) { if (lds < 84 * 1024) lds = 84 * 1024; }
@@ -504,6 +527,7 @@
         const double cost = wpc == 1 ? valu + serial : (valu > serial ? valu + 0.35 * serial : 0.5 * valu + serial);
         if (cost < best) {
             best = cost; found = true;
+            plan->cost = cost;
             plan->rpw = rpw; plan->cw = cw; plan->helpers = nh; plan->wgs_per_cu = wpc; plan->parts = P; plan->per_xcd = per_xcd;
             plan->grid = num_cus * wpc; plan->threads = threads; plan->units = 2 * rw; plan->device = 0; plan->lds = lds;
             plan->expected = (unsigned)(m.nrep_g * P);
@@ -512,6 +536,22 @@
         }
     }
     return found;
+}
+
+bool cluster_plan(const DevModel& m, int num_cus, int num_xcc, int forced_geom, int forced_late, int xcd_count, ClusterPlan* plan) {
+    if (xcd_count < 1 || xcd_count > 8) return false;
+    const int per_xcd = (m.nrep_g + xcd_count - 1) / xcd_count;
+    *plan = ClusterPlan();
+    if (!cluster_plan_search(m, num_cus, num_xcc, forced_geom, forced_late, xcd_count, per_xcd, 0, 0, plan)) return false;
+    if (xcd_count == 8 && m.nrep_g >= 12 && m.nrep_g % 8 == 4) {
+        ClusterPlan light = *plan;
+        if (cluster_plan_search(m, num_cus, num_xcc, forced_geom, forced_late, xcd_count, per_xcd - 1, plan->rpw, plan->late_tiles, &light) &&
+            light.cost < plan->cost) {
+            plan->light_parts = light.parts; plan->light_cw = light.cw; plan->light_threads = light.threads; plan->light_lds = light.lds;
+            plan->light_cost = light.cost;
+        }
+    }
+    return true;
 }
 
 size_t cluster_record_bytes(const DevModel& m, const ClusterPlan& pl) { (void)pl; return (size_t)2 * m.nrep_g * (m.npad + m.npad / 4) * 16; }
@@ -541,6 +581,23 @@
             hipLaunchKernelGGL((K<POT, RPW, NB, WL, LATE>), dim3(pl.grid), dim3(pl.threads), pl.lds, s, tgt, claim, runs, pl.parts, pl.cw, pl.helpers, \
                                sp, m.n, run0, skip0, nsteps, tag_base, reinterpret_cast<u32x4*>(rec), timeout, pl.expected, io, m, fp);                \
     } while (0)
+    if (pl.budget) {
+        if constexpr (POT == 4) {
+#define C3D_CL_LAUNCH_BUD(K)                                                                                                                          \
+    do {                                                                                                                                              \
+        if (pl.t0 && pl.t1)                                                                                                                           \
+            hipExtLaunchKernelGGL((K<POT, RPW, NB, WL, LATE>), dim3(pl.grid), dim3(pl.threads), pl.lds, s, pl.t0, pl.t1, 0, tgt, claim, runs,          \
+                                  pl.parts, pl.cw, pl.helpers, sp, m.n, run0, skip0, nsteps, tag_base, reinterpret_cast<u32x4*>(rec), timeout, pl.expected, io, m, fp, pl.budget); \
+        else                                                                                                                                          \
+            hipLaunchKernelGGL((K<POT, RPW, NB, WL, LATE>), dim3(pl.grid), dim3(pl.threads), pl.lds, s, tgt, claim, runs, pl.parts, pl.cw, pl.helpers, \
+                               sp, m.n, run0, skip0, nsteps, tag_base, reinterpret_cast<u32x4*>(rec), timeout, pl.expected, io, m, fp, pl.budget);     \
+    } while (0)
+            if constexpr (kHasTp) { if (tp) C3D_CL_LAUNCH_BUD(k_cluster_tp_bud); }
+            if constexpr (kHasLean) { if (!tp) C3D_CL_LAUNCH_BUD(k_cluster_bud); }
+#undef C3D_CL_LAUNCH_BUD
+            return hipGetLastError();
+        } else return hipErrorInvalidValue;
+    }
     if constexpr (kHasTp) { if (tp) C3D_CL_LAUNCH(k_cluster_tp); }
     if constexpr (kHasLean) { if (!tp) C3D_CL_LAUNCH(k_cluster); }
 #undef C3D_CL_LAUNCH
@@ -581,6 +638,12 @@
         if constexpr (TP) k = reinterpret_cast<const void*>(&k_cluster_tp<POT, R, B, W, L>);
         else k = reinterpret_cast<const void*>(&k_cluster<POT, R, B, W, L>);
         if (e == hipSuccess) e = hipFuncSetAttribute(k, hipFuncAttributeMaxDynamicSharedMemorySize, 160 * 1024);
+        if constexpr (POT == 4) {
+            const void* kb;
+            if constexpr (TP) kb = reinterpret_cast<const void*>(&k_cluster_tp_bud<POT, R, B, W, L>);
+            else kb = reinterpret_cast<const void*>(&k_cluster_bud<POT, R, B, W, L>);
+            if (e == hipSuccess) e = hipFuncSetAttribute(kb, hipFuncAttributeMaxDynamicSharedMemorySize, 160 * 1024);
+        }
     });
     return e;
 }
diff --git a/chromosome3d_amd/csrc/c3d_config.cpp b/chromosome3d_amd/csrc/c3d_config.cpp
--- a/chromosome3d_amd/csrc/c3d_config.cpp
+++ b/chromosome3d_amd/csrc/c3d_config.cpp
@@ -95,6 +95,14 @@
     {"embed_batch",               0,     whole_in<&X::embed_batch, 0, INT_MAX>, "embed_batch is 0 (by the scratch budget) or a number of replicas"},
     {"column_chunk",              G,     chunk<&X::column_chunk, c3d::column_chunk_valid>, "column_chunk must be 0 (the library's choice), 256, 1024 or 2048"},
     {"graph_chunk",               G,     set_graph_chunk, "graph_chunk must be >= 8"},
+};
+const char* set_budget_ratio(c3d_ctx* c, double v, const char* refusal) { return v != 0 && (v <= 1000 || v > 4000) ? refusal : store(c->cluster_budget_ratio, (int)v); }
+const char* set_cluster_budget(c3d_ctx* c, double v, const char*) { c->budget_skip = c->budget_backoff = 0; return store(c->cluster_budget, v < 0 ? -1 : (v != 0)); }
+const Option kBudgetOptions[] = {
+    {"cluster_budget",            0,     set_cluster_budget},
+    {"cluster_budget_min_steps",  0,     whole_in<&X::cluster_budget_min_steps, 1, INT_MAX>, "cluster_budget_min_steps must be an integer >= 1"},
+    {"cluster_budget_ratio",      0,     set_budget_ratio, "cluster_budget_ratio is 0 (model, then measured) or 1001..4000 permille"},
+    {"cluster_budget_inject_segment", 0, whole_in<&X::budget_inject_segment, 0, 64>, "cluster_budget_inject_segment is a segment number, 0..64"},
 };
 
 template <auto M> double value(const c3d_ctx* c) { return (double)(c->*M); }
@@ -170,6 +178,14 @@
     {"units_loaded", [](const c3d_ctx*) { return (double)units_loaded(); }},
     {"units_loaded_mask", [](const c3d_ctx* c) { return (double)units_loaded_mask(c->device); }},
 };
+const Stat kBudgetStats[] = {
+    {"budget_segments", value<&X::budget_segments>},
+    {"budget_ranges", value<&X::budget_ranges>},
+    {"budget_light_parts", planned<&c3d::ClusterPlan::light_parts>},
+    {"budget_light_waves", planned<&c3d::ClusterPlan::light_cw>},
+    {"budget_ratio", value<&X::budget_last_ratio>},
+    {"budget_seen_ratio", value<&X::budget_seen_ratio>},
+};
 
 template <class Row, size_t N> const Row* find_row(const Row (&rows)[N], const char* key) {
     for (const Row& r : rows) if (!strcmp(key, r.key)) return &r;
@@ -309,6 +325,7 @@
 extern "C" int c3d_set_option(c3d_ctx* c, const char* key, double value) {
     if (!c || !key) return fail(C3D_ERR_INVALID, "c3d_set_option: null argument");
     const Option* row = find_row(kOptions, key);
+    if (!row) row = find_row(kBudgetOptions, key);
     if (!row) return fail(C3D_ERR_INVALID, std::string("unknown option ") + key);
     if (const char* refusal = row->admit(c, value, row->refusal)) return fail(C3D_ERR_INVALID, refusal);
     return drop_stale_gated(c, row->stale);
@@ -317,6 +334,7 @@
 extern "C" int c3d_get_stat(const c3d_ctx* c, const char* key, double* value) {
     if (!c || !key || !value) return fail(C3D_ERR_INVALID, "c3d_get_stat: null argument");
     const Stat* row = find_row(kStats, key);
+    if (!row) row = find_row(kBudgetStats, key);
     if (!row) return fail(C3D_ERR_INVALID, std::string("c3d_get_stat: unknown key ") + key);
     if (row->enter) return row->enter(c, value);
     *value = row->get(c);
diff --git a/chromosome3d_amd/csrc/c3d_ctx.h b/chromosome3d_amd/csrc/c3d_ctx.h
--- a/chromosome3d_amd/csrc/c3d_ctx.h
+++ b/chromosome3d_amd/csrc/c3d_ctx.h
@@ -113,6 +113,10 @@
     int cluster_geom = 0;
     int xcd_base = 0, xcd_count = 8;
     bool static_place = true;
+    int cluster_budget = -1;
+    int cluster_budget_min_steps = C3D_CLUSTER_BUDGET_MIN_STEPS_DEFAULT;
+    int cluster_budget_ratio = 0;
+    int budget_inject_segment = 0;
     int eval_rpw = 4;
     bool pair_targets = true;
     bool wide_tiles = true;
@@ -190,6 +194,17 @@
     unsigned *h_tmo = nullptr, *h_tmo_dev = nullptr;
     int resident_skip = 0;
     int resident_backoff = 0;
+    int* d_budget = nullptr;
+    size_t budget_cap = 0;
+    void* d_budget_ckpt = nullptr;
+    size_t budget_ckpt_bytes = 0;
+    int budget_ratio = 0;
+    int budget_skip = 0, budget_backoff = 0;
+    double budget_us_per_step = 0;
+    std::vector<int> h_budget;
+    long budget_segments = 0, budget_ranges = 0;
+    int budget_last_ratio = 0;
+    int budget_seen_ratio = 0;
     void* h_stage = nullptr;
     size_t h_stage_bytes = 0;
     void* d_score = nullptr;
diff --git a/chromosome3d_amd/csrc/c3d_internal.h b/chromosome3d_amd/csrc/c3d_internal.h
--- a/chromosome3d_amd/csrc/c3d_internal.h
+++ b/chromosome3d_amd/csrc/c3d_internal.h
@@ -171,7 +171,14 @@
     unsigned expected = 0;
     size_t lds;
     hipEvent_t t0 = nullptr, t1 = nullptr;
-};
+    int light_parts = 0, light_cw = 0, light_threads = 0;
+    size_t light_lds = 0;
+    double cost = 0, light_cost = 0;
+    const int* budget = nullptr;
+};
+struct ClusterBudgetHead { int light_first, light_count, light_parts, light_cw; };
+struct ClusterBudgetEntry { int rep, run0, skip0, nsteps; };
+bool cluster_budget_segments(long K, int q, int ratio_permille, int* h, int* d);
 bool cluster_plan(const DevModel& m, int num_cus, int num_xcc, int forced_geom, int forced_late, int xcd_count, ClusterPlan* plan);
 size_t cluster_record_bytes(const DevModel& m, const ClusterPlan& pl);
 hipError_t launch_cluster(const DevModel& m, const DevFire& fp, const ClusterPlan& pl, const AnnealIO& io, const float* tgt, void* rec,
diff --git a/chromosome3d_amd/csrc/c3d_run.cpp b/chromosome3d_amd/csrc/c3d_run.cpp
--- a/chromosome3d_amd/csrc/c3d_run.cpp
+++ b/chromosome3d_amd/csrc/c3d_run.cpp
@@ -6,6 +6,20 @@
 
 static bool is_two_point(int kind) { return kind == 5 || kind == 6; }
 static bool is_lbfgs(int kind) { return kind == 8 || kind == 9; }
+
+namespace c3d {
+bool cluster_budget_segments(long K, int q, int ratio_permille, int* h, int* d) {
+    if (K < 1 || q < 1 || ratio_permille <= 1000) return false;
+    const long S = 2 * q + 1, e = ratio_permille - 1000;
+    const long den = 1000 * S + q * e;
+    const long dd = (e * K + den / 2) / den;
+    const long H = K - q * dd;
+    if (dd < 1 || H < S || K >= (1L << 20)) return false;
+    for (long i = 0; i < S; ++i) h[i] = (int)(H / S + (i < H % S ? 1 : 0));
+    *d = (int)dd;
+    return true;
+}
+}
 
 namespace c3d::host {
 void drop_graphs(c3d_ctx* c) {
@@ -70,6 +84,8 @@
         c->crec_bytes = bytes;
     }
     c->cl_seq = 0;
+    c->budget_ratio = 0;
+    c->budget_us_per_step = 0;
     c->cl_ok = true;
     return C3D_OK;
 }
@@ -179,12 +195,18 @@
     return !c3d::general_tail(dev_model(c));
 }
 
-bool launch_was_abandoned(c3d_ctx* c, unsigned done_mark) {
+bool launch_was_abandoned(c3d_ctx* c, unsigned done_mark, bool budget = false) {
     if (c->h_tmo[2]) { c->h_tmo[2] = 0; c->static_place = false; ++c->placement_mismatches; }
     const bool complete = c->h_tmo[1] == done_mark;
-    if (!*c->h_tmo && complete) { c->resident_backoff = 0; return false; }
+    if (!*c->h_tmo && complete) { (budget ? c->budget_backoff : c->resident_backoff) = 0; return false; }
     if (!*c->h_tmo) ++c->cluster_incomplete;
     *c->h_tmo = 0;
+    if (budget) {
+        c->budget_backoff = std::min(4096, std::max(4, 2 * c->budget_backoff));
+        c->budget_skip = c->budget_backoff;
+        ++c->resident_fallbacks;
+        return true;
+    }
     c->resident_backoff = std::min(4096, std::max(4, 2 * c->resident_backoff));
     c->resident_skip = c->resident_backoff;
     ++c->resident_fallbacks;
@@ -198,48 +220,48 @@
     c->pc += nops;
 }
 
-int run_cluster(c3d_ctx* c, size_t nops, bool* ran) {
-    if (c->prog_dirty) {
-        if (c->prog_runs.size() > c->prog_cap) {
-            if (c->d_prog) { HIP_TRY(hipStreamSynchronize(c->stream)); dev_free(c->d_prog); }
-            c->prog_cap = std::max<size_t>(c->prog_runs.size(), 256);
-            HIP_TRY(hipMalloc(&c->d_prog, sizeof(c3d::StepRun) * c->prog_cap));
-        }
-        HIP_TRY(hipMemcpyAsync(c->d_prog, c->prog_runs.data(), sizeof(c3d::StepRun) * c->prog_runs.size(), hipMemcpyHostToDevice, c->stream));
-        HIP_TRY(hipStreamSynchronize(c->stream));
-        c->prog_dirty = false;
-    }
+int upload_program(c3d_ctx* c) {
+    if (!c->prog_dirty) return C3D_OK;
+    if (c->prog_runs.size() > c->prog_cap) {
+        if (c->d_prog) { HIP_TRY(hipStreamSynchronize(c->stream)); dev_free(c->d_prog); }
+        c->prog_cap = std::max<size_t>(c->prog_runs.size(), 256);
+        HIP_TRY(hipMalloc(&c->d_prog, sizeof(c3d::StepRun) * c->prog_cap));
+    }
+    HIP_TRY(hipMemcpyAsync(c->d_prog, c->prog_runs.data(), sizeof(c3d::StepRun) * c->prog_runs.size(), hipMemcpyHostToDevice, c->stream));
+    HIP_TRY(hipStreamSynchronize(c->stream));
+    c->prog_dirty = false;
+    return C3D_OK;
+}
+
+int cluster_launch(c3d_ctx* c, c3d::ClusterPlan pl, int run0, int skip0, int nsteps, bool inject, double spin_us, bool* ok, double* wait_us) {
     const unsigned seq = c->cl_seq % c3d_ctx::kClaimSets;
     if (seq == 0) {
         HIP_TRY(hipMemsetAsync(c->d_crec, 0, c->crec_bytes, c->stream));
         HIP_TRY(hipMemsetAsync(c->d_claim, 0, sizeof(unsigned) * c3d_ctx::kClaimWords * c3d_ctx::kClaimSets, c->stream));
     }
     ++c->cl_seq;
-    if (c->inject_timeout) { *c->h_tmo = 1; c->inject_timeout = false; }
+    if (inject && c->inject_timeout) { *c->h_tmo = 1; c->inject_timeout = false; }
     c->h_tmo[1] = 0;
     const c3d::DevModel m = dev_model(c);
-    c3d::ClusterPlan pl = c->cl_plan;
-    if (c->inject_incomplete) { ++pl.expected; c->inject_incomplete = false; }
+    if (inject && c->inject_incomplete) { ++pl.expected; c->inject_incomplete = false; }
     if (c->kernel_timing) { pl.t0 = c->kev0; pl.t1 = c->kev1; }
-    pl.static_place = c->static_place ? (c->inject_misplaced ? 2 : 1) : 0;
+    pl.static_place = c->static_place ? (inject && c->inject_misplaced ? 2 : 1) : 0;
     pl.xcd_base = c->xcd_base;
-    pl.two_point = false;
-    for (size_t k = 0; k < nops && !pl.two_point; ++k) pl.two_point = is_two_point(c->program[c->pc + k].p.kind);
-    c->inject_misplaced = false;
+    if (inject) c->inject_misplaced = false;
     c->h_tmo[2] = 0;
     const auto h0 = std::chrono::steady_clock::now();
     LAUNCH_TRY("cluster launch", c3d::launch_cluster(m, dev_fire(c), pl, c3d::anneal_io(c->buf, c->parity), c->buf.tgt, c->d_crec, c->d_prog,
-                                                     c->op_run[c->pc], c->op_skip[c->pc], (int)nops, seq << 20, c->h_tmo_dev,
+                                                     run0, skip0, nsteps, seq << 20, c->h_tmo_dev,
                                                      c->d_claim + c3d_ctx::kClaimWords * seq, c->stream));
     if (c->event_timing) HIP_TRY(hipEventRecord(c->ev1, c->stream));
     const auto h1 = std::chrono::steady_clock::now();
     bool marked = false;
-    if (c->spin_wait_us > 0 && !c->kernel_timing) {
+    if (spin_us > 0 && !c->kernel_timing) {
         const unsigned mark = (seq << 20) | 1u;
         for (;;) {
             if (__atomic_load_n(&c->h_tmo[1], __ATOMIC_ACQUIRE) == mark) { marked = true; break; }
             if (__atomic_load_n(&c->h_tmo[0], __ATOMIC_RELAXED) || __atomic_load_n(&c->h_tmo[2], __ATOMIC_RELAXED)) break;
-            if (std::chrono::duration<double, std::micro>(std::chrono::steady_clock::now() - h1).count() > c->spin_wait_us) break;
+            if (std::chrono::duration<double, std::micro>(std::chrono::steady_clock::now() - h1).count() > spin_us) break;
             __builtin_ia32_pause();
         }
     }
@@ -248,6 +270,7 @@
     const auto h2 = std::chrono::steady_clock::now();
     c->last_host_launch_us += std::chrono::duration<double, std::micro>(h1 - h0).count();
     c->last_host_sync_us += std::chrono::duration<double, std::micro>(h2 - h1).count();
+    if (wait_us) *wait_us = std::chrono::duration<double, std::micro>(h2 - h1).count();
     c->ev1_recorded = true;
     ++c->cluster_launches;
     if (c->kernel_timing) {
@@ -255,15 +278,149 @@
         HIP_TRY(hipEventElapsedTime(&kms, c->kev0, c->kev1));
         c->last_kernel_ms += kms;
     }
-    if (launch_was_abandoned(c, (seq << 20) | 1u)) { *ran = false; c->ev1_recorded = false; return C3D_OK; }
-    *ran = true;
+    *ok = !launch_was_abandoned(c, (seq << 20) | 1u, pl.budget != nullptr);
+    if (!*ok) c->ev1_recorded = false;
+    return C3D_OK;
+}
+
+bool range_has_two_point(const c3d_ctx* c, size_t nops) {
+    for (size_t k = 0; k < nops; ++k)
+        if (is_two_point(c->program[c->pc + k].p.kind)) return true;
+    return false;
+}
+void account_cluster(c3d_ctx* c, const c3d::ClusterPlan& pl, size_t nops, long launches) {
+    const c3d::DevModel m = dev_model(c);
     c->last_path = 2;
     KernelRecord& k = c->ran;
     k = KernelRecord();
     k.family = KernelRecord::CLUSTER;
     k.pot = c3d::device_pot(m.noe_pot); k.rpw = pl.rpw; k.nb = m.npad / 256; k.wl = m.wl; k.late = pl.late_tiles != 0; k.tp = pl.two_point;
+    account_ops(c, nops, launches);
+}
+
+int run_cluster(c3d_ctx* c, size_t nops, bool* ran) {
+    if (int rc = upload_program(c)) return rc;
+    c3d::ClusterPlan pl = c->cl_plan;
+    pl.two_point = range_has_two_point(c, nops);
+    if (int rc = cluster_launch(c, pl, c->op_run[c->pc], c->op_skip[c->pc], (int)nops, true, c->spin_wait_us, ran, nullptr)) return rc;
+    if (!*ran) return C3D_OK;
     c->parity ^= 1;
-    account_ops(c, nops, 1);
+    account_cluster(c, pl, nops, 1);
+    return C3D_OK;
+}
+
+bool budget_applies(const c3d_ctx* c, size_t nops) {
+    if (c->cluster_budget == 0 || nops < (size_t)c->cluster_budget_min_steps || nops >= ((size_t)1 << 20)) return false;
+    if (c->xcd_count != 8 || c->xcd_base != 0 || c->nrep < 12 || c->nrep % 8 != 4) return false;
+    if (!c->cl_plan.light_parts && c->cluster_budget != 1) return false;
+    return c3d::device_pot(dev_model(c).noe_pot) == 4;
+}
+int budget_ratio_now(const c3d_ctx* c) {
+    if (c->cluster_budget_ratio) return c->cluster_budget_ratio;
+    if (c->budget_ratio) return c->budget_ratio;
+    const c3d::ClusterPlan& p = c->cl_plan;
+    return p.light_parts && p.light_cost > 0 ? std::min(2000, std::max(1001, (int)(1000.0 * p.cost / p.light_cost + 0.5))) : 1000;
+}
+
+int run_budget(c3d_ctx* c, size_t nops, bool* ran) {
+    *ran = false;
+    const int nrep = c->nrep, q = (nrep - 4) / 8, S = 2 * q + 1;
+    const int ratio = budget_ratio_now(c);
+    std::vector<int> h((size_t)S);
+    int d = 0;
+    if (!c3d::cluster_budget_segments((long)nops, q, ratio, h.data(), &d)) return C3D_OK;
+    if (c->budget_skip > 0) { --c->budget_skip; return C3D_OK; }
+    if (int rc = upload_program(c)) return rc;
+    const c3d::ClusterPlan& base = c->cl_plan;
+    const int lp = base.light_parts ? base.light_parts : base.parts, lcw = base.light_parts ? base.light_cw : base.cw;
+    const size_t stride = 4 + 4 * (size_t)nrep;
+    std::vector<int>& tab = c->h_budget;
+    tab.assign(stride * S, 0);
+    std::vector<size_t> pos((size_t)nrep, c->pc);
+    for (int i = 0; i < S; ++i) {
+        int* t = tab.data() + stride * i;
+        t[0] = 4; t[1] = 4; t[2] = lp; t[3] = lcw;
+        for (int cl = 0; cl < S; ++cl) {
+            const int k = (cl - i + S) % S;
+            const bool light = k < q;
+            for (int j = 0; j < 4; ++j) {
+                const int rep = 4 * cl + j, lrep = light ? 4 + j + 8 * k : j + 8 * (k - q), n = h[i] + (light ? d : 0);
+                int* e = t + 4 + 4 * lrep;
+                e[0] = rep; e[1] = c->op_run[pos[rep]]; e[2] = c->op_skip[pos[rep]]; e[3] = n;
+                pos[rep] += (size_t)n;
+            }
+        }
+    }
+    for (int r = 0; r < nrep; ++r)
+        if (pos[r] != c->pc + nops) return fail(C3D_ERR_INVALID, "step budgets: a replica's segments do not add up to the range");
+    if (tab.size() > c->budget_cap) {
+        if (c->d_budget) { HIP_TRY(hipStreamSynchronize(c->stream)); dev_free(c->d_budget); }
+        c->budget_cap = 0;
+        HIP_TRY(hipMalloc(&c->d_budget, sizeof(int) * tab.size()));
+        c->budget_cap = tab.size();
+    }
+    const size_t xb = sizeof(float) * c->rep_floats * nrep, pb = sizeof(float) * 4 * (size_t)nrep * c->ntiles, sb = sizeof(c3d::FireState) * nrep;
+    if (2 * xb + pb + sb > c->budget_ckpt_bytes) {
+        if (c->d_budget_ckpt) { HIP_TRY(hipStreamSynchronize(c->stream)); dev_free(c->d_budget_ckpt); }
+        c->budget_ckpt_bytes = 0;
+        HIP_TRY(hipMalloc(&c->d_budget_ckpt, 2 * xb + pb + sb));
+        c->budget_ckpt_bytes = 2 * xb + pb + sb;
+    }
+    const int par0 = c->parity;
+    char* ck = static_cast<char*>(c->d_budget_ckpt);
+    auto checkpoint = [&](bool restore) -> hipError_t {
+        struct { void* buf; size_t off, bytes; } part[4] = {{c->buf.X[par0], 0, xb}, {c->buf.V[par0], xb, xb}, {c->buf.P[par0], 2 * xb, pb}, {c->buf.S[par0], 2 * xb + pb, sb}};
+        for (const auto& p : part) {
+            const hipError_t e = restore ? hipMemcpyAsync(p.buf, ck + p.off, p.bytes, hipMemcpyDeviceToDevice, c->stream)
+                                         : hipMemcpyAsync(ck + p.off, p.buf, p.bytes, hipMemcpyDeviceToDevice, c->stream);
+            if (e != hipSuccess) return e;
+        }
+        return hipSuccess;
+    };
+    HIP_TRY(hipMemcpyAsync(c->d_budget, tab.data(), sizeof(int) * tab.size(), hipMemcpyHostToDevice, c->stream));
+    LAUNCH_TRY("step budgets: checkpoint", checkpoint(false));
+    c3d::ClusterPlan pl = base;
+    pl.two_point = range_has_two_point(c, nops);
+    pl.threads = std::max(base.threads, base.light_parts ? base.light_threads : base.threads);
+    pl.lds = std::max(base.lds, base.light_parts ? base.light_lds : base.lds);
+    pl.expected = (unsigned)(4 * (q + 1) * base.parts + 4 * q * lp);
+    double seen_sum = 0;
+    int seen_n = 0;
+    for (int i = 0; i < S; ++i) {
+        pl.budget = c->d_budget + stride * i;
+        const double expect_us = (c->budget_us_per_step > 0 ? c->budget_us_per_step : 4.0) * h[i];
+        const double spin = c->spin_wait_us > 0 ? std::max(c->spin_wait_us, 1.25 * expect_us) : 0.0;
+        bool ok = false;
+        double wait_us = 0;
+        c->h_tmo[5] = c->h_tmo[6] = 0;
+        if (int rc = cluster_launch(c, pl, c->op_run[c->pc], c->op_skip[c->pc], h[i], i == c->budget_inject_segment, spin, &ok, &wait_us)) return rc;
+        ++c->budget_segments;
+        if (!ok) {
+            LAUNCH_TRY("step budgets: restore", checkpoint(true));
+            HIP_TRY(hipStreamSynchronize(c->stream));
+            c->parity = par0;
+            c->budget_inject_segment = 0;
+            return C3D_OK;
+        }
+        c->parity ^= 1;
+        const double gap_us = 0.01 * (double)(int)(c->h_tmo[5] - c->h_tmo[6]);
+        const double t_heavy = gap_us >= 0 ? wait_us : wait_us + gap_us, t_light = gap_us >= 0 ? wait_us - gap_us : wait_us;
+        if (c->h_tmo[5] && c->h_tmo[6] && t_heavy > 0.5 * wait_us && t_light > 0.5 * wait_us) {
+            seen_sum += (t_heavy / h[i]) / (t_light / (h[i] + d));
+            ++seen_n;
+            c->budget_us_per_step = t_heavy / h[i];
+        }
+    }
+    if (seen_n) {
+        c->budget_seen_ratio = (int)(1000.0 * seen_sum / seen_n + 0.5);
+        const int r = std::min(2000, std::max(1001, c->budget_seen_ratio));
+        c->budget_ratio = c->budget_ratio ? (c->budget_ratio + r + 1) / 2 : r;
+    }
+    c->budget_last_ratio = ratio;
+    ++c->budget_ranges;
+    c->budget_inject_segment = 0;
+    *ran = true;
+    account_cluster(c, pl, nops, S);
     return C3D_OK;
 }
 
@@ -283,7 +440,10 @@
     else if (nops >= (size_t)c->resident_min_ops && nops < ((size_t)1 << 20)) {
         bool ran = false;
         int rc = C3D_OK;
-        if (cluster_ok(c)) rc = run_cluster(c, nops, &ran);
+        if (cluster_ok(c)) {
+            if (budget_applies(c, nops)) rc = run_budget(c, nops, &ran);
+            if (rc == C3D_OK && !ran) rc = run_cluster(c, nops, &ran);
+        }
         if (rc != C3D_OK || ran) return rc;
     }
     c->last_path = 0;
@@ -433,6 +593,34 @@
     return C3D_OK;
 }
 
+extern "C" int c3d_debug_budget_segments(long K, int q, int ratio_permille, int* h, int* d, int* light) {
+    if (!h || !d || !light || q < 1 || q > 31) return 0;
+    const int S = 2 * q + 1;
+    if (!c3d::cluster_budget_segments(K, q, ratio_permille, h, d)) return 0;
+    for (int i = 0; i < S; ++i)
+        for (int cl = 0; cl < S; ++cl) light[i * S + cl] = (cl - i + S) % S < q;
+    return 1;
+}
+extern "C" int c3d_debug_budget_plan(int n, int nrep, int* out) {
+    if (!out || n < 1 || n > 1024 || nrep < 1) return 0;
+    c3d_ctx c;
+    c3d_default_model(&c.model);
+    c.n = n; c.npad = (n + 255) / 256 * 256; c.ntiles = (n + 7) / 8; c.nrep = nrep;
+    c3d::DevModel m = dev_model(&c);
+    m.nrep = nrep; m.nrep_g = nrep; m.rep_base = 0;
+    c3d::ClusterPlan p;
+    for (int k = 0; k < 12; ++k) out[k] = 0;
+    if (!c3d::cluster_plan(m, 256, 8, 0, -1, 8, &p)) return 0;
+    out[0] = p.parts; out[1] = p.cw; out[2] = p.rpw; out[3] = p.late_tiles; out[4] = p.threads; out[5] = p.helpers;
+    out[6] = p.light_parts; out[7] = p.light_cw; out[8] = p.light_threads;
+    if (p.light_parts) {
+        const int late = p.late_tiles, kumax = m.npad / 256 > 2 ? 3 : 2;
+        out[9] = (late ? m.n : m.n + 2 * ((m.n + 7) / 8)) <= (late ? p.light_threads - 64 : p.light_threads) * kumax;
+    }
+    out[10] = (int)(1000.0 * p.cost); out[11] = (int)(1000.0 * p.light_cost);
+    return 1;
+}
+
 extern "C" int c3d_centre(c3d_ctx* c) {
     if (!c || !c->have_replicas) return fail(C3D_ERR_INVALID, "c3d_centre: bad state");
     C3D_ENTRY(c, 0u);
diff --git a/chromosome3d_amd/lib.py b/chromosome3d_amd/lib.py
--- a/chromosome3d_amd/lib.py
+++ b/chromosome3d_amd/lib.py
@@ -68,6 +68,8 @@
     "c3d_debug_tear16": (_i, [_vp, _i, C.POINTER(C.c_ulonglong), C.POINTER(C.c_ulonglong), C.POINTER(C.c_ulonglong)]),
     "c3d_debug_step_scalars": (_i, [_vp, _i, _f, _f, _i, _fp, _fp, _i32p, _fp, _fp, _i32p]),
     "c3d_debug_lbfgs_direction": (_i, [_vp, _i, _dp, _i32p, _dp, _i32p, _i32p, _i32p, _dp, _dp, _i32p]),
+    "c3d_debug_budget_segments": (_i, [_l, _i, _i, _i32p, _i32p, _i32p]),
+    "c3d_debug_budget_plan": (_i, [_i, _i, _i32p]),
     "c3d_dg_smoothed_bounds": (_i, [_vp, _fp, _fp]),
     "c3d_debug_if_ranks": (_i, [_vp, _dp, _i, _dp, _dp, C.POINTER(C.c_size_t)]),
     "c3d_eval": (_i, [_vp, _f, _f, _f, _fp, _dp]),
diff --git a/include/c3d.h b/include/c3d.h
--- a/include/c3d.h
+++ b/include/c3d.h
@@ -76,6 +76,7 @@
 int c3d_set_option(c3d_ctx* ctx, const char* key, double value);
 #define C3D_MAX_BEADS_DEFAULT 5120
 #define C3D_MAX_BEADS_LIMIT 16384
+#define C3D_CLUSTER_BUDGET_MIN_STEPS_DEFAULT 1000
 #define C3D_F64_MAX_BEADS_DEFAULT 2560
 #define C3D_F64_MAX_BEADS_LIMIT 16384
 #define C3D_EMBED_MAX_BEADS_DEFAULT 4549
@@ -102,6 +103,8 @@
 int c3d_last_timing(const c3d_ctx* ctx, double* ms_total, long* steps, long* launches);
 int c3d_get_stat(const c3d_ctx* ctx, const char* key, double* value);
 int c3d_debug_tear16(c3d_ctx* ctx, int iterations, unsigned long long* unit_reads, unsigned long long* torn, unsigned long long* fresh);
+int c3d_debug_budget_segments(long K, int q, int ratio_permille, int* h, int* d, int* light);
+int c3d_debug_budget_plan(int n, int nrep, int* out);
 int c3d_debug_step_scalars(c3d_ctx* ctx, int kind, float dt, float t_bath, int rows, const float* psum, const float* state_in,
                            const int32_t* npos_in, float* scalars, float* state_out, int32_t* npos_out);
 #define C3D_LBFGS_MAX_PAIRS 8
```

After: 4.644 million. 1.3% lower.
